# jacklishufan/InstructAny2Pix

Hardware: AMD Instinct MI355X
Metric: denoise-steps/sec (512x512, 50-step DDIM, batch 8) (higher is better)
Workload: dtype f16; 1 GPU; BASELINE configs[2]: 512x512, latent [8,4,64,64], 50-step DDIM, ctx 81 (77 text + 4 IP tokens), SDXL-base UNet + IP-Adapter; global_batch=8, parallelism=dp1, context_kv=projected in every step (reference schedule, as rounds 1-4), ranks=1, dist_backend=none (single process), weight_broadcast_route=none

## Files before the change

### include/ia2p.h

```cpp
#ifndef IA2P_H
#define IA2P_H

#include <stddef.h>
#include <stdint.h>

#ifdef __cplusplus
extern "C" {
#endif

typedef struct ia2p_ctx ia2p_ctx;

typedef enum {
  IA2P_OK = 0,
  IA2P_ERR_INVALID = 1,
  IA2P_ERR_SHAPE = 2,
  IA2P_ERR_KEY = 3,
  IA2P_ERR_STATE = 4,
  IA2P_ERR_NOMEM = 5,
  IA2P_ERR_HIP = 6,
  IA2P_ERR_ARCH = 7
} ia2p_status;

#define IA2P_MAX_BLOCKS 4

typedef struct {
  int in_channels, out_channels;
  int n_blocks;
  int block_out_channels[IA2P_MAX_BLOCKS];
  int transformer_layers_per_block[IA2P_MAX_BLOCKS];
  int num_heads[IA2P_MAX_BLOCKS];
  int layers_per_block;
  int cross_attention_dim;
  int norm_num_groups;
  float norm_eps;
  int addition_time_embed_dim;
  int projection_class_embeddings_input_dim;
  int time_embed_dim;
  int time_proj_dim;
  int mid_transformer_layers;
  int num_time_ids;
} ia2p_unet_config;

ia2p_status ia2p_create(const ia2p_unet_config* cfg, ia2p_ctx** out);
void ia2p_destroy(ia2p_ctx* ctx);
const char* ia2p_last_error(ia2p_ctx* ctx);
int ia2p_device_is_gfx950(void);

size_t ia2p_arena_bytes(ia2p_ctx* ctx);
ia2p_status ia2p_bind_arena(ia2p_ctx* ctx, void* dev_arena, size_t bytes);
ia2p_status ia2p_load_tensor(ia2p_ctx* ctx, const char* key, const void* dev_src, const int64_t* shape, int ndim, void* stream);
ia2p_status ia2p_finalize_weights(ia2p_ctx* ctx);
size_t ia2p_arena_raw_bytes(ia2p_ctx* ctx);
ia2p_status ia2p_adopt_arena(ia2p_ctx* ctx, int with_ip_adapter);
ia2p_status ia2p_adopt_arena_on(ia2p_ctx* ctx, int with_ip_adapter, void* stream);
ia2p_status ia2p_bcast_arena(ia2p_ctx* ctx, void* rccl_comm, int root, int with_ip_adapter, void* stream);
int ia2p_rccl_available(void);
ia2p_status ia2p_set_gn_fuse(ia2p_ctx* ctx, int mode);
ia2p_status ia2p_set_ip_adapter(ia2p_ctx* ctx, int enabled, int num_tokens, float scale);

size_t ia2p_workspace_bytes(ia2p_ctx* ctx, int B, int h, int w, int L);
ia2p_status ia2p_unet_forward(ia2p_ctx* ctx, void* stream, const void* sample, float timestep, const void* context, int L,
                              const void* text_embeds, const void* time_ids, void* out, int B, int h, int w,
                              void* workspace, size_t workspace_bytes);
ia2p_status ia2p_unet_forward_v(ia2p_ctx* ctx, void* stream, const void* sample, const float* timesteps, const float* ip_scales,
                                const void* context, const void* kv, int L, const void* text_embeds, const void* time_ids, void* out,
                                int B, int h, int w, void* workspace, size_t workspace_bytes);

size_t ia2p_context_kv_bytes(ia2p_ctx* ctx, int B, int L);
ia2p_status ia2p_project_context(ia2p_ctx* ctx, void* stream, const void* context, int L, int B, void* kv, size_t kv_bytes,
                                 void* workspace, size_t workspace_bytes);
ia2p_status ia2p_unet_forward_kv(ia2p_ctx* ctx, void* stream, const void* sample, float timestep, const void* kv, int L,
                                 const void* text_embeds, const void* time_ids, void* out, int B, int h, int w,
                                 void* workspace, size_t workspace_bytes);

ia2p_status ia2p_autotune(ia2p_ctx* ctx, void* stream, const void* sample, float timestep, const void* context, int L,
                          const void* text_embeds, const void* time_ids, void* out, int B, int h, int w,
                          void* workspace, size_t workspace_bytes, int reps, int* sites);
size_t ia2p_plan_export(char* buf, size_t len);
int ia2p_plan_import(const char* text);
void ia2p_plan_clear(void);
unsigned long long ia2p_plan_generation(void);

ia2p_status ia2p_ddim_step(void* stream, const void* x, const void* eps_u, const void* eps_c, float g, float c_x, float c_e,
                           void* out, void* out2, int64_t n);
ia2p_status ia2p_ddim_step_v(void* stream, const void* x, const void* eps_u, const void* eps_c, const float* coef, void* out, void* out2,
                             int B, int64_t per);
ia2p_status ia2p_mask_blend(void* stream, const void* x, const void* init, const void* noise, const void* mask, float c0, float c1,
                            void* out, void* out2, int B, int C, int64_t HW);

ia2p_status ia2p_groupnorm_silu(void* stream, const void* x, void* y, const void* gamma, const void* beta, int B, int HW, int C,
                                int groups, float eps, int silu, float* partial_ws );
ia2p_status ia2p_layernorm(void* stream, const void* x, void* y, const void* gamma, const void* beta, int M, int C, float eps);
ia2p_status ia2p_gemm(void* stream, const void* A, const void* W, const void* bias, const void* residual, void* C,
                      int M, int N, int K, int geglu);
typedef struct { const float* stats; int slots; const float* colsum; const float* fbias; float eps; } ia2p_ln_fold;
ia2p_status ia2p_ffn(void* stream, const void* X, const void* W1p, const void* b1p, const void* W2, const void* b2, const void* R, void* H, void* out,
                     int M, int C, int splitk, float* partial);
ia2p_status ia2p_fold_layernorm(void* stream, const void* W, const void* gamma, const void* beta, const void* bias, void* Wf,
                                float* colsum, float* fbias, int N, int K);
ia2p_status ia2p_gemm_ex(void* stream, const void* A, const void* W, const void* bias, const void* residual, void* C, int M, int N, int K,
                         int geglu, const ia2p_ln_fold* ln, float* stats_out, int* stats_slots, int splitk, float* partial);
ia2p_status ia2p_gemm_splitk(void* stream, const void* A, const void* W, const void* bias, const void* residual, void* C,
                             int M, int N, int K, int splitk, float* partial);
ia2p_status ia2p_conv3x3(void* stream, const void* x, const void* Wp, const void* bias, const void* rowvec, const void* residual,
                         void* y, int B, int Hs, int Ws, int Cin, int Co, int stride, int up);
ia2p_status ia2p_gn_colstats(void* stream, const void* x, int M, int C, int rows, double* out );
ia2p_status ia2p_gn_apply_stats(void* stream, const void* x0, int C0, const double* st0, int rows0, const void* x1 , int C1, const double* st1, int rows1,
                                const void* gamma, const void* beta, void* y , int B, int HW, int groups, float eps, int silu);
typedef struct {
  const void* x0; int C0; const double* st0; int rows0;
  const void* x1; int C1; const double* st1; int rows1;
  const void* gamma; const void* beta; int groups; float eps;
  const void* Wp; const void* bias; const void* rowvec; const void* residual; void* y;
  int B, H, W, Co;
  const void* xa; int Ca;
  int splitk; float* partial;
  double* gn_out;
} ia2p_conv_gn;
ia2p_status ia2p_conv3x3_gn(void* stream, const ia2p_conv_gn* d, int* gn_out_rows);
ia2p_status ia2p_gemm_gnstats(void* stream, const void* A, const void* W, const void* bias, const void* residual, void* C, int M, int N, int K, int splitk, float* partial,
                              int HW, double* gn_out, int* rows);
ia2p_status ia2p_conv3x3_splitk(void* stream, const void* x, const void* Wp, const void* bias, const void* rowvec, const void* residual,
                                void* y, int B, int Hs, int Ws, int Cin, int Co, int splitk, float* partial);
ia2p_status ia2p_conv3x3_cat(void* stream, const void* x, const void* x2, const void* Wcat, const void* bias, void* y,
                             int B, int Hs, int Ws, int Cin, int Cin2, int Co);
ia2p_status ia2p_pack_conv3x3(void* stream, const void* w_oihw, void* w_packed, int Co, int Cin);
ia2p_status ia2p_pack_conv_out(void* stream, const void* w_oihw, void* w_packed, int Co, int C);
ia2p_status ia2p_pack_geglu(void* stream, const void* src, void* dst, int rows, int rowlen);
ia2p_status ia2p_conv_in(void* stream, const void* x_nchw, const void* w_oihw, const void* bias, void* y_nhwc, void* w_scratch,
                         int B, int Cin, int H, int W, int Co);
ia2p_status ia2p_conv_out(void* stream, const void* x_nhwc, const void* w_packed, const void* bias, void* y_nchw, int B, int C, int H, int W, int Co);
ia2p_status ia2p_attention(void* stream, const void* Q, int ldq, void* O, int ldo, int B, int heads, int Nq, int nseg,
                           const void* K0, const void* V0, int ld0, int nkeys0, float w0,
                           const void* K1, const void* V1, int ld1, int nkeys1, float w1);
ia2p_status ia2p_qproj_attention(void* stream, const void* X, const void* Wq, const void* bias, const ia2p_ln_fold* ln, void* O, int ldo,
                                 int B, int heads, int Nq, int K, int nseg,
                                 const void* K0, const void* V0, int ld0, int nkeys0, float w0,
                                 const void* K1, const void* V1, int ld1, int nkeys1, float w1);
ia2p_status ia2p_qkv_self_attention(void* stream, const void* X, const void* Wqkv, const void* bias, const ia2p_ln_fold* ln, void* O, int ldo,
                                    int B, int heads, int K);
ia2p_status ia2p_ip_attn_map(void* stream, const void* Q, int ldq, const void* Kip, int ldk, void* out, int B, int heads, int Nq, int ntok);
ia2p_status ia2p_linear_small(void* stream, const void* X, const void* W, const void* bias, void* out, int M, int N, int K,
                              int silu_in, int silu_out);


typedef struct ia2p_vae ia2p_vae;
typedef struct {
  int in_channels, out_channels, latent_channels;
  int n_blocks;
  int block_out_channels[IA2P_MAX_BLOCKS];
  int layers_per_block;
  int norm_num_groups;
  float norm_eps;
  float stream_scale;
} ia2p_vae_config;
ia2p_status ia2p_vae_create(const ia2p_vae_config* cfg, ia2p_vae** out);
void ia2p_vae_destroy(ia2p_vae* vae);
const char* ia2p_vae_last_error(ia2p_vae* vae);
size_t ia2p_vae_arena_bytes(ia2p_vae* vae);
ia2p_status ia2p_vae_bind_arena(ia2p_vae* vae, void* dev_arena, size_t bytes);
ia2p_status ia2p_vae_load_tensor(ia2p_vae* vae, const char* key, const void* dev_src, const int64_t* shape, int ndim, void* stream);
ia2p_status ia2p_vae_finalize_weights(ia2p_vae* vae);
size_t ia2p_vae_workspace_bytes(ia2p_vae* vae, int B, int h, int w, int decode);
ia2p_status ia2p_vae_decode(ia2p_vae* vae, void* stream, const void* latents, void* image, int B, int h, int w, void* workspace, size_t workspace_bytes);
ia2p_status ia2p_vae_encode(ia2p_vae* vae, void* stream, const void* image, void* moments, int B, int h, int w, void* workspace, size_t workspace_bytes);

ia2p_status ia2p_image_from_u8(void* stream, const void* src, void* dst, int B, int H, int W, int C, int normalize);
ia2p_status ia2p_image_to_u8(void* stream, const void* src, void* dst, int B, int H, int W, int C);
ia2p_status ia2p_image_to_f32(void* stream, const void* src, float* dst, int B, int H, int W, int C, int nhwc);
ia2p_status ia2p_image_requantize(void* stream, const void* src, void* dst, int64_t n);

typedef struct ia2p_clip ia2p_clip;
typedef struct {
  int vocab_size, hidden_size, num_layers, num_heads, intermediate_size, max_positions;
  int projection_dim;
  int hidden_act;
  int eos_token_id;
  float layer_norm_eps;
} ia2p_clip_config;
ia2p_status ia2p_clip_create(const ia2p_clip_config* cfg, ia2p_clip** out);
void ia2p_clip_destroy(ia2p_clip* clip);
const char* ia2p_clip_last_error(ia2p_clip* clip);
size_t ia2p_clip_arena_bytes(ia2p_clip* clip);
ia2p_status ia2p_clip_bind_arena(ia2p_clip* clip, void* dev_arena, size_t bytes);
ia2p_status ia2p_clip_load_tensor(ia2p_clip* clip, const char* key, const void* dev_src, const int64_t* shape, int ndim, void* stream);
ia2p_status ia2p_clip_finalize_weights(ia2p_clip* clip);
size_t ia2p_clip_workspace_bytes(ia2p_clip* clip, int B, int T);
ia2p_status ia2p_clip_encode(ia2p_clip* clip, void* stream, const int32_t* input_ids, int B, int T, void* hidden_penultimate,
                             void* last_hidden, void* pooled, void* workspace, size_t workspace_bytes);
ia2p_status ia2p_clip_encode_embeds(ia2p_clip* clip, void* stream, const void* inputs_embeds, int B, int T, void* hidden_penultimate,
                                    void* last_hidden, void* workspace, size_t workspace_bytes);
ia2p_status ia2p_prior_step(void* stream, const float* sample, const void* out_cond, const void* out_uncond, const float* noise, float g,
                            float sqrt_a, float sqrt_b, float k0, float k1, float sigma, float* out, int64_t n);

typedef struct ia2p_llm ia2p_llm;
typedef struct {
  int vocab_size, hidden_size, num_layers, num_heads, num_kv_heads, intermediate_size;
  float rms_norm_eps;
  float rope_theta;
} ia2p_llm_config;
ia2p_status ia2p_llm_create(const ia2p_llm_config* cfg, ia2p_llm** out);
void ia2p_llm_destroy(ia2p_llm* llm);
const char* ia2p_llm_last_error(ia2p_llm* llm);
size_t ia2p_llm_arena_bytes(ia2p_llm* llm);
ia2p_status ia2p_llm_bind_arena(ia2p_llm* llm, void* dev_arena, size_t bytes);
ia2p_status ia2p_llm_load_tensor(ia2p_llm* llm, const char* key, const void* dev_src, const int64_t* shape, int ndim, void* stream);
ia2p_status ia2p_llm_finalize_weights(ia2p_llm* llm);
ia2p_status ia2p_llm_set_weight_format(ia2p_llm* llm, int bits, const float* codebook);
int ia2p_llm_weight_bits(ia2p_llm* llm);
size_t ia2p_llm_kv_bytes(ia2p_llm* llm, int max_positions);
ia2p_status ia2p_llm_bind_kv(ia2p_llm* llm, void* dev_cache, size_t bytes, int max_positions);
size_t ia2p_llm_workspace_bytes(ia2p_llm* llm, int max_T);
ia2p_status ia2p_llm_reset(ia2p_llm* llm);
int ia2p_llm_position(ia2p_llm* llm);
ia2p_status ia2p_llm_embed(ia2p_llm* llm, void* stream, const int32_t* input_ids, int T, void* out);
ia2p_status ia2p_llm_prefill(ia2p_llm* llm, void* stream, const void* inputs_embeds, int T, float* hidden_out, float* logits_out, void* workspace,
                             size_t workspace_bytes);
ia2p_status ia2p_llm_decode(ia2p_llm* llm, void* stream, int token_id, float* hidden_out, float* logits_out, void* workspace, size_t workspace_bytes);
ia2p_status ia2p_llm_gemv(void* stream, const void* W, const float* x, float* out, int N, int K);
size_t ia2p_llm_q4_packed_bytes(int64_t N, int64_t K);
ia2p_status ia2p_llm_quantize_q4(void* stream, const void* W, int64_t N, int64_t K, const float* codebook, void* packed, float* absmax);
ia2p_status ia2p_llm_dequantize_q4(void* stream, const void* packed, const float* absmax, int64_t N, int64_t K, const float* codebook, void* W);
ia2p_status ia2p_llm_gemv_q4(void* stream, const void* packed, const float* absmax, const float* codebook, const float* x, float* out, int N, int K);
ia2p_status ia2p_gelu(void* stream, void* x, int64_t n);

#ifdef __cplusplus
}
#endif
#endif
```

### instructany2pix_amd/_ffi.py

```python
from __future__ import annotations

import ctypes as C
import os

_HERE = os.path.dirname(os.path.abspath(__file__))
LIB_PATH = os.path.join(_HERE, "libia2p_hip.so")

IA2P_OK = 0
_STATUS_NAMES = {1: "INVALID", 2: "SHAPE", 3: "KEY", 4: "STATE", 5: "NOMEM", 6: "HIP", 7: "ARCH"}
MAX_BLOCKS = 4


class UNetConfigC(C.Structure):
    _fields_ = [
        ("in_channels", C.c_int), ("out_channels", C.c_int), ("n_blocks", C.c_int),
        ("block_out_channels", C.c_int * MAX_BLOCKS), ("transformer_layers_per_block", C.c_int * MAX_BLOCKS),
        ("num_heads", C.c_int * MAX_BLOCKS), ("layers_per_block", C.c_int), ("cross_attention_dim", C.c_int),
        ("norm_num_groups", C.c_int), ("norm_eps", C.c_float), ("addition_time_embed_dim", C.c_int),
        ("projection_class_embeddings_input_dim", C.c_int), ("time_embed_dim", C.c_int), ("time_proj_dim", C.c_int),
        ("mid_transformer_layers", C.c_int), ("num_time_ids", C.c_int),
    ]


class LnFoldC(C.Structure):
    _fields_ = [("stats", C.c_void_p), ("slots", C.c_int), ("colsum", C.c_void_p), ("fbias", C.c_void_p), ("eps", C.c_float)]


class CLIPConfigC(C.Structure):
    _fields_ = [("vocab_size", C.c_int), ("hidden_size", C.c_int), ("num_layers", C.c_int), ("num_heads", C.c_int), ("intermediate_size", C.c_int),
                ("max_positions", C.c_int), ("projection_dim", C.c_int), ("hidden_act", C.c_int), ("eos_token_id", C.c_int), ("layer_norm_eps", C.c_float)]


class LLMConfigC(C.Structure):
    _fields_ = [("vocab_size", C.c_int), ("hidden_size", C.c_int), ("num_layers", C.c_int), ("num_heads", C.c_int), ("num_kv_heads", C.c_int),
                ("intermediate_size", C.c_int), ("rms_norm_eps", C.c_float), ("rope_theta", C.c_float)]


class VAEConfigC(C.Structure):
    _fields_ = [("in_channels", C.c_int), ("out_channels", C.c_int), ("latent_channels", C.c_int), ("n_blocks", C.c_int),
                ("block_out_channels", C.c_int * MAX_BLOCKS), ("layers_per_block", C.c_int), ("norm_num_groups", C.c_int),
                ("norm_eps", C.c_float), ("stream_scale", C.c_float)]


class ConvGnC(C.Structure):
    _fields_ = [("x0", C.c_void_p), ("C0", C.c_int), ("st0", C.c_void_p), ("rows0", C.c_int),
                ("x1", C.c_void_p), ("C1", C.c_int), ("st1", C.c_void_p), ("rows1", C.c_int),
                ("gamma", C.c_void_p), ("beta", C.c_void_p), ("groups", C.c_int), ("eps", C.c_float),
                ("Wp", C.c_void_p), ("bias", C.c_void_p), ("rowvec", C.c_void_p), ("residual", C.c_void_p), ("y", C.c_void_p),
                ("B", C.c_int), ("H", C.c_int), ("W", C.c_int), ("Co", C.c_int),
                ("xa", C.c_void_p), ("Ca", C.c_int), ("splitk", C.c_int), ("partial", C.c_void_p), ("gn_out", C.c_void_p)]


_P, _I, _F, _SZ, _I64 = C.c_void_p, C.c_int, C.c_float, C.c_size_t, C.c_int64
SIGNATURES = {
    "ia2p_create": (_I, [C.POINTER(UNetConfigC), C.POINTER(_P)]),
    "ia2p_destroy": (None, [_P]),
    "ia2p_last_error": (C.c_char_p, [_P]),
    "ia2p_device_is_gfx950": (_I, []),
    "ia2p_arena_bytes": (_SZ, [_P]),
    "ia2p_bind_arena": (_I, [_P, _P, _SZ]),
    "ia2p_load_tensor": (_I, [_P, C.c_char_p, _P, C.POINTER(_I64), _I, _P]),
    "ia2p_finalize_weights": (_I, [_P]),
    "ia2p_adopt_arena": (_I, [_P, _I]),
    "ia2p_adopt_arena_on": (_I, [_P, _I, _P]),
    "ia2p_arena_raw_bytes": (_SZ, [_P]),
    "ia2p_bcast_arena": (_I, [_P, _P, _I, _I, _P]),
    "ia2p_rccl_available": (_I, []),
    "ia2p_set_ip_adapter": (_I, [_P, _I, _I, _F]),
    "ia2p_workspace_bytes": (_SZ, [_P, _I, _I, _I, _I]),
    "ia2p_unet_forward": (_I, [_P, _P, _P, _F, _P, _I, _P, _P, _P, _I, _I, _I, _P, _SZ]),
    "ia2p_unet_forward_v": (_I, [_P, _P, _P, _P, _P, _P, _P, _I, _P, _P, _P, _I, _I, _I, _P, _SZ]),
    "ia2p_context_kv_bytes": (_SZ, [_P, _I, _I]),
    "ia2p_project_context": (_I, [_P, _P, _P, _I, _I, _P, _SZ, _P, _SZ]),
    "ia2p_unet_forward_kv": (_I, [_P, _P, _P, _F, _P, _I, _P, _P, _P, _I, _I, _I, _P, _SZ]),
    "ia2p_autotune": (_I, [_P, _P, _P, _F, _P, _I, _P, _P, _P, _I, _I, _I, _P, _SZ, _I, _P]),
    "ia2p_plan_export": (_SZ, [_P, _SZ]),
    "ia2p_plan_import": (_I, [C.c_char_p]),
    "ia2p_plan_clear": (None, []),
    "ia2p_plan_generation": (C.c_ulonglong, []),
    "ia2p_ddim_step": (_I, [_P, _P, _P, _P, _F, _F, _F, _P, _P, _I64]),
    "ia2p_ddim_step_v": (_I, [_P, _P, _P, _P, _P, _P, _P, _I, _I64]),
    "ia2p_mask_blend": (_I, [_P, _P, _P, _P, _P, _F, _F, _P, _P, _I, _I, _I64]),
    "ia2p_groupnorm_silu": (_I, [_P, _P, _P, _P, _P, _I, _I, _I, _I, _F, _I, _P]),
    "ia2p_layernorm": (_I, [_P, _P, _P, _P, _P, _I, _I, _F]),
    "ia2p_gemm": (_I, [_P, _P, _P, _P, _P, _P, _I, _I, _I, _I]),
    "ia2p_gemm_splitk": (_I, [_P, _P, _P, _P, _P, _P, _I, _I, _I, _I, _P]),
    "ia2p_ffn": (_I, [_P, _P, _P, _P, _P, _P, _P, _P, _P, _I, _I, _I, _P]),
    "ia2p_fold_layernorm": (_I, [_P, _P, _P, _P, _P, _P, _P, _P, _I, _I]),
    "ia2p_gemm_ex": (_I, [_P, _P, _P, _P, _P, _P, _I, _I, _I, _I, _P, _P, _P, _I, _P]),
    "ia2p_debug_set_gemm_splitk": (None, [_I]),
    "ia2p_conv3x3": (_I, [_P, _P, _P, _P, _P, _P, _P, _I, _I, _I, _I, _I, _I, _I]),
    "ia2p_conv3x3_splitk": (_I, [_P, _P, _P, _P, _P, _P, _P, _I, _I, _I, _I, _I, _I, _P]),
    "ia2p_pack_conv3x3": (_I, [_P, _P, _P, _I, _I]),
    "ia2p_pack_conv_out": (_I, [_P, _P, _P, _I, _I]),
    "ia2p_conv3x3_cat": (_I, [_P, _P, _P, _P, _P, _P, _I, _I, _I, _I, _I, _I]),
    "ia2p_pack_geglu": (_I, [_P, _P, _P, _I, _I]),
    "ia2p_conv_in": (_I, [_P, _P, _P, _P, _P, _P, _I, _I, _I, _I, _I]),
    "ia2p_conv_out": (_I, [_P, _P, _P, _P, _P, _I, _I, _I, _I, _I]),
    "ia2p_attention": (_I, [_P, _P, _I, _P, _I, _I, _I, _I, _I, _P, _P, _I, _I, _F, _P, _P, _I, _I, _F]),
    "ia2p_qkv_self_attention": (_I, [_P, _P, _P, _P, _P, _P, _I, _I, _I, _I]),
    "ia2p_qproj_attention": (_I, [_P, _P, _P, _P, _P, _P, _I, _I, _I, _I, _I, _I, _P, _P, _I, _I, _F, _P, _P, _I, _I, _F]),
    "ia2p_linear_small": (_I, [_P, _P, _P, _P, _P, _I, _I, _I, _I, _I]),
    "ia2p_ip_attn_map": (_I, [_P, _P, _I, _P, _I, _P, _I, _I, _I, _I]),
    "ia2p_debug_set_gemm_tile": (None, [_I]),
    "ia2p_debug_gemm_tile_info": (_I, [_I, _P]),
    "ia2p_debug_set_xattn_min_tiles": (None, [_I]),
    "ia2p_debug_set_attn_fold": (None, [_I]),
    "ia2p_debug_set_splitk_inkernel": (None, [C.c_longlong]),
    "ia2p_debug_invalidate_splitk_counters": (None, []),
    "ia2p_debug_fill_splitk_counters": (_I, [_P, _I]),
    "ia2p_debug_gemm_plan": (None, [_I, _I, _I, _I, _I, _P, _P]),
    "ia2p_clip_create": (_I, [C.POINTER(CLIPConfigC), C.POINTER(_P)]),
    "ia2p_clip_destroy": (None, [_P]),
    "ia2p_clip_last_error": (C.c_char_p, [_P]),
    "ia2p_clip_arena_bytes": (_SZ, [_P]),
    "ia2p_clip_bind_arena": (_I, [_P, _P, _SZ]),
    "ia2p_clip_load_tensor": (_I, [_P, C.c_char_p, _P, C.POINTER(C.c_int64), _I, _P]),
    "ia2p_clip_finalize_weights": (_I, [_P]),
    "ia2p_clip_workspace_bytes": (_SZ, [_P, _I, _I]),
    "ia2p_clip_encode": (_I, [_P, _P, _P, _I, _I, _P, _P, _P, _P, _SZ]),
    "ia2p_clip_encode_embeds": (_I, [_P, _P, _P, _I, _I, _P, _P, _P, _SZ]),
    "ia2p_prior_step": (_I, [_P, _P, _P, _P, _P, _F, _F, _F, _F, _F, _F, _P, _I64]),
    "ia2p_llm_create": (_I, [C.POINTER(LLMConfigC), C.POINTER(_P)]),
    "ia2p_llm_destroy": (None, [_P]),
    "ia2p_llm_last_error": (C.c_char_p, [_P]),
    "ia2p_llm_arena_bytes": (_SZ, [_P]),
    "ia2p_llm_bind_arena": (_I, [_P, _P, _SZ]),
    "ia2p_llm_load_tensor": (_I, [_P, C.c_char_p, _P, C.POINTER(C.c_int64), _I, _P]),
    "ia2p_llm_finalize_weights": (_I, [_P]),
    "ia2p_llm_kv_bytes": (_SZ, [_P, _I]),
    "ia2p_llm_bind_kv": (_I, [_P, _P, _SZ, _I]),
    "ia2p_llm_workspace_bytes": (_SZ, [_P, _I]),
    "ia2p_llm_reset": (_I, [_P]),
    "ia2p_llm_position": (_I, [_P]),
    "ia2p_llm_embed": (_I, [_P, _P, _P, _I, _P]),
    "ia2p_llm_prefill": (_I, [_P, _P, _P, _I, _P, _P, _P, _SZ]),
    "ia2p_llm_decode": (_I, [_P, _P, _I, _P, _P, _P, _SZ]),
    "ia2p_llm_gemv": (_I, [_P, _P, _P, _P, _I, _I]),
    "ia2p_llm_set_weight_format": (_I, [_P, _I, C.POINTER(_F)]),
    "ia2p_llm_weight_bits": (_I, [_P]),
    "ia2p_llm_q4_packed_bytes": (_SZ, [_I64, _I64]),
    "ia2p_llm_quantize_q4": (_I, [_P, _P, _I64, _I64, C.POINTER(_F), _P, _P]),
    "ia2p_llm_dequantize_q4": (_I, [_P, _P, _P, _I64, _I64, C.POINTER(_F), _P]),
    "ia2p_llm_gemv_q4": (_I, [_P, _P, _P, C.POINTER(_F), _P, _P, _I, _I]),
    "ia2p_gelu": (_I, [_P, _P, _I64]),
    "ia2p_vae_create": (_I, [C.POINTER(VAEConfigC), C.POINTER(_P)]),
    "ia2p_vae_destroy": (None, [_P]),
    "ia2p_vae_last_error": (C.c_char_p, [_P]),
    "ia2p_vae_arena_bytes": (_SZ, [_P]),
    "ia2p_vae_bind_arena": (_I, [_P, _P, _SZ]),
    "ia2p_vae_load_tensor": (_I, [_P, C.c_char_p, _P, C.POINTER(_I64), _I, _P]),
    "ia2p_vae_finalize_weights": (_I, [_P]),
    "ia2p_vae_workspace_bytes": (_SZ, [_P, _I, _I, _I, _I]),
    "ia2p_vae_decode": (_I, [_P, _P, _P, _P, _I, _I, _I, _P, _SZ]),
    "ia2p_vae_encode": (_I, [_P, _P, _P, _P, _I, _I, _I, _P, _SZ]),
    "ia2p_image_from_u8": (_I, [_P, _P, _P, _I, _I, _I, _I, _I]),
    "ia2p_image_to_u8": (_I, [_P, _P, _P, _I, _I, _I, _I]),
    "ia2p_image_to_f32": (_I, [_P, _P, _P, _I, _I, _I, _I, _I]),
    "ia2p_image_requantize": (_I, [_P, _P, _P, _I64]),
    "ia2p_profile_enable": (_I, [_P, _I]),
    "ia2p_profile_classes": (_I, []),
    "ia2p_profile_read_region": (_I, [_P, _I, C.POINTER(_I64), C.POINTER(C.c_double), C.POINTER(C.c_double), C.POINTER(C.c_double)]),
    "ia2p_profile_read_prefetch": (_I, [_P, _I, _P]),
    "ia2p_set_gn_fuse": (_I, [_P, _I]),
    "ia2p_debug_set_gn_plan": (None, [_I]),
    "ia2p_gn_colstats": (_I, [_P, _P, _I, _I, _I, _P]),
    "ia2p_gn_apply_stats": (_I, [_P, _P, _I, _P, _I, _P, _I, _P, _I, _P, _P, _P, _I, _I, _I, _F, _I]),
    "ia2p_conv3x3_gn": (_I, [_P, C.POINTER(ConvGnC), _P]),
    "ia2p_gemm_gnstats": (_I, [_P, _P, _P, _P, _P, _P, _I, _I, _I, _I, _P, _I, _P, _P]),
    "ia2p_profile_roles": (_I, []),
    "ia2p_profile_read_role_class": (_I, [_P, _I, _I, C.POINTER(_I64), C.POINTER(C.c_double)]),
    "ia2p_profile_read_role": (_I, [_P, _I, C.c_char_p, _I, C.POINTER(_I64), C.POINTER(C.c_double), C.POINTER(C.c_double), C.POINTER(C.c_double)]),
    "ia2p_profile_read": (_I, [_P, _I, C.c_char_p, _I, C.POINTER(_I64), C.POINTER(C.c_double), C.POINTER(C.c_double), C.POINTER(C.c_double)]),
}

_lib = None


class IA2PError(RuntimeError):
    pass


def lib() -> C.CDLL:
    global _lib
    if _lib is None:
        if not os.path.exists(LIB_PATH):
            raise IA2PError(f"{LIB_PATH} is missing: build it with `python -m instructany2pix_amd.build` "
                            f"(the denoise path has no non-HIP fallback)")
        import torch
        l = C.CDLL(LIB_PATH)
        for name, (res, args) in SIGNATURES.items():
            fn = getattr(l, name)
            fn.restype, fn.argtypes = res, args
        _lib = l
    return _lib


def check(status: int, ctx=None, vae=False, clip=False, llm=False):
    if status == IA2P_OK:
        return
    msg = (lib().ia2p_llm_last_error(ctx) if llm else lib().ia2p_clip_last_error(ctx) if clip else lib().ia2p_vae_last_error(ctx) if vae
           else lib().ia2p_last_error(ctx))
    msg = msg.decode() if msg else ""
    text = f"ia2p {_STATUS_NAMES.get(status, status)}: {msg}"
    if status in (1, 2):
        raise ValueError(text)
    if status == 3:
        raise KeyError(text)
    if status == 5:
        raise MemoryError(text)
    raise IA2PError(text)


def ptr(t):
    if t is None:
        return None
    assert t.is_cuda and t.is_contiguous(), "ia2p needs contiguous device tensors"
    return C.c_void_p(t.data_ptr())


def current_stream():
    import torch
    return C.c_void_p(torch.cuda.current_stream().cuda_stream)


def make_config(cfg) -> UNetConfigC:
    c = UNetConfigC()
    c.in_channels, c.out_channels = cfg.in_channels, cfg.out_channels
    c.n_blocks = len(cfg.block_out_channels)
    if c.n_blocks > MAX_BLOCKS:
        raise ValueError(f"at most {MAX_BLOCKS} resolution levels are supported")
    for i in range(c.n_blocks):
        c.block_out_channels[i] = cfg.block_out_channels[i]
        c.transformer_layers_per_block[i] = cfg.transformer_layers_per_block[i]
        c.num_heads[i] = cfg.attention_head_dim[i]
    c.layers_per_block = cfg.layers_per_block
    c.cross_attention_dim = cfg.cross_attention_dim
    c.norm_num_groups, c.norm_eps = cfg.norm_num_groups, cfg.norm_eps
    c.addition_time_embed_dim = cfg.addition_time_embed_dim
    c.projection_class_embeddings_input_dim = cfg.projection_class_embeddings_input_dim
    c.time_embed_dim, c.time_proj_dim = cfg.time_embed_dim, cfg.time_proj_dim
    c.mid_transformer_layers, c.num_time_ids = cfg.mid_block_transformer_layers, cfg.num_time_ids
    return c


def make_clip_config(cfg) -> CLIPConfigC:
    c = CLIPConfigC()
    c.vocab_size, c.hidden_size, c.num_layers, c.num_heads = cfg.vocab_size, cfg.hidden_size, cfg.num_hidden_layers, cfg.num_attention_heads
    c.intermediate_size, c.max_positions, c.projection_dim = cfg.intermediate_size, cfg.max_position_embeddings, cfg.projection_dim
    c.hidden_act = {"gelu": 1, "quick_gelu": 2, "gelu_new": 3}[cfg.hidden_act]
    c.eos_token_id, c.layer_norm_eps = cfg.eos_token_id, cfg.layer_norm_eps
    return c

# ... 21 lines not shown
```

### instructany2pix_amd/csrc/common.h

```cpp
#pragma once
#include <hip/hip_runtime.h>
#include <cstdio>
#include <cstdlib>
#include <stdint.h>

typedef _Float16 half_t;
typedef _Float16 h8 __attribute__((ext_vector_type(8)));
typedef _Float16 h4 __attribute__((ext_vector_type(4)));
typedef _Float16 h2 __attribute__((ext_vector_type(2)));
typedef float f4 __attribute__((ext_vector_type(4)));
typedef float f16v __attribute__((ext_vector_type(16)));
typedef __fp16 fp16x4 __attribute__((__vector_size__(4 * sizeof(__fp16))));

#define IA2P_WAVE 64

__device__ __forceinline__ float wave_sum(float v) {
#pragma unroll
  for (int o = 32; o > 0; o >>= 1) v += __shfl_xor(v, o, 64);
  return v;
}
__device__ __forceinline__ float wave_max(float v) {
#pragma unroll
  for (int o = 32; o > 0; o >>= 1) v = fmaxf(v, __shfl_xor(v, o, 64));
  return v;
}
__device__ __forceinline__ float silu_f(float x) { return x * __builtin_amdgcn_rcpf(1.0f + __expf(-x)); }
__device__ __forceinline__ float erf_as_f(float x) {
  const float ax = fabsf(x);
  const float t = __builtin_amdgcn_rcpf(fmaf(0.3275911f, ax, 1.0f));
  const float poly = t * fmaf(t, fmaf(t, fmaf(t, fmaf(t, 1.061405429f, -1.453152027f), 1.421413741f), -0.284496736f), 0.254829592f);
  const float r = 1.0f - poly * __expf(-ax * ax);
  return copysignf(r, x);
}
__device__ __forceinline__ float gelu_erf_f(float x) { return 0.5f * x * (1.0f + erf_as_f(x * 0.70710678118654752440f)); }
constexpr int IA2P_PHI_LUT_N = 513;
__device__ __forceinline__ float gelu_lut_f(float g, const float2* lut) {
  const float f = fmaf(__builtin_amdgcn_fmed3f(g, -8.0f, 7.99f), 32.0f, 256.0f);
  const float fl = floorf(f);
#ifdef IA2P_TIMING_NOLUT
  const float2 e = lut[threadIdx.x & 63];
#else
  const float2 e = lut[(int)fl];
#endif
  return g * fmaf(f - fl, e.y, e.x);
}
__device__ __forceinline__ float quick_gelu_f(float x) { return x * __builtin_amdgcn_rcpf(1.0f + __expf(-1.702f * x)); }
__device__ __forceinline__ float gelu_tanh_f(float x) { return 0.5f * x * (1.0f + tanhf(0.79788456080286535588f * (x + 0.044715f * x * x * x))); }
#ifndef IA2P_WT_AUX
#define IA2P_WT_AUX 16
#endif
__device__ __forceinline__ __amdgpu_buffer_rsrc_t wt_rsrc(void* base, size_t bytes) {
  return __builtin_amdgcn_make_buffer_rsrc(base, 0, (int)(bytes < (size_t)0x7ffffff0 ? bytes : (size_t)0x7ffffff0), 0x00020000);
}
__device__ __forceinline__ void store16_wt(__amdgpu_buffer_rsrc_t r, size_t byte_off, h8 v) {
  typedef unsigned u4v __attribute__((__vector_size__(4 * sizeof(unsigned))));
  __builtin_amdgcn_raw_buffer_store_b128(__builtin_bit_cast(u4v, v), r, (int)byte_off, 0, IA2P_WT_AUX);
}
__device__ __forceinline__ void store8_wt(__amdgpu_buffer_rsrc_t r, size_t byte_off, h4 v) {
  typedef unsigned u2v __attribute__((__vector_size__(2 * sizeof(unsigned))));
  __builtin_amdgcn_raw_buffer_store_b64(__builtin_bit_cast(u2v, v), r, (int)byte_off, 0, IA2P_WT_AUX);
}
static inline const char* ia2p_exp_env(const char* name) {
#ifdef IA2P_EXPERIMENTS
  return getenv(name);
#else
  if (getenv(name)) {
    static thread_local int warned = 0;
    if (warned < 8) { ++warned; fprintf(stderr, "[ia2p] %s is set but this build ignores it (experiment knob: rebuild with IA2P_EXTRA_FLAGS=-DIA2P_EXPERIMENTS)\n", name); }
  }
  return nullptr;
#endif
}
static inline int ia2p_wt_mask() {
  static const int m = getenv("IA2P_WT") ? atoi(getenv("IA2P_WT")) : 31;
  return m;
}

__device__ __forceinline__ float ln_fold_f(float acc, float mean, float rstd, float colsum, float fbias) { return fmaf(rstd, fmaf(-mean, colsum, acc), fbias); }
__device__ __forceinline__ float2 ln_mean_rstd_f(float s1, float s2, int K, float eps) {
  const float inv = 1.f / (float)K;
  const float mean = __fmul_rn(s1, inv);
  const float var = fmaxf(fmaf(s2, inv, -__fmul_rn(mean, mean)), 0.f);
  return make_float2(mean, rsqrtf(__fadd_rn(var, eps)));
}
__device__ __forceinline__ float act_f(float x, int act) { return act == 1 ? gelu_erf_f(x) : act == 2 ? quick_gelu_f(x) : act == 3 ? gelu_tanh_f(x) : x; }


struct GemmArgs {
  const half_t* A;
  const half_t* W;
  half_t* C;
  const half_t* zero;
  int M, N, K;
  int lda, ldc, ldw;
  int rpb, bstride, roff;
  int Hs, Ws;
  int Ho, Wo;
  int stride, up;
  int pad;
  int Cin;
  const half_t* A2; int lda2, Cin2;
  const half_t* A3; int lda3, Cin3;
  const half_t* bias;
  const half_t* rowvec;
  int rowvec_ld, rows_per_batch;
  const half_t* residual;
  int ldr;
  int geglu;
  const float* phi_lut;
  int m_fastest;
  int vec8;
  int c_wt;
  int group_w;
  const void* pf;
  long pf_bytes;
  int pf_blocks;
  int splitk;
  float* partial;
#ifdef IA2P_CLOCK_STAMP
  unsigned long long* stamp;
#endif
  int* sk_counters;
  float acc_scale, bias_scale;
  int act;
  const float* ln_stats;
  int ln_slots;
  const float* ln_cs;
  const float* ln_bias;
  float ln_eps;
  float* stats_out;
  double* gn_out;
  const half_t* A1b; int lda1b;
  struct GnIn {
    const double* st0; int rows0;
    const double* st1; int rows1;
    int C0;
    const half_t* gamma; const half_t* beta;
    int gs;
    int groups;
    float eps; int silu;
  } gn;
};

static inline bool ia2p_fits_buffer(size_t rows, size_t ld) { return rows * ld * 2 < (size_t)0x7ffffe00; }
constexpr int IA2P_GN_MAX_SLOTS = 16;
static inline bool ia2p_conv_gn_ok(const GemmArgs& a) {
  if (!a.gn.st0) return true;
  const int HW = a.Ho * a.Wo, C1 = a.Cin - a.gn.C0;
  return a.up == 0 && a.gn.silu && a.gn.gamma && a.gn.beta && a.gn.groups > 0 && a.gn.groups <= 64 && a.gn.gs > 0 && a.gn.gs * a.gn.groups == a.Cin && a.gn.gs <= 96 && a.gn.C0 > 0 && a.gn.C0 % 64 == 0 && C1 >= 0 && C1 % 64 == 0 &&
         a.gn.rows0 > 0 && HW % a.gn.rows0 == 0 && HW / a.gn.rows0 <= IA2P_GN_MAX_SLOTS && ((C1 == 0 && !a.gn.st1 && !a.A1b) || (C1 > 0 && a.gn.st1 && a.A1b && a.lda1b >= C1 && a.gn.rows1 > 0 && HW % a.gn.rows1 == 0 &&
         HW / a.gn.rows1 <= IA2P_GN_MAX_SLOTS && ia2p_fits_buffer(a.M, a.lda1b))) && a.Cin <= 48 * 1024 / 16;
}
static inline bool ia2p_conv_halo_ok(const GemmArgs& a) {
  const int c2 = a.A2 ? a.Cin2 : 0, c3 = a.A3 ? a.Cin3 : 0;
  return a.stride == 1 && (a.up == 0 || (a.up == 1 && !a.A2)) && a.pad == 1 && (a.Hs << a.up) == a.Ho && (a.Ws << a.up) == a.Wo && a.Ho > 0 && a.Ho % 16 == 0 && a.Wo % 16 == 0 && a.Cin >= 64 && a.Cin % 64 == 0 && c2 % 64 == 0 &&
         c3 % 64 == 0 && a.Cin2 == c2 && (a.A3 == nullptr || a.A2 != nullptr) && a.K == 9 * a.Cin + c2 + c3 && a.M % (a.Ho * a.Wo) == 0 && !a.rpb && !a.geglu &&
         ia2p_fits_buffer(a.M, a.lda) && ia2p_fits_buffer(a.N, a.ldw) && (!a.A2 || ia2p_fits_buffer(a.M, a.lda2)) && (!a.A3 || ia2p_fits_buffer(a.M, a.lda3));
}

struct GemmPlan { int variant; int splitk; int gn = 0; };
static inline bool ia2p_tile_geglu_only(int pp) { return pp == 4; }
static inline bool ia2p_geglu320_shape_ok(int M, int N, int K, bool conv, bool geglu) { return geglu && !conv && M > 0 && M % 256 == 0 && N > 0 && N % 320 == 0 && K >= 64 && K % 64 == 0; }
struct GemmTile { int bm, bn, stages, pp, halo; };
constexpr int IA2P_GEMM_NVARIANT = 28;
constexpr GemmTile IA2P_GEMM_TILES[IA2P_GEMM_NVARIANT] = {{128, 128, 2, 0, 0}, {128, 128, 3, 0, 0}, {128, 64, 2, 0, 0}, {128, 64, 3, 0, 0}, {64, 64, 2, 0, 0}, {64, 64, 3, 0, 0},
                                                          {64, 160, 2, 0, 0}, {64, 160, 3, 0, 0}, {128, 160, 2, 0, 0}, {128, 160, 3, 0, 0}, {160, 128, 2, 0, 0}, {160, 160, 2, 0, 0},
                                                          {256, 128, 3, 1, 0},
                                                          {64, 64, 4, 0, 0}, {64, 64, 6, 0, 0}, {128, 64, 4, 0, 0},
                                                          {128, 80, 2, 0, 0}, {128, 80, 4, 0, 0},
                                                          {256, 160, 3, 1, 0},
                                                          {128, 160, 3, 1, 0},
                                                          {32, 64, 3, 0, 0}, {32, 128, 3, 0, 0},
                                                          {256, 256, 2, 2, 0}, {256, 128, 2, 2, 0},
                                                          {256, 160, 3, 1, 1}, {256, 128, 3, 1, 1},
                                                          {256, 80, 3, 1, 1},
                                                          {256, 320, 2, 4, 0}};
GemmPlan ia2p_gemm_plan(int M, int N, int K, bool conv, bool geglu);
bool ia2p_plan_lookup(int M, int N, int K, bool conv, bool geglu, GemmPlan* out);
void ia2p_plan_set(int M, int N, int K, bool conv, bool geglu, GemmPlan pl);

struct AttnSeg {
  const half_t* K;
  const half_t* V;
  int nkeys, ld, rows_per_batch;
  float weight;
};

struct AttnArgs {
  const half_t* Q;
  half_t* O;
  int ldq, ldo, B, heads, Nq, nseg;
  float scale_log2e;
  int xcd_map;
  AttnSeg seg[2];
  const float* w1_b;
};
```

### instructany2pix_amd/csrc/engine.hip

```cpp
#include "engine_rt.h"

#include <dlfcn.h>
#include <rccl/rccl.h>

thread_local std::string g_err;

const half_t* zero_page() {
  static thread_local void* z[16] = {nullptr};
  int dev = 0;
  if (hipGetDevice(&dev) != hipSuccess || dev < 0 || dev >= 16) return nullptr;
  if (!z[dev]) {
    if (hipMalloc(&z[dev], 256) != hipSuccess) return nullptr;
    (void)hipMemset(z[dev], 0, 256);
  }
  return (const half_t*)z[dev];
}

struct Resnet {
  int cin, cout, temb_off;
  bool shortcut;
  size_t n1g, n1b, w1, b1, n2g, n2b, w2, b2, wsc, bsc;
  size_t wcat, bcat;
};
struct TBlock {
// ... 244 lines not shown
  if (c->temb_total != tot) return fail(c, IA2P_ERR_STATE, "internal: time_emb_proj stacking mismatch %d != %d", c->temb_total, tot);
  if (P.kv_cursor != c->kv_rows) return fail(c, IA2P_ERR_STATE, "internal: context K/V stacking mismatch %d != %d", P.kv_cursor, c->kv_rows);
  c->ngo = P.vec("conv_norm_out.weight", ch[0]); c->nbo = P.vec("conv_norm_out.bias", ch[0]);
  c->conv_out_w = P.conv3("conv_out.weight", g.out_channels, ch[0], PK_CONV_TAP); c->conv_out_b = P.vec("conv_out.bias", g.out_channels);

  int idx = 0;
  auto add_ip = [&](std::vector<std::pair<std::string, size_t>>& v) {
    for (auto& s : v) {
      const std::string& q = s.first;
      const size_t cc = (size_t)std::llround(std::sqrt((double)c->params[q + ".attn2.to_q.weight"].elems));
      const std::string k = "ip_adapter." + std::to_string(2 * idx + 1);
      P.reg(k + ".to_k_ip.weight", s.second, cc * ctx, PK_COPY, 0, 0, true);
      P.reg(k + ".to_v_ip.weight", s.second + cc * ctx, cc * ctx, PK_COPY, 0, 0, true);
      ++idx;
    }
  };
  add_ip(ipslots_down); add_ip(ipslots_up); add_ip(ipslots_mid);
  c->n_attn2 = idx;
  *raw_elems = P.cur; *fold_elems = P.fold_cur;
  return IA2P_OK;
}
static ia2p_status build_plan(ia2p_ctx* c) {
  size_t raw = 0, fold = 0;
  ia2p_status st = plan_pass(c, 0, &raw, &fold);
  if (st != IA2P_OK) return st;
  st = plan_pass(c, raw, &raw, &fold);
  if (st != IA2P_OK) return st;
  c->arena_raw_elems = raw;
  c->arena_elems = raw + fold;
  return IA2P_OK;
}

T2 wsalloc(RunCtx* c, size_t elems) {
  const size_t off = c->ws.alloc(elems * sizeof(half_t));
  if (off == (size_t)-1) { if (!c->failed) fail(c, IA2P_ERR_NOMEM, "workspace too small"); return T2{off, nullptr}; }
  return T2{off, c->dry ? nullptr : (half_t*)(c->ws_base + off)};
}
void wsfree(RunCtx* c, T2 t) {
  if (t.off == (size_t)-1) return;
  c->ws.release(t.off);
}

hipEvent_t get_event(RunCtx* c) {
  if (!c->evpool.empty()) { hipEvent_t e = c->evpool.back(); c->evpool.pop_back(); return e; }
  hipEvent_t e; (void)hipEventCreate(&e); return e;
}
static void set_prefetch(RunCtx* c, GemmArgs& a, const half_t* W, size_t bytes) {
  if (c->dry) { if (c->record) c->wseq.push_back({W, bytes}); return; }
  if (!c->prefetch || c->widx + 1 > c->wseq.size()) { ++c->widx; return; }
  const bool last = c->widx + 1 == c->wseq.size();
  if (last && !c->tail_pf) { ++c->widx; return; }
  const std::pair<const half_t*, size_t> nx = last ? std::make_pair(c->tail_pf, c->tail_pf_bytes) : c->wseq[c->widx + 1];
  ++c->widx;
  if (nx.second > ((size_t)96 << 20)) return;
  a.pf = nx.first; a.pf_bytes = (long)nx.second;
  static const size_t pf_cap = ia2p_exp_env("IA2P_PF_BLOCKS") ? (size_t)atoi(ia2p_exp_env("IA2P_PF_BLOCKS")) : 128;
  static const size_t pf_per = ia2p_exp_env("IA2P_PF_BLOCK_BYTES") ? (size_t)atol(ia2p_exp_env("IA2P_PF_BLOCK_BYTES")) : 131072;
  a.pf_blocks = (int)std::max<size_t>(1, std::min<size_t>(pf_cap, (nx.second + pf_per - 1) / pf_per));
}

static void tune_site(RunCtx* c, const GemmArgs& a, bool conv) {
  const GemmArgs* fa = c->tune_fused;
  const float gn_ms = (float)c->tune_gn_ms;
  c->tune_fused = nullptr; c->tune_gn_ms = 0.0;
  if (ia2p_plan_lookup(a.M, a.N, a.K, conv, a.geglu != 0, nullptr)) return;
  std::vector<GemmPlan> cands;
  ia2p_gemm_candidates(a.M, a.N, a.K, conv, a.geglu != 0, c->tune_slab_bytes, ia2p_exp_env("IA2P_TUNE_SLACK") ? atof(ia2p_exp_env("IA2P_TUNE_SLACK")) : 2.5, &cands);
  static const bool tune_log = getenv("IA2P_TUNE_LOG") != nullptr;
  hipEvent_t e0 = get_event(c), e1 = get_event(c);
  std::vector<float> best_ms(cands.size(), 1e30f);
  std::vector<char> ok(cands.size(), 1);
  for (size_t i = 0; i < cands.size(); ++i)
    if (IA2P_GEMM_TILES[cands[i].variant].halo && !(conv && ia2p_conv_halo_ok(a) && cands[i].splitk <= a.Cin / 64)) ok[i] = 0;
  for (int r = -1; r < c->tune_reps; ++r)
    for (size_t i = 0; i < cands.size(); ++i) {
      if (!ok[i]) continue;
      GemmArgs b = a;
      b.splitk = cands[i].splitk > 1 ? cands[i].splitk : 0;
      b.partial = cands[i].splitk > 1 ? (float*)c->tune_scratch : nullptr;
      bool good = hipMemsetAsync(c->tune_scratch + c->tune_slab_bytes, r & 1, c->tune_flush_bytes, c->stream) == hipSuccess;
      const size_t a_bytes = conv ? (size_t)(a.M / std::max(1, a.Ho * a.Wo)) * a.Hs * a.Ws * a.Cin * sizeof(half_t)
                                  : (a.rpb ? 0 : (size_t)a.M * a.lda * sizeof(half_t));
      good = good && ia2p_launch_touch(a.A, std::min<size_t>(a_bytes, (size_t)64 << 20), (unsigned*)c->tune_scratch, c->stream) == hipSuccess;
      if (a.residual) good = good && ia2p_launch_touch(a.residual, std::min<size_t>((size_t)a.M * a.ldr * sizeof(half_t), (size_t)64 << 20), (unsigned*)c->tune_scratch, c->stream) == hipSuccess;
      good = good && hipEventRecord(e0, c->stream) == hipSuccess;
      good = good && ia2p_launch_gemm_variant(b, conv, cands[i].variant, c->stream) == hipSuccess;
      good = good && hipEventRecord(e1, c->stream) == hipSuccess && hipEventSynchronize(e1) == hipSuccess;
      float ms = 0.f;
      good = good && hipEventElapsedTime(&ms, e0, e1) == hipSuccess;
      if (!good) { (void)hipGetLastError(); ok[i] = 0; continue; }
      if (r >= 0 && ms < best_ms[i]) best_ms[i] = ms;
    }
  c->evpool.push_back(e0); c->evpool.push_back(e1);
  float fastest = 1e30f;
  for (size_t i = 0; i < cands.size(); ++i) {
    if (!ok[i]) continue;
    if (tune_log) fprintf(stderr, "[ia2p tune] %d %d %d conv=%d geglu=%d variant=%d splitk=%d us=%.2f\n", a.M, a.N, a.K, (int)conv, a.geglu, cands[i].variant, cands[i].splitk, 1e3 * best_ms[i]);
    fastest = std::min(fastest, best_ms[i]);
  }
  GemmPlan best{-1, 1};
  for (size_t i = 0; i < cands.size() && best.variant < 0; ++i)
    if (ok[i] && best_ms[i] <= 1.02f * fastest) best = cands[i];
  if (fa && conv && best.variant >= 0 && gn_ms > 0.f) {
    std::vector<GemmPlan> fc;
    ia2p_conv_gn_candidates(*fa, c->tune_slab_bytes, &fc);
    std::vector<float> fms(fc.size(), 1e30f);
    hipEvent_t f0 = get_event(c), f1 = get_event(c);
    for (int r = -1; r < c->tune_reps; ++r)
      for (size_t i = 0; i < fc.size(); ++i) {
        GemmArgs b = *fa;
        b.splitk = fc[i].splitk > 1 ? fc[i].splitk : 0;
        b.partial = fc[i].splitk > 1 ? (float*)c->tune_scratch : nullptr;
        bool good = hipMemsetAsync(c->tune_scratch + c->tune_slab_bytes, r & 1, c->tune_flush_bytes, c->stream) == hipSuccess;
        const size_t a_bytes = (size_t)(fa->M / std::max(1, fa->Ho * fa->Wo)) * fa->Hs * fa->Ws * fa->gn.C0 * sizeof(half_t);
        good = good && ia2p_launch_touch(fa->A, std::min<size_t>(a_bytes, (size_t)64 << 20), (unsigned*)c->tune_scratch, c->stream) == hipSuccess;
        if (fa->A1b) good = good && ia2p_launch_touch(fa->A1b, std::min<size_t>((size_t)fa->M * fa->lda1b * sizeof(half_t), (size_t)64 << 20), (unsigned*)c->tune_scratch, c->stream) == hipSuccess;
        if (fa->residual) good = good && ia2p_launch_touch(fa->residual, std::min<size_t>((size_t)fa->M * fa->ldr * sizeof(half_t), (size_t)64 << 20), (unsigned*)c->tune_scratch, c->stream) == hipSuccess;
        good = good && hipEventRecord(f0, c->stream) == hipSuccess;
        good = good && ia2p_launch_gemm_variant(b, true, fc[i].variant, c->stream) == hipSuccess;
        good = good && hipEventRecord(f1, c->stream) == hipSuccess && hipEventSynchronize(f1) == hipSuccess;
        float ms = 0.f;
        good = good && hipEventElapsedTime(&ms, f0, f1) == hipSuccess;
        if (!good) { (void)hipGetLastError(); fms[i] = -1.f; continue; }
        if (r >= 0 && fms[i] >= 0.f && ms < fms[i]) fms[i] = ms;
      }
    c->evpool.push_back(f0); c->evpool.push_back(f1);
    float unfused = 1e30f;
    for (size_t i = 0; i < cands.size(); ++i)
      if (ok[i]) unfused = std::min(unfused, best_ms[i]);
    unfused += gn_ms;
    int bi = -1;
    for (size_t i = 0; i < fc.size(); ++i) {
      if (tune_log && fms[i] >= 0.f) fprintf(stderr, "[ia2p tune] %d %d %d conv=1 FUSED groupnorm variant=%d splitk=%d us=%.2f (groupnorm launch %.2f us + best plain plan = %.2f us)\n", fa->M, fa->N, fa->K, fc[i].variant, fc[i].splitk,
                                             1e3 * fms[i], 1e3 * gn_ms, 1e3 * unfused);
      if (fms[i] >= 0.f && fms[i] < 1e29f && (bi < 0 || fms[i] < fms[bi])) bi = (int)i;
    }
    if (bi >= 0 && fms[bi] < 0.97f * unfused) best = fc[bi];
  }
  if (best.variant < 0) { fail(c, IA2P_ERR_HIP, "autotune: no candidate plan ran for %d x %d x %d", a.M, a.N, a.K); return; }
  ia2p_plan_set(a.M, a.N, a.K, conv, a.geglu != 0, best);
  ++c->tune_sites;
}

static int gn_fallback_rows(int HW) {
  for (int k = 1; k <= HW / 16; ++k)
    if (HW % k == 0 && (HW / k) % 16 == 0 && HW / k <= 1024) return HW / k;
  return 0;
}
static int gn_epilogue_rows(const GemmArgs& a, bool conv, int variant, int splitk, bool combined, int HW) {
  const int bm = IA2P_GEMM_TILES[ia2p_gemm_variant_ran(a, conv, variant)].bm;
  return (!a.geglu && !a.act && a.ldc % 8 == 0 && a.N % 8 == 0 && bm % 16 == 0 && HW % bm == 0 && a.M % HW == 0 && HW / bm <= IA2P_GN_MAX_SLOTS && (splitk <= 1 || combined)) ? bm : 0;
}
static void run_gemm(RunCtx* c, GemmArgs& a, bool conv, const char* what, double flops, double bytes, int* stat_slots = nullptr, GnWant* gw = nullptr) {
  if (c->tuning && !c->dry && !c->failed) tune_site(c, a, conv);
  c->tune_fused = nullptr; c->tune_gn_ms = 0.0;
  const GemmPlan pl = ia2p_gemm_plan(a.M, a.N, a.K, conv, a.geglu != 0);
  if (pl.variant < 0 || pl.variant >= IA2P_GEMM_NVARIANT) { fail(c, IA2P_ERR_INVALID, "%s: tile variant %d out of range", what, pl.variant); return; }
  if (c->tuning && !c->dry && pl.splitk > 1 && (size_t)pl.splitk * a.M * a.N * sizeof(float) > c->tune_slab_bytes) {
    fail(c, IA2P_ERR_NOMEM, "%s: plan (variant %d, K split %d) needs %zu bytes of slabs, the autotune scratch holds %zu", what, pl.variant, pl.splitk,
         (size_t)pl.splitk * a.M * a.N * sizeof(float), c->tune_slab_bytes);
    return;
  }
  T2 slab{(size_t)-1, nullptr};
  if (pl.splitk > 1) {
    a.splitk = pl.splitk;
    if (c->tuning && !c->dry) a.partial = (float*)c->tune_scratch;
    else { slab = wsalloc(c, (size_t)pl.splitk * a.M * a.N * 2); a.partial = (float*)slab.p; }
  }
  struct Rel { RunCtx* c; T2 t; ~Rel() { wsfree(c, t); } } rel{c, slab};
  int combined = pl.splitk > 1 && ia2p_splitk_inkernel(a.M, a.N, pl.splitk);
  int gn_rows_epi = 0;
  if (gw) {
    gw->out = GnStats{};
    gn_rows_epi = gn_epilogue_rows(a, conv, pl.variant, pl.splitk, combined != 0, gw->HW);
    if (gn_rows_epi) {
      gw->out.buf = wsalloc(c, (size_t)(a.M / gn_rows_epi) * a.N * 8);
      a.gn_out = (double*)gw->out.buf.p;
    }
  }
#ifdef IA2P_CLOCK_STAMP
  if (c->stamp_buf && c->role == c->stamp_role && (pl.splitk <= 1 || combined) && !c->dry && !c->tuning && c->stamp_n < c->stamp_cap) {
    const GemmTile& t = IA2P_GEMM_TILES[pl.variant];
    const int tiles = ((a.M + t.bm - 1) / t.bm) * ((a.N + t.bn - 1) / t.bn) * (pl.splitk > 1 ? pl.splitk : 1);
    if (tiles <= RunCtx::STAMP_WG && !t.halo) {
      unsigned long long* rec = c->stamp_buf + (size_t)c->stamp_n * RunCtx::STAMP_WG * 8;
      if (pl.splitk > 1) a.stamp = rec;
      else a.partial = (float*)rec;
      c->stamp_meta.push_back({a.M, a.N, a.K, pl.splitk > 1 ? -100 * pl.splitk - pl.variant : pl.variant, tiles});
      ++c->stamp_n;
    }
  }
#endif
  {
    ProfScope ps(c, (conv ? PK_CONV0 : PK_GEMM0) + pl.variant, flops, bytes);
    ps.pf = a.pf ? (double)a.pf_bytes : 0.0;
    int ran = pl.variant;
    CHECK_LAUNCH(c, ia2p_launch_gemm_variant(a, conv, pl.variant, c->stream, false, &combined, &ran), what);
    ps.set_class(conv && a.gn.st0 && ran >= 24 && ran <= 26 ? PK_HALO_GN0 + ran - 24 : (conv ? PK_CONV0 : PK_GEMM0) + ran);
  }
  if (pl.splitk > 1 && !combined) {
    ProfScope ps(c, PK_REDUCE, 0, (double)pl.splitk * a.M * a.N * 4 + 2.0 * a.M * a.N);
    CHECK_LAUNCH(c, ia2p_launch_splitk_reduce(a, c->stream), what);
  }
  if (gw && gw->out.buf.off != (size_t)-1) {
    if (gn_rows_epi && (pl.splitk <= 1 || combined)) gw->out.rows = gn_rows_epi;
    else { wsfree(c, gw->out.buf); gw->out = GnStats{}; }
  }
  if (stat_slots) *stat_slots = (pl.splitk > 1 && !combined) ? 1 : (a.N + IA2P_GEMM_TILES[pl.variant].bn - 1) / IA2P_GEMM_TILES[pl.variant].bn;
}

static GemmArgs gemm_args(RunCtx* c, const half_t* A, int lda, const half_t* W, const half_t* bias, const half_t* residual, int ldr,
                          half_t* C, int ldc, int M, int N, int K, int geglu, int rpb, int bstride, int roff, int ldw,
                          const LnIn* ln, float* stats_out, int act) {
  GemmArgs a;
  memset(&a, 0, sizeof a);
  a.pad = 1;
  if (ln) { a.ln_stats = ln->stats; a.ln_slots = ln->slots; a.ln_cs = ln->cs; a.ln_bias = ln->lb; a.ln_eps = ln->eps; }
  a.stats_out = stats_out;
  a.act = act;
  a.A = A; a.W = W; a.C = C; a.zero = zero_page(); a.M = M; a.N = N; a.K = K; a.ldw = ldw ? ldw : K; a.lda = lda; a.ldc = ldc;
  a.rpb = rpb; a.bstride = bstride; a.roff = roff; a.bias = bias; a.residual = residual; a.ldr = ldr; a.geglu = geglu;
  a.rows_per_batch = 1;
  a.m_fastest = (long)M * K <= (long)N * K ? 1 : 0;
  a.acc_scale = c->ep_acc_scale; a.bias_scale = c->ep_bias_scale; c->ep_acc_scale = c->ep_bias_scale = 1.f;
  return a;
}
static double gemm_bytes(int M, int N, int K, int geglu, bool residual) { return 2.0 * ((double)M * K + (double)N * K + (double)M * (geglu ? N / 2 : N) + (residual ? (double)M * N : 0)); }
void op_gemm(RunCtx* c, const half_t* A, int lda, const half_t* W, const half_t* bias, const half_t* residual, int ldr,
             half_t* C, int ldc, int M, int N, int K, int geglu, int rpb, int bstride, int roff, int ldw,
             const LnIn* ln, float* stats_out, int* stat_slots, int act, GnWant* gw) {
  GemmArgs a = gemm_args(c, A, lda, W, bias, residual, ldr, C, ldc, M, N, K, geglu, rpb, bstride, roff, ldw, ln, stats_out, act);
  set_prefetch(c, a, W, (size_t)N * K * sizeof(half_t));
  run_gemm(c, a, false, "gemm", 2.0 * M * N * K, gemm_bytes(M, N, K, geglu, residual != nullptr), stat_slots, gw);
}
static void run_ffn(RunCtx* c, GemmArgs& a, GemmArgs& b, int* stat_slots_b) {
  set_prefetch(c, a, a.W, (size_t)a.N * a.K * sizeof(half_t));
  set_prefetch(c, b, b.W, (size_t)b.N * b.K * sizeof(half_t));
  { RoleScope role(c, ROLE_FF_IN); run_gemm(c, a, false, "ff.net.0", 2.0 * a.M * (double)a.N * a.K, gemm_bytes(a.M, a.N, a.K, 1, false)); }
  RoleScope role(c, ROLE_FF_OUT);
  run_gemm(c, b, false, "ff.net.2", 2.0 * b.M * (double)b.N * b.K, gemm_bytes(b.M, b.N, b.K, 0, true), stat_slots_b);
}
void op_conv3(RunCtx* c, const half_t* X, int B, int Hs, int Ws, int Cin, const half_t* W, const half_t* bias, int Co,
              int stride, int up, const half_t* rowvec, int rowvec_ld, const half_t* residual, half_t* Y, int pad_lo, const half_t* X2, int Cin2,
              const half_t* X3, int Cin3, const ConvGn* gn, GnWant* gw) {
  GemmArgs a;
  memset(&a, 0, sizeof a);
  if ((Cin2 > 0 && (stride != 1 || up || pad_lo != 1 || Cin2 % 64)) || (Cin3 > 0 && (Cin2 <= 0 || Cin3 % 64)) || Cin2 < 0 || Cin3 < 0 ||
      (!c->dry && ((Cin2 > 0) != (X2 != nullptr) || (Cin3 > 0) != (X3 != nullptr)))) { fail(c, IA2P_ERR_SHAPE, "conv3x3 with appended 1x1 blocks: stride 1, no upsampling, Cin2 / Cin3 %% 64 == 0 (stride %d up %d pad %d Cin %d Cin2 %d Cin3 %d, X2 %s, X3 %s)", stride, up, pad_lo, Cin, Cin2, Cin3, X2 ? "set" : "null", X3 ? "set" : "null"); return; }
  a.pad = pad_lo;
  const int Hv = Hs << up, Wv = Ws << up;
  a.Ho = (Hv + pad_lo + 1 - 3) / stride + 1; a.Wo = (Wv + pad_lo + 1 - 3) / stride + 1;
  a.A = X; a.W = W; a.C = Y; a.zero = zero_page(); a.M = B * a.Ho * a.Wo; a.N = Co; a.K = 9 * Cin + Cin2 + Cin3; a.ldw = a.K; a.lda = Cin; a.ldc = Co;
  if (gn && gn->fused) {
    a.lda = gn->C0; a.A1b = gn->X1b; a.lda1b = Cin - gn->C0;
    a.gn.st0 = (const double*)gn->s0.buf.p; a.gn.rows0 = gn->s0.rows; a.gn.st1 = (const double*)gn->s1.buf.p; a.gn.rows1 = gn->s1.rows; a.gn.C0 = gn->C0;
    a.gn.gamma = gn->gamma; a.gn.beta = gn->beta; a.gn.groups = gn->groups; a.gn.gs = Cin / gn->groups; a.gn.eps = gn->eps; a.gn.silu = 1;
  }
  a.A2 = X2; a.lda2 = Cin2; a.Cin2 = Cin2;
  a.A3 = X3; a.lda3 = Cin3; a.Cin3 = Cin3;
  a.Hs = Hs; a.Ws = Ws; a.stride = stride; a.up = up; a.Cin = Cin;
  a.bias = bias; a.rowvec = rowvec; a.rowvec_ld = rowvec_ld; a.rows_per_batch = a.Ho * a.Wo; a.residual = residual; a.ldr = Co;
  a.m_fastest = 0;
  a.acc_scale = c->ep_acc_scale; a.bias_scale = c->ep_bias_scale; c->ep_acc_scale = c->ep_bias_scale = 1.f;
  set_prefetch(c, a, W, (size_t)Co * a.K * sizeof(half_t));
  GemmArgs fa;
  if (gn && gn->tune && !gn->fused && c->tuning && !c->dry && gn->s0.ok() && gn->Xraw) {
    fa = a;
    fa.A = gn->Xraw; fa.lda = gn->C0; fa.A1b = gn->X1b; fa.lda1b = Cin - gn->C0;
    fa.gn.st0 = (const double*)gn->s0.buf.p; fa.gn.rows0 = gn->s0.rows; fa.gn.st1 = gn->X1b ? (const double*)gn->s1.buf.p : nullptr; fa.gn.rows1 = gn->s1.rows; fa.gn.C0 = gn->C0;
    fa.gn.gamma = gn->gamma; fa.gn.beta = gn->beta; fa.gn.groups = gn->groups; fa.gn.gs = Cin / gn->groups; fa.gn.eps = gn->eps; fa.gn.silu = 1;
    if (ia2p_conv_gn_ok(fa)) c->tune_fused = &fa;
  }
  RoleScope role(c, ROLE_CONV3X3);
  run_gemm(c, a, true, "conv3x3", 2.0 * a.M * (double)Co * a.K, 2.0 * ((double)B * Hs * Ws * Cin + (double)Co * a.K + (double)a.M * Co + (residual ? (double)a.M * Co : 0) + (double)a.M * (Cin2 + Cin3)), nullptr, gw);
}
void op_gn(RunCtx* c, const half_t* x, half_t* y, size_t g, size_t b, int B, int HW, int C, float eps, int silu, float* partial, const half_t* x2, int Ca) {
  RoleScope role(c, ROLE_GROUPNORM);
  ProfScope ps(c, PK_GN, 8.0 * B * HW * C, 4.0 * B * HW * C);
  if (x2) CHECK_LAUNCH(c, ia2p_launch_groupnorm(x, Ca, y, C, W_(c, g), W_(c, b), partial, B, HW, C, c->groups, eps, silu, c->stream, x2, C - Ca, Ca), "groupnorm");
  else CHECK_LAUNCH(c, ia2p_launch_groupnorm(x, C, y, C, W_(c, g), W_(c, b), partial, B, HW, C, c->groups, eps, silu, c->stream), "groupnorm");
}
void op_ln(RunCtx* c, const half_t* x, half_t* y, size_t g, size_t b, int M, int C) {
  ProfScope ps(c, PK_LN, 8.0 * M * C, 4.0 * M * C);
  CHECK_LAUNCH(c, ia2p_launch_layernorm(x, C, y, C, W_(c, g), W_(c, b), M, C, 1e-5f, c->stream), "layernorm");
}

struct Fwd {
  ia2p_ctx* c;
  int B, h, w, L;
  const half_t* ctxp;
  T2 temb_all;
  float* gn_partial;
  T2 kv_text, kv_ip;
  const float* ip_scales = nullptr;
  std::unordered_map<size_t, GnStats> gst;
  bool gn_on = false;
  bool tune_like = false;
};
static void gst_put(Fwd& f, T2 t, const GnStats& s) { if (s.ok() && t.off != (size_t)-1) f.gst[t.off] = s; else if (s.buf.off != (size_t)-1) wsfree(f.c, s.buf); }
static GnStats gst_get(Fwd& f, T2 t) { auto it = f.gst.find(t.off); return it == f.gst.end() ? GnStats{} : it->second; }
static void act_free(Fwd& f, T2 t) {
  auto it = f.gst.find(t.off);
  if (it != f.gst.end()) { wsfree(f.c, it->second.buf); f.gst.erase(it); }
  wsfree(f.c, t);
}

struct TuneGnTimer {
  RunCtx* c; hipEvent_t e0{}, e1{}; bool on;
  explicit TuneGnTimer(RunCtx* c_) : c(c_), on(c_->tuning && !c_->dry && !c_->failed && c_->gn_fuse != 0) {
    if (on) { e0 = get_event(c); e1 = get_event(c); (void)hipEventRecord(e0, c->stream); }
  }
  void stop() {
    if (!on) return;
    float ms = 0.f;
    if (hipEventRecord(e1, c->stream) == hipSuccess && hipEventSynchronize(e1) == hipSuccess && hipEventElapsedTime(&ms, e0, e1) == hipSuccess) c->tune_gn_ms = ms;
    c->evpool.push_back(e0); c->evpool.push_back(e1);
    on = false;
  }
};
struct RegionScope { RunCtx* c; int prev; RegionScope(RunCtx* c_, int r) : c(c_), prev(c_->region) { c->region = r; } ~RegionScope() { c->region = prev; } };

static bool gn_conv_fusable(Fwd& f, int H, int Wd, int cin, int cout, int cin2, int cin3, const GnStats& s0, const GnStats* s1, int c0) {
  if (!f.gn_on || !s0.ok() || (s1 && !s1->ok())) return false;
  GemmArgs a;
  memset(&a, 0, sizeof a);
  a.pad = 1; a.Hs = a.Ho = H; a.Ws = a.Wo = Wd; a.stride = 1; a.Cin = cin; a.M = f.B * H * Wd; a.N = cout; a.K = 9 * cin + cin2 + cin3; a.lda = c0; a.ldw = a.K; a.ldc = cout;
  a.Cin2 = cin2; a.Cin3 = cin3; a.lda2 = cin2; a.lda3 = cin3;
  if (cin2) a.A2 = (const half_t*)16;
  if (cin3) a.A3 = (const half_t*)16;
  const GemmPlan pl = ia2p_gemm_plan(a.M, a.N, a.K, true, false);
  if (!pl.gn || !ia2p_conv_gn_fusable(a, pl.variant, pl.splitk)) return false;
  const int HW = H * Wd, groups = f.c->groups;
  if (cin % groups || cin / groups > 96 || c0 % 64 || (cin - c0) % 64 || cin > 3072) return false;
  return HW % s0.rows == 0 && HW / s0.rows <= IA2P_GN_MAX_SLOTS && (!s1 || (HW % s1->rows == 0 && HW / s1->rows <= IA2P_GN_MAX_SLOTS));
}

static GnStats gn_ensure_stats(Fwd& f, T2 t, int C, int HW) {
  GnStats s = gst_get(f, t);
  if (s.ok() && HW % s.rows == 0 && HW / s.rows <= IA2P_GN_MAX_SLOTS) return s;
  RunCtx* c = f.c;
  const int rows = gn_fallback_rows(HW);
  if (!rows || C % 8) return GnStats{};
  auto it = f.gst.find(t.off);
  if (it != f.gst.end()) { wsfree(c, it->second.buf); f.gst.erase(it); }
  s = GnStats{};
  s.buf = wsalloc(c, (size_t)(f.B * HW / rows) * C * 8);
  s.rows = rows;
  {
    RoleScope role(c, ROLE_GROUPNORM);
    ProfScope ps(c, PK_GN, 4.0 * f.B * HW * C, 2.0 * f.B * HW * C);
    CHECK_LAUNCH(c, ia2p_launch_gn_colstats(t.p, C, f.B * HW, C, rows, (double*)s.buf.p, c->stream), "groupnorm statistics");
  }
  f.gst[t.off] = s;
  return s;
}

static T2 run_resnet(Fwd& f, const Resnet& r, T2 x, int H, int Wd, const T2* x2t = nullptr, int cx = 0, bool out_stats = false) {
  const half_t* x2 = x2t ? x2t->p : nullptr;
  const bool two = x2t != nullptr;
  ia2p_ctx* c = f.c;
  RegionScope rs(c, PR_CONV_BLOCK);
  const int HW = H * Wd, M = f.B * HW;
  GnStats probe; probe.rows = gn_fallback_rows(HW);
  GnStats sx, sx2;
  bool fuse1 = probe.ok() && gn_conv_fusable(f, H, Wd, r.cin, r.cout, 0, 0, probe, two ? &probe : nullptr, two ? cx : r.cin);
  if (fuse1) {
    sx = gn_ensure_stats(f, x, two ? cx : r.cin, HW);
    if (two) sx2 = gn_ensure_stats(f, *x2t, r.cin - cx, HW);
    fuse1 = gn_conv_fusable(f, H, Wd, r.cin, r.cout, 0, 0, sx, two ? &sx2 : nullptr, two ? cx : r.cin);
  }
  GnWant w1{HW};
  const bool cat = r.shortcut && c->sc_fuse;
  const bool want1 = f.gn_on && probe.ok() && gn_conv_fusable(f, H, Wd, r.cout, r.cout, cat ? (two ? cx : r.cin) : 0, cat && two ? r.cin - cx : 0, probe, nullptr, r.cout);
  T2 hh = wsalloc(c, (size_t)M * r.cout);
  const bool twin = (c->gn_dry_mode >= 0 ? c->gn_dry_mode : c->gn_fuse) == 2;
  auto apply_stats = [&](const half_t* a0, int c0, const half_t* a1, const GnStats& s0, const GnStats& s1, size_t gam, size_t bet, int C, half_t* y) {
    GemmArgs::GnIn g;
    memset(&g, 0, sizeof g);
    g.st0 = (const double*)s0.buf.p; g.rows0 = s0.rows; g.st1 = a1 ? (const double*)s1.buf.p : nullptr; g.rows1 = s1.rows; g.C0 = c0; g.gamma = W_(c, gam); g.beta = W_(c, bet);
    g.groups = c->groups; g.gs = C / c->groups; g.eps = c->cfg.norm_eps; g.silu = 1;
    RoleScope role(c, ROLE_GROUPNORM);
    ProfScope ps(c, PK_GN, 8.0 * M * C, 4.0 * M * C);
    CHECK_LAUNCH(c, ia2p_launch_gn_apply_stats(a0, c0, a1, C - c0, y, C, f.B, HW, C, g, c->stream), "groupnorm (apply from producer statistics)");
  };
  if (fuse1 && twin) {
    T2 n1 = wsalloc(c, (size_t)M * r.cin);
    apply_stats(x.p, two ? cx : r.cin, x2, sx, sx2, r.n1g, r.n1b, r.cin, n1.p);
    op_conv3(c, n1.p, f.B, H, Wd, r.cin, W_(c, r.w1), W_(c, r.b1), r.cout, 1, 0, c->dry ? nullptr : f.temb_all.p + r.temb_off, c->temb_total, nullptr, hh.p, 1, nullptr, 0, nullptr, 0, nullptr, want1 ? &w1 : nullptr);
    wsfree(c, n1);
  } else if (fuse1) {
    ConvGn g;
    g.fused = true; g.X1b = x2; g.C0 = two ? cx : r.cin; g.s0 = sx; g.s1 = sx2; g.gamma = W_(c, r.n1g); g.beta = W_(c, r.n1b); g.eps = c->cfg.norm_eps; g.groups = c->groups;
    op_conv3(c, x.p, f.B, H, Wd, r.cin, W_(c, r.w1), W_(c, r.b1), r.cout, 1, 0, c->dry ? nullptr : f.temb_all.p + r.temb_off, c->temb_total, nullptr, hh.p, 1, nullptr, 0, nullptr, 0, &g, want1 ? &w1 : nullptr);
  } else {
    T2 n1 = wsalloc(c, (size_t)M * r.cin);
    const bool tune = f.tune_like && probe.ok() && H % 16 == 0 && Wd % 16 == 0;
    ConvGn tg1;
    if (tune) {
      tg1.tune = true; tg1.Xraw = x.p; tg1.X1b = x2; tg1.C0 = two ? cx : r.cin; tg1.gamma = W_(c, r.n1g); tg1.beta = W_(c, r.n1b); tg1.eps = c->cfg.norm_eps; tg1.groups = c->groups;
      tg1.s0 = gn_ensure_stats(f, x, tg1.C0, HW);
      if (two) tg1.s1 = gn_ensure_stats(f, *x2t, r.cin - cx, HW);
    }
    TuneGnTimer tg(c);
    op_gn(c, x.p, n1.p, r.n1g, r.n1b, f.B, HW, r.cin, c->cfg.norm_eps, 1, f.gn_partial, x2, cx);
    tg.stop();
    op_conv3(c, n1.p, f.B, H, Wd, r.cin, W_(c, r.w1), W_(c, r.b1), r.cout, 1, 0, c->dry ? nullptr : f.temb_all.p + r.temb_off, c->temb_total, nullptr, hh.p, 1, nullptr, 0, nullptr, 0, tune ? &tg1 : nullptr,
             want1 ? &w1 : nullptr);
    wsfree(c, n1);
  }
  const GnStats sh = w1.out;
  const bool fuse2 = want1 && gn_conv_fusable(f, H, Wd, r.cout, r.cout, cat ? (two ? cx : r.cin) : 0, cat && two ? r.cin - cx : 0, sh, nullptr, r.cout);
  ConvGn g2;
  g2.fused = fuse2 && !twin; g2.C0 = r.cout; g2.s0 = sh; g2.gamma = W_(c, r.n2g); g2.beta = W_(c, r.n2b); g2.eps = c->cfg.norm_eps; g2.groups = c->groups;
  T2 n2{(size_t)-1, nullptr};
  const bool tune2 = f.tune_like && probe.ok() && H % 16 == 0 && Wd % 16 == 0;
  if (tune2) {
    g2.tune = true; g2.Xraw = hh.p;
    g2.s0 = gn_ensure_stats(f, hh, r.cout, HW);
  }
  if (!fuse2 || twin) {
    n2 = wsalloc(c, (size_t)M * r.cout);
    if (fuse2) apply_stats(hh.p, r.cout, nullptr, sh, GnStats{}, r.n2g, r.n2b, r.cout, n2.p);
    else {
      TuneGnTimer tg(c);
      op_gn(c, hh.p, n2.p, r.n2g, r.n2b, f.B, HW, r.cout, c->cfg.norm_eps, 1, f.gn_partial);
      tg.stop();
    }
    if (!tune2) wsfree(c, hh);
  }
  const half_t* in2 = g2.fused ? hh.p : n2.p;
  GnWant w2{HW};
  GnWant* gw2 = f.gn_on && out_stats && ia2p_plan_any_gn(M) ? &w2 : nullptr;
  T2 xs{(size_t)-1, nullptr};
  const half_t* resid = x.p;
  if (r.shortcut && !cat) {
    xs = wsalloc(c, (size_t)M * r.cout);
    { RoleScope role(c, ROLE_CONV3X3); op_gemm(c, x.p, r.cin, W_(c, r.wsc), W_(c, r.bsc), nullptr, 0, xs.p, r.cout, M, r.cout, r.cin); }
    resid = xs.p;
  }
  T2 out = wsalloc(c, (size_t)M * r.cout);
  if (cat && two) op_conv3(c, in2, f.B, H, Wd, r.cout, W_(c, r.wcat), W_(c, r.bcat), r.cout, 1, 0, nullptr, 0, nullptr, out.p, 1, x.p, cx, x2, r.cin - cx, &g2, gw2);
  else if (cat) op_conv3(c, in2, f.B, H, Wd, r.cout, W_(c, r.wcat), W_(c, r.bcat), r.cout, 1, 0, nullptr, 0, nullptr, out.p, 1, x.p, r.cin, nullptr, 0, &g2, gw2);
  else op_conv3(c, in2, f.B, H, Wd, r.cout, W_(c, r.w2), W_(c, r.b2), r.cout, 1, 0, nullptr, 0, c->dry ? nullptr : resid, out.p, 1, nullptr, 0, nullptr, 0, &g2, gw2);
  if (g2.fused) wsfree(c, hh); else { wsfree(c, n2); if (tune2) act_free(f, hh); }
  if (sh.buf.off != (size_t)-1) wsfree(c, sh.buf);
  if (r.shortcut && !cat) wsfree(c, xs);
  if (gw2) gst_put(f, out, w2.out);
  return out;
}

static void op_qkv_sattn(RunCtx* c, const half_t* A, int lda, const half_t* W, const LnIn* ln, int M, int C, const AttnArgs& x) {
  GemmArgs a;
  memset(&a, 0, sizeof a);
  a.pad = 1;
  if (ln) { a.ln_stats = ln->stats; a.ln_slots = ln->slots; a.ln_cs = ln->cs; a.ln_bias = ln->lb; a.ln_eps = ln->eps; }
  a.A = A; a.W = W; a.zero = zero_page(); a.M = M; a.N = 3 * C; a.K = C; a.ldw = C; a.lda = lda; a.ldc = 3 * C;
  a.rows_per_batch = 1;
  set_prefetch(c, a, W, (size_t)3 * C * C * sizeof(half_t));
  RoleScope role(c, ROLE_QKV_SATTN);
#ifdef IA2P_CLOCK_STAMP
  if (c->stamp_buf && c->role == c->stamp_role && !c->dry && !c->tuning && c->stamp_n < c->stamp_cap && x.B * x.heads <= RunCtx::STAMP_WG) {
    a.partial = (float*)(c->stamp_buf + (size_t)c->stamp_n * RunCtx::STAMP_WG * 8);
    c->stamp_meta.push_back({a.M, a.N, a.K, -4, x.B * x.heads});
    ++c->stamp_n;
  }
#endif
  ProfScope ps(c, PK_QKVATTN, 2.0 * M * 3.0 * C * C + 4.0 * x.B * x.heads * (double)x.Nq * x.Nq * 64, 2.0 * ((double)M * C + 3.0 * C * C + (double)M * C));
  ps.pf = a.pf ? (double)a.pf_bytes : 0.0;
  CHECK_LAUNCH(c, ia2p_launch_qkv_sattn(a, x, c->stream), "qkv projection + self-attention");
}

static void op_attn(RunCtx* c, const AttnArgs& a) {
  double keys = 0;
  for (int s = 0; s < a.nseg; ++s) keys += a.seg[s].nkeys;
  ProfScope ps(c, PK_ATTN, 4.0 * a.B * a.heads * (double)a.Nq * keys * 64, 2.0 * ((double)a.B * a.Nq * a.heads * 64 * 2 + 2.0 * a.B * keys * a.heads * 64));
  CHECK_LAUNCH(c, ia2p_launch_attention(a, c->stream), "attention");
}

static void op_qxattn(RunCtx* c, const half_t* A, int lda, const half_t* W, const LnIn* ln, int M, int N, int K, const AttnArgs& x) {
  GemmArgs a;
  memset(&a, 0, sizeof a);
  a.pad = 1;
  if (ln) { a.ln_stats = ln->stats; a.ln_slots = ln->slots; a.ln_cs = ln->cs; a.ln_bias = ln->lb; a.ln_eps = ln->eps; }
  a.A = A; a.W = W; a.zero = zero_page(); a.M = M; a.N = N; a.K = K; a.ldw = K; a.lda = lda; a.ldc = N;
  a.rows_per_batch = 1;
  a.m_fastest = M <= N ? 1 : 0;
  a.acc_scale = a.bias_scale = 1.f;
  set_prefetch(c, a, W, (size_t)N * K * sizeof(half_t));
  double keys = 0;
  for (int s = 0; s < x.nseg; ++s) keys += x.seg[s].nkeys;
  RoleScope role(c, ROLE_Q_XATTN);
#ifdef IA2P_CLOCK_STAMP
  if (c->stamp_buf && c->role == c->stamp_role && !c->dry && !c->tuning && c->stamp_n < c->stamp_cap && (M / 128) * (N / 64) <= RunCtx::STAMP_WG) {
    a.partial = (float*)(c->stamp_buf + (size_t)c->stamp_n * RunCtx::STAMP_WG * 8);
    c->stamp_meta.push_back({a.M, a.N, a.K, -5, (M / 128) * (N / 64)});
    ++c->stamp_n;
  }
#endif
  ProfScope ps(c, PK_QXATTN, 2.0 * M * N * K + 4.0 * x.B * x.heads * (double)x.Nq * keys * 64,
               2.0 * ((double)M * K + (double)N * K + (double)M * N + 2.0 * x.B * keys * x.heads * 64));
  CHECK_LAUNCH(c, ia2p_launch_qproj_xattn(a, x, c->stream), "to_q + cross-attention");
}

static T2 run_transformer(Fwd& f, const Transformer& t, T2 x, int H, int Wd, bool out_stats = false) {
  ia2p_ctx* c = f.c;
  RegionScope rs(c, PR_TRANSFORMER);
  const int HW = H * Wd, M = f.B * HW, C = t.c;
  const int ctxd = c->cfg.cross_attention_dim;
  const int Lt = c->ip_enabled ? f.L - c->ip_tokens : f.L;
  const int Li = c->ip_enabled ? c->ip_tokens : 0;
  const float sl2e = 0.125f * 1.4426950408889634f;
  T2 n = wsalloc(c, (size_t)M * C);
  op_gn(c, x.p, n.p, t.ng, t.nb, f.B, HW, C, 1e-6f, 0, f.gn_partial);
  T2 tk = wsalloc(c, (size_t)M * C);
  T2 stt = wsalloc(c, (size_t)M * ((C + 63) / 64) * 2 * 2);
  float* st = (float*)stt.p;
  int slots = 0;
  const float eps = 1e-5f;
  auto F_ = [&](size_t off) { return (const float*)(c->arena + off); };
  const bool fold = c->ln_fold;
  if (!fold) st = nullptr;
  { RoleScope role(c, ROLE_PROJ_IO); op_gemm(c, n.p, C, W_(c, t.win), W_(c, t.bin), nullptr, 0, tk.p, C, M, C, C, 0, 0, 0, 0, 0, nullptr, st, &slots); }
  wsfree(c, n);
  T2 lnb = fold ? T2{(size_t)-1, nullptr} : wsalloc(c, (size_t)M * C);
  T2 qkv = wsalloc(c, (size_t)M * 3 * C), att = wsalloc(c, (size_t)M * C);
  T2 ff = wsalloc(c, (size_t)M * 4 * C);
  const int ldkv = c->kv_rows;
  for (const TBlock& b : t.blocks) {
    {
    RoleScope role_sa(c, ROLE_QKV_SATTN);
#ifdef IA2P_NO_SATTN_FUSE
    bool fuse_sa = false;
#else
    bool fuse_sa = fold && c->sattn_fuse && HW == 256 && C == t.heads * 64 && (long)f.B * t.heads >= c->xattn_min_tiles;
#endif
    AttnArgs sa;
    memset(&sa, 0, sizeof sa);
    sa.O = att.p; sa.ldo = C; sa.B = f.B; sa.heads = t.heads; sa.Nq = HW; sa.nseg = 1; sa.scale_log2e = sl2e;
    sa.seg[0].nkeys = HW; sa.seg[0].weight = 1.f;
    if (fuse_sa) {
      GemmArgs g;
      memset(&g, 0, sizeof g);
      g.A = tk.p; g.W = W_(c, b.fqkv); g.M = M; g.N = 3 * C; g.K = C; g.lda = C; g.ldw = C; g.ldc = 3 * C;
      g.ln_stats = st; g.ln_slots = slots; g.ln_cs = F_(b.cs1); g.ln_bias = F_(b.lb1);
      fuse_sa = ia2p_qkv_sattn_ok(g, sa);
    }
    if (fuse_sa) {
      const LnIn ln{st, slots, F_(b.cs1), F_(b.lb1), eps};
      op_qkv_sattn(c, tk.p, C, W_(c, b.fqkv), &ln, M, C, sa);
    } else if (fold) {
      const LnIn ln{st, slots, F_(b.cs1), F_(b.lb1), eps};
      op_gemm(c, tk.p, C, W_(c, b.fqkv), nullptr, nullptr, 0, qkv.p, 3 * C, M, 3 * C, C, 0, 0, 0, 0, 0, &ln);
    } else {
      op_ln(c, tk.p, lnb.p, b.ln1g, b.ln1b, M, C);
      op_gemm(c, lnb.p, C, W_(c, b.wqkv), nullptr, nullptr, 0, qkv.p, 3 * C, M, 3 * C, C);
    }
    if (!fuse_sa) {
      AttnArgs a;
      memset(&a, 0, sizeof a);
      a.Q = qkv.p; a.ldq = 3 * C; a.O = att.p; a.ldo = C; a.B = f.B; a.heads = t.heads; a.Nq = HW; a.nseg = 1; a.scale_log2e = sl2e;
      a.seg[0].K = c->dry ? nullptr : qkv.p + C; a.seg[0].V = c->dry ? nullptr : qkv.p + 2 * C;
      a.seg[0].nkeys = HW; a.seg[0].ld = 3 * C; a.seg[0].rows_per_batch = HW; a.seg[0].weight = 1.f;
      op_attn(c, a);
    }
    }
    { RoleScope role(c, ROLE_ATTN_OUT); op_gemm(c, att.p, C, W_(c, b.wo1), W_(c, b.bo1), tk.p, C, tk.p, C, M, C, C, 0, 0, 0, 0, 0, nullptr, st, &slots); }
    {
      RoleScope role(c, ROLE_Q_XATTN);
      AttnArgs a;
      memset(&a, 0, sizeof a);
      a.Q = qkv.p; a.ldq = C; a.O = att.p; a.ldo = C; a.B = f.B; a.heads = t.heads; a.Nq = HW; a.nseg = Li ? 2 : 1; a.scale_log2e = sl2e;
      const half_t* kt = c->dry ? nullptr : f.kv_text.p + b.kv_col;
      const half_t* ki = (c->dry || !Li) ? nullptr : f.kv_ip.p + b.kv_col;
      a.seg[0].K = kt; a.seg[0].V = c->dry ? nullptr : kt + C; a.seg[0].nkeys = Lt; a.seg[0].ld = ldkv; a.seg[0].rows_per_batch = Lt; a.seg[0].weight = 1.f;
      a.seg[1].K = ki; a.seg[1].V = ki ? ki + C : nullptr; a.seg[1].nkeys = Li; a.seg[1].ld = ldkv; a.seg[1].rows_per_batch = Li; a.seg[1].weight = c->ip_scale;
      a.w1_b = Li ? f.ip_scales : nullptr;
      const bool fuse = c->xattn_fuse && HW % 128 == 0 && C == t.heads * 64 && (Lt + 63) / 64 + (Li + 63) / 64 <= 3 && (long)(M / 128) * t.heads >= c->xattn_min_tiles;
      if (fold) {
        const LnIn ln{st, slots, F_(b.cs2), F_(b.lb2), eps};
        if (fuse) op_qxattn(c, tk.p, C, W_(c, b.fq2), &ln, M, C, C, a);
        else op_gemm(c, tk.p, C, W_(c, b.fq2), nullptr, nullptr, 0, qkv.p, C, M, C, C, 0, 0, 0, 0, 0, &ln);
      } else {
        op_ln(c, tk.p, lnb.p, b.ln2g, b.ln2b, M, C);
        if (fuse) op_qxattn(c, lnb.p, C, W_(c, b.wq2), nullptr, M, C, C, a);
        else op_gemm(c, lnb.p, C, W_(c, b.wq2), nullptr, nullptr, 0, qkv.p, C, M, C, C);
      }
      if (!fuse) op_attn(c, a);
    }
    { RoleScope role(c, ROLE_ATTN_OUT); op_gemm(c, att.p, C, W_(c, b.wo2), W_(c, b.bo2), tk.p, C, tk.p, C, M, C, C, 0, 0, 0, 0, 0, nullptr, st, &slots); }
    if (!fold) op_ln(c, tk.p, lnb.p, b.ln3g, b.ln3b, M, C);
    {
      const LnIn ln{st, slots, F_(b.cs3), F_(b.lb3), eps};
      GemmArgs g1 = fold ? gemm_args(c, tk.p, C, W_(c, b.fff1), W_(c, b.bff1), nullptr, 0, ff.p, 4 * C, M, 8 * C, C, 1, 0, 0, 0, 0, &ln, nullptr, 0)
                         : gemm_args(c, lnb.p, C, W_(c, b.wff1), W_(c, b.bff1), nullptr, 0, ff.p, 4 * C, M, 8 * C, C, 1, 0, 0, 0, 0, nullptr, nullptr, 0);
      GemmArgs g2 = gemm_args(c, ff.p, 4 * C, W_(c, b.wff2), W_(c, b.bff2), tk.p, C, tk.p, C, M, C, 4 * C, 0, 0, 0, 0, 0, nullptr, st, 0);
      run_ffn(c, g1, g2, &slots);
    }
  }
  wsfree(c, stt); wsfree(c, lnb); wsfree(c, qkv); wsfree(c, att); wsfree(c, ff);
  (void)ctxd;
  T2 out = wsalloc(c, (size_t)M * C);
  GnWant gw{HW};
  const bool want = f.gn_on && out_stats && ia2p_plan_any_gn(M);
  { RoleScope role(c, ROLE_PROJ_IO); op_gemm(c, tk.p, C, W_(c, t.wout), W_(c, t.bout), x.p, C, out.p, C, M, C, C, 0, 0, 0, 0, 0, nullptr, nullptr, nullptr, 0, want ? &gw : nullptr); }
  wsfree(c, tk);
  if (want) gst_put(f, out, gw.out);
  return out;
}

static void project_context(ia2p_ctx* c, const half_t* context, int L, int B, half_t* kv_text, half_t* kv_ip) {
  RegionScope rs(c, PR_TRANSFORMER);
  RoleScope role(c, ROLE_CTX_KV);
  const int ctxd = c->cfg.cross_attention_dim;
  const int Lt = c->ip_enabled ? L - c->ip_tokens : L, Li = c->ip_enabled ? c->ip_tokens : 0;
  op_gemm(c, context, ctxd, W_(c, c->kv_text_base), nullptr, nullptr, 0, kv_text, c->kv_rows, B * Lt, c->kv_rows, ctxd, 0, Lt, L, 0);
  if (Li) op_gemm(c, context, ctxd, W_(c, c->kv_ip_base), nullptr, nullptr, 0, kv_ip, c->kv_rows, B * Li, c->kv_rows, ctxd, 0, Li, L, Lt);
}

static ia2p_status run_forward(ia2p_ctx* c, const half_t* sample, float timestep, const half_t* context, int L,
                               const half_t* text_embeds, const half_t* time_ids, half_t* out, int B, int h, int w,
                               const half_t* kv_cached = nullptr, const float* timesteps = nullptr, const float* ip_scales = nullptr) {
  const ia2p_unet_config& g = c->cfg;
  const int n = g.n_blocks;
  const int T = g.time_embed_dim, Tp = g.time_proj_dim, Ain = g.projection_class_embeddings_input_dim, Ad = g.addition_time_embed_dim;
  const int pooled = Ain - g.num_time_ids * Ad;
  Fwd f{c, B, h, w, L, context, T2{(size_t)-1, nullptr}, nullptr, T2{(size_t)-1, nullptr}, T2{(size_t)-1, nullptr}};
  f.ip_scales = ip_scales;
  const int gn_mode = c->gn_dry_mode >= 0 ? c->gn_dry_mode : c->gn_fuse;
  f.tune_like = c->gn_fuse != 0 && (c->dry ? c->gn_dry_mode == 3 || (c->gn_dry_mode < 0 && c->tuning) : c->tuning);
  f.gn_on = gn_mode != 0 && gn_mode != 3 && !c->tuning;

  T2 gnp = wsalloc(c, (size_t)B * 64 * g.norm_num_groups * 2 * 2);
  f.gn_partial = (float*)gnp.p;
  T2 tsin = wsalloc(c, (size_t)B * Tp), addin = wsalloc(c, (size_t)B * Ain), e1 = wsalloc(c, (size_t)B * T), emb0 = wsalloc(c, (size_t)B * T);
  T2 a1 = wsalloc(c, (size_t)B * T), emb = wsalloc(c, (size_t)B * T);
  f.temb_all = wsalloc(c, (size_t)B * c->temb_total);
  {
    RoleScope role(c, ROLE_EMBED);
    ProfScope ps(c, PK_EMBED, 0, 0);
    CHECK_LAUNCH(c, ia2p_launch_embed(timestep, timesteps, text_embeds, time_ids, tsin.p, addin.p, B, Tp, pooled, Ad, g.num_time_ids, c->stream), "embed");
    auto lin = [&](const half_t* X, int ldx, size_t w, size_t b, const half_t* add, int ldadd, half_t* o, int ldo, int N, int K, int si, int so, const char* what) {
      for (int r0 = 0; r0 < B; r0 += 16) {
        const int rows = std::min(16, B - r0);
        CHECK_LAUNCH(c, ia2p_launch_linear_small(c->dry ? nullptr : X + (size_t)r0 * ldx, ldx, W_(c, w), W_(c, b), (c->dry || !add) ? nullptr : add + (size_t)r0 * ldadd, ldadd,
                                                 c->dry ? nullptr : o + (size_t)r0 * ldo, ldo, rows, N, K, si, so, c->stream), what);
      }
    };
    lin(tsin.p, Tp, c->te1w, c->te1b, nullptr, 0, e1.p, T, T, Tp, 0, 1, "time_embedding.linear_1");
    lin(e1.p, T, c->te2w, c->te2b, nullptr, 0, emb0.p, T, T, T, 0, 0, "time_embedding.linear_2");
    lin(addin.p, Ain, c->ae1w, c->ae1b, nullptr, 0, a1.p, T, T, Ain, 0, 1, "add_embedding.linear_1");
    lin(a1.p, T, c->ae2w, c->ae2b, emb0.p, T, emb.p, T, T, T, 0, 1, "add_embedding.linear_2 (+ SiLU)");
    lin(emb.p, T, c->tw_all, c->tb_all, nullptr, 0, f.temb_all.p, c->temb_total, c->temb_total, T, 0, 0, "time_emb_proj (stacked)");
  }
  wsfree(c, tsin); wsfree(c, addin); wsfree(c, e1); wsfree(c, emb0); wsfree(c, a1); wsfree(c, emb);

  if (c->kv_rows > 0) {
    const int Lt = c->ip_enabled ? L - c->ip_tokens : L, Li = c->ip_enabled ? c->ip_tokens : 0;
    if (kv_cached) {
      f.kv_text.p = const_cast<half_t*>(kv_cached);
      if (Li) f.kv_ip.p = const_cast<half_t*>(kv_cached) + (size_t)B * Lt * c->kv_rows;
    } else {
      f.kv_text = wsalloc(c, (size_t)B * Lt * c->kv_rows);
      if (Li) f.kv_ip = wsalloc(c, (size_t)B * Li * c->kv_rows);
      project_context(c, context, L, B, f.kv_text.p, f.kv_ip.p);
    }
  }

  RegionScope rs_conv(c, PR_CONV_BLOCK);
  int H = h, Wd = w;
  std::vector<T2> skips;
  std::vector<int> skip_c;
  T2 x = wsalloc(c, (size_t)B * H * Wd * g.block_out_channels[0]);
  {
    RoleScope role(c, ROLE_CONV_IO);
    ProfScope ps(c, PK_CONV_IN, 2.0 * B * H * Wd * 9.0 * g.in_channels * g.block_out_channels[0],
                 2.0 * ((double)B * H * Wd * (g.in_channels + g.block_out_channels[0]) + 64.0 * g.block_out_channels[0]));
    CHECK_LAUNCH(c, ia2p_launch_conv_in(sample, W_(c, c->conv_in_w), W_(c, c->conv_in_b), x.p, B, g.in_channels, H, Wd, g.block_out_channels[0], c->stream), "conv_in");
  }
  skips.push_back(x); skip_c.push_back(g.block_out_channels[0]);
  for (int i = 0; i < n; ++i) {
    const Stage& st = c->down[i];
    for (size_t j = 0; j < st.res.size(); ++j) {
      const bool att = !st.att.empty();
      T2 r = run_resnet(f, st.res[j], x, H, Wd, nullptr, 0, !att);
      if (att) { T2 t = run_transformer(f, st.att[j], r, H, Wd, true); act_free(f, r); r = t; }
      x = r;
      skips.push_back(x); skip_c.push_back(st.res[j].cout);
    }
    if (st.resample) {
      const int Ho = (H - 1) / 2 + 1, Wo = (Wd - 1) / 2 + 1;
      T2 d = wsalloc(c, (size_t)B * Ho * Wo * st.rc);
      GnWant gw{Ho * Wo};
      const bool want = f.gn_on && ia2p_plan_any_gn(B * Ho * Wo);
      op_conv3(c, x.p, B, H, Wd, st.rc, W_(c, st.rw), W_(c, st.rb), st.rc, 2, 0, nullptr, 0, nullptr, d.p, 1, nullptr, 0, nullptr, 0, nullptr, want ? &gw : nullptr);
      if (want) gst_put(f, d, gw.out);
      H = Ho; Wd = Wo; x = d;
      skips.push_back(x); skip_c.push_back(st.rc);
    }
  }
  {
    T2 r0 = run_resnet(f, c->mid_r0, x, H, Wd);
    T2 t = run_transformer(f, c->mid_t, r0, H, Wd, true); act_free(f, r0);
    T2 r1 = run_resnet(f, c->mid_r1, t, H, Wd, nullptr, 0, true); act_free(f, t);
    x = r1;
  }
  for (int i = 0; i < n; ++i) {
    const Stage& st = c->up[i];
    for (size_t j = 0; j < st.res.size(); ++j) {
      T2 sk = skips.back(); skips.pop_back();
      const int cs = skip_c.back(); skip_c.pop_back();
      const int cx = st.res[j].cin - cs;
      const long M = (long)B * H * Wd;
      T2 r;
      const bool att = !st.att.empty();
      const bool last = i == n - 1 && j + 1 == st.res.size();
      if (c->sc_fuse && c->cat_free && st.res[j].shortcut && cx % 64 == 0 && cs % 64 == 0) {
        r = run_resnet(f, st.res[j], x, H, Wd, &sk, cx, !att && !last);
        act_free(f, x); act_free(f, sk);
      } else {
        T2 cat = wsalloc(c, (size_t)M * st.res[j].cin);
        {
          ProfScope ps(c, PK_CONCAT, 0, 4.0 * M * st.res[j].cin);
          CHECK_LAUNCH(c, ia2p_launch_concat(x.p, cx, cx, sk.p, cs, cs, cat.p, M, c->stream), "concat");
        }
        act_free(f, x); act_free(f, sk);
        r = run_resnet(f, st.res[j], cat, H, Wd, nullptr, 0, !att && !last);
        act_free(f, cat);
      }
      if (att) { T2 t = run_transformer(f, st.att[j], r, H, Wd, true); act_free(f, r); r = t; }
      x = r;
    }
    if (st.resample) {
      T2 u = wsalloc(c, (size_t)B * (2 * H) * (2 * Wd) * st.rc);
      GnWant gw{4 * H * Wd};
      const bool want = f.gn_on && ia2p_plan_any_gn(4 * B * H * Wd);
      op_conv3(c, x.p, B, H, Wd, st.rc, W_(c, st.rw), W_(c, st.rb), st.rc, 1, 1, nullptr, 0, nullptr, u.p, 1, nullptr, 0, nullptr, 0, nullptr, want ? &gw : nullptr);
      if (want) gst_put(f, u, gw.out);
      act_free(f, x);
      H *= 2; Wd *= 2; x = u;
    }
  }
  if (H != h || Wd != w) return fail(c, IA2P_ERR_SHAPE, "latent %dx%d does not survive the down/up path (needs divisibility by 2^%d)", h, w, n - 1);
  const int c0 = g.block_out_channels[0];
  T2 no = wsalloc(c, (size_t)B * H * Wd * c0);
  op_gn(c, x.p, no.p, c->ngo, c->nbo, B, H * Wd, c0, g.norm_eps, 1, f.gn_partial);
  act_free(f, x);
  {
    RoleScope role(c, ROLE_CONV_IO);
    ProfScope ps(c, PK_CONV_OUT, 2.0 * B * H * Wd * 9.0 * c0 * g.out_channels, 2.0 * ((double)B * H * Wd * (c0 + g.out_channels) + 9.0 * c0 * g.out_channels));
    CHECK_LAUNCH(c, ia2p_launch_conv_out(no.p, c0, W_(c, c->conv_out_w), W_(c, c->conv_out_b), out, B, c0, H, Wd, g.out_channels, c->stream), "conv_out");
  }
  for (auto& kv : f.gst) wsfree(c, kv.second.buf);
  f.gst.clear();
  wsfree(c, no); wsfree(c, f.temb_all); wsfree(c, gnp); wsfree(c, f.kv_text); wsfree(c, f.kv_ip);
  return c->failed ? IA2P_ERR_HIP : IA2P_OK;
}

ia2p_status rc_bind_arena(RunCtx* c, void* dev, size_t bytes) {
  if (!c || !dev) return fail(c, IA2P_ERR_INVALID, "bind_arena: null argument");
  if (bytes < c->arena_elems * sizeof(half_t)) return fail(c, IA2P_ERR_NOMEM, "arena needs %zu bytes, got %zu", c->arena_elems * sizeof(half_t), bytes);
  if (((uintptr_t)dev) & 255) return fail(c, IA2P_ERR_INVALID, "arena must be 256-byte aligned");
  c->arena = (half_t*)dev;
  c->finalized = false;
  c->wseq_key = -1;
  return IA2P_OK;
}
ia2p_status rc_load_tensor(RunCtx* c, const char* key, const void* src, const int64_t* shape, int ndim, void* stream) {
  if (!c || !key || !src || !shape) return fail(c, IA2P_ERR_INVALID, "load_tensor: null argument");
  if (!c->arena) return fail(c, IA2P_ERR_STATE, "load_tensor before bind_arena");
  auto it = c->params.find(key);
  if (it == c->params.end()) return fail(c, IA2P_ERR_KEY, "unknown parameter key '%s'", key);
  Param& p = it->second;
  size_t n = 1;
  for (int i = 0; i < ndim; ++i) n *= (size_t)shape[i];
  if (n != p.elems) return fail(c, IA2P_ERR_SHAPE, "parameter '%s': expected %zu elements, got %zu", key, p.elems, n);
  hipStream_t s = (hipStream_t)stream;
  half_t* dst = c->arena + p.off;
  hipError_t e = hipSuccess;
  switch (p.kind) {
    case PK_COPY: e = hipMemcpyAsync(dst, src, n * sizeof(half_t), hipMemcpyDeviceToDevice, s); break;
    case PK_CONV: e = ia2p_launch_pack_conv((const half_t*)src, dst, p.d0, p.d1, s); break;
    case PK_CONV_TAP: e = ia2p_launch_pack_conv((const half_t*)src, dst, p.d0, p.d1, s); break;
    case PK_GEGLU_W: case PK_GEGLU_B: e = ia2p_launch_pack_geglu((const half_t*)src, dst, p.d0, p.d1, s); break;
    case PK_PAD_CONV_IN: e = ia2p_launch_pack_conv_in((const half_t*)src, dst, p.d0, p.d1, s); break;
  }
  if (e != hipSuccess) return fail_hip(c, e, (std::string("load '") + key + "'").c_str());
  p.loaded = true;
  c->fold_dirty = true;
  return IA2P_OK;
}
ia2p_status rc_finalize(RunCtx* c, const char* what) {
  if (!c) return IA2P_ERR_INVALID;
  if (!c->arena) return fail(c, IA2P_ERR_STATE, "finalize before bind_arena");
  int missing = 0;
  std::string first;
  for (auto& kv : c->params)
    if (!kv.second.loaded && !kv.second.optional) { if (!missing) first = kv.first; ++missing; }
  if (missing) return fail(c, IA2P_ERR_KEY, "%d %s parameters not loaded (e.g. '%s')", missing, what, first.c_str());
  c->finalized = true;
  return IA2P_OK;
}
ia2p_status rc_adopt(RunCtx* c, bool with_optional) {
  if (!c || !c->arena) return fail(c, IA2P_ERR_STATE, "adopt_arena before bind_arena");
  for (auto& kv : c->params)
    if (with_optional || !kv.second.optional) kv.second.loaded = true;
  c->finalized = true;
  return IA2P_OK;
}

extern "C" {

int ia2p_device_is_gfx950(void) {
  int dev = 0;
  hipDeviceProp_t p;
  if (hipGetDevice(&dev) != hipSuccess || hipGetDeviceProperties(&p, dev) != hipSuccess) return 0;
  return strncmp(p.gcnArchName, "gfx950", 6) == 0;
}
// ... 439 lines not shown
                                const void* gamma, const void* beta, void* y, int B, int HW, int groups, float eps, int silu) {
  if (!x0 || !y || (C1 > 0 && !x1)) return fail(nullptr, IA2P_ERR_INVALID, "gn_apply_stats: null argument");
  GemmArgs::GnIn g;
  const ia2p_status st = gn_in_from_abi("gn_apply_stats", &g, C0, st0, rows0, C1, st1, rows1, gamma, beta, groups, eps, silu, HW);
  if (st != IA2P_OK) return st;
  hipError_t e = ia2p_launch_gn_apply_stats((const half_t*)x0, C0, C1 > 0 ? (const half_t*)x1 : nullptr, C1, (half_t*)y, C0 + C1, B, HW, C0 + C1, g, (hipStream_t)stream);
  RET_HIP(e, "gn_apply_stats");
}
ia2p_status ia2p_conv3x3_gn(void* stream, const ia2p_conv_gn* d, int* gn_out_rows) {
  if (gn_out_rows) *gn_out_rows = 0;
  if (!d || !d->x0 || !d->Wp || !d->y || (d->splitk > 1 && !d->partial) || (d->Ca > 0 && !d->xa)) return fail(nullptr, IA2P_ERR_INVALID, "conv3x3_gn: null argument");
  const int Cin = d->C0 + (d->st0 ? d->C1 : 0), HW = d->H * d->W;
  if (Cin % 64 || d->C0 % 64 || d->Co % 8 || d->Ca % 64 || d->B < 1 || HW < 1 || d->splitk < 0 || d->splitk > (9 * Cin + d->Ca) / 64 || d->splitk > 255) return fail(nullptr, IA2P_ERR_SHAPE, "conv3x3_gn: C0=%d C1=%d Co=%d Ca=%d splitk=%d", d->C0, d->C1, d->Co, d->Ca, d->splitk);
  GemmArgs a;
  memset(&a, 0, sizeof a);
  a.pad = 1; a.Ho = a.Hs = d->H; a.Wo = a.Ws = d->W; a.stride = 1;
  a.A = (const half_t*)d->x0; a.W = (const half_t*)d->Wp; a.C = (half_t*)d->y; a.zero = zero_page(); a.M = d->B * HW; a.N = d->Co; a.K = 9 * Cin + d->Ca; a.ldw = a.K; a.lda = d->C0; a.ldc = d->Co;
  a.Cin = Cin; a.bias = (const half_t*)d->bias; a.rowvec = (const half_t*)d->rowvec; a.rowvec_ld = d->Co; a.rows_per_batch = HW; a.residual = (const half_t*)d->residual; a.ldr = d->Co;
  if (d->Ca > 0) { a.A2 = (const half_t*)d->xa; a.lda2 = d->Ca; a.Cin2 = d->Ca; }
  if (d->splitk > 1) { a.splitk = d->splitk; a.partial = d->partial; }
  const GemmPlan pl = ia2p_gemm_plan(a.M, a.N, a.K, true, false);
  if (d->st0) {
    const ia2p_status st = gn_in_from_abi("conv3x3_gn", &a.gn, d->C0, d->st0, d->rows0, d->C1, d->st1, d->rows1, d->gamma, d->beta, d->groups, d->eps, 1, HW);
    if (st != IA2P_OK) return st;
    a.A1b = d->C1 > 0 ? (const half_t*)d->x1 : nullptr; a.lda1b = d->C1;
    if (d->C1 > 0 && !d->x1) return fail(nullptr, IA2P_ERR_INVALID, "conv3x3_gn: null second source");
    if (!ia2p_conv_gn_fusable(a, pl.variant, a.splitk) || !ia2p_conv_gn_ok(a)) return fail(nullptr, IA2P_ERR_SHAPE, "conv3x3_gn: this site has no halo-staged plan (variant %d) or its statistics do not fit the fused kernel", pl.variant);
  }
  const bool combined = a.splitk > 1 && ia2p_splitk_inkernel(a.M, a.N, a.splitk);
  int rows = 0;
  if (d->gn_out) { rows = gn_epilogue_rows(a, true, pl.variant, a.splitk, combined, HW); if (rows) a.gn_out = d->gn_out; }
  int comb = 0;
  hipError_t e = ia2p_launch_gemm_variant(a, true, pl.variant, (hipStream_t)stream, true, &comb);
  if (e == hipSuccess && gn_out_rows) *gn_out_rows = (rows && (a.splitk <= 1 || comb)) ? rows : 0;
  RET_HIP(e, "conv3x3_gn");
}
ia2p_status ia2p_gemm_gnstats(void* stream, const void* A, const void* W, const void* bias, const void* residual, void* C, int M, int N, int K, int splitk, float* partial,
                              int HW, double* gn_out, int* rows) {
  if (rows) *rows = 0;
  if (!A || !W || !C || !gn_out || !rows || (splitk > 1 && !partial)) return fail(nullptr, IA2P_ERR_INVALID, "gemm_gnstats: null argument");
  if (K % 64 || N % 8 || HW < 16 || M % HW || splitk < 0 || splitk > K / 64 || splitk > 255) return fail(nullptr, IA2P_ERR_SHAPE, "gemm_gnstats: K=%d N=%d HW=%d splitk=%d", K, N, HW, splitk);
  GemmArgs a;
  memset(&a, 0, sizeof a);
  a.pad = 1;
  a.A = (const half_t*)A; a.W = (const half_t*)W; a.C = (half_t*)C; a.zero = zero_page(); a.M = M; a.N = N; a.K = K; a.ldw = a.K; a.lda = K; a.ldc = N;
  a.bias = (const half_t*)bias; a.residual = (const half_t*)residual; a.ldr = N; a.rows_per_batch = 1; a.m_fastest = M <= N;
  if (splitk > 1) { a.splitk = splitk; a.partial = partial; }
  const GemmPlan pl = ia2p_gemm_plan(M, N, K, false, false);
  const bool combined = splitk > 1 && ia2p_splitk_inkernel(M, N, splitk);
  const int r = gn_epilogue_rows(a, false, pl.variant, a.splitk, combined, HW);
  if (r) a.gn_out = gn_out;
  int comb = 0;
  hipError_t e = ia2p_launch_gemm_variant(a, false, pl.variant, (hipStream_t)stream, true, &comb);
  if (e == hipSuccess) *rows = (r && (a.splitk <= 1 || comb)) ? r : 0;
  RET_HIP(e, "gemm_gnstats");
}
ia2p_status ia2p_conv3x3_cat(void* stream, const void* x, const void* x2, const void* Wcat, const void* bias, void* y, int B, int Hs, int Ws, int Cin, int Cin2, int Co) {
  if (!x || !x2 || !Wcat || !y) return fail(nullptr, IA2P_ERR_INVALID, "conv3x3_cat: null argument");
  if (Cin % 64 || Cin2 % 64 || Cin2 < 64 || Co % 4) return fail(nullptr, IA2P_ERR_SHAPE, "conv3x3_cat: Cin=%d, Cin2=%d (multiples of 64) Co=%d (mult of 4)", Cin, Cin2, Co);
  GemmArgs a;
  memset(&a, 0, sizeof a);
  a.pad = 1;
  a.Ho = Hs; a.Wo = Ws;
  a.A = (const half_t*)x; a.W = (const half_t*)Wcat; a.C = (half_t*)y; a.zero = zero_page(); a.M = B * Hs * Ws; a.N = Co; a.K = 9 * Cin + Cin2; a.ldw = a.K; a.lda = Cin; a.ldc = Co;
  a.Hs = Hs; a.Ws = Ws; a.stride = 1; a.up = 0; a.Cin = Cin; a.bias = (const half_t*)bias; a.rows_per_batch = Hs * Ws;
  a.A2 = (const half_t*)x2; a.lda2 = Cin2; a.Cin2 = Cin2;
  hipError_t e = ia2p_launch_gemm(a, true, (hipStream_t)stream, nullptr);
  RET_HIP(e, "conv3x3_cat");
}
ia2p_status ia2p_pack_conv3x3(void* stream, const void* src, void* dst, int Co, int Cin) {
  if (!src || !dst) return fail(nullptr, IA2P_ERR_INVALID, "pack_conv3x3: null argument");
  if (Cin % 64) return fail(nullptr, IA2P_ERR_SHAPE, "pack_conv3x3: Cin=%d must be a multiple of 64 (the layout of ia2p_conv3x3; ia2p_pack_conv_out packs for ia2p_conv_out)", Cin);
  hipError_t e = ia2p_launch_pack_conv((const half_t*)src, (half_t*)dst, Co, Cin, (hipStream_t)stream);
  RET_HIP(e, "pack_conv3x3");
}
ia2p_status ia2p_pack_conv_out(void* stream, const void* src, void* dst, int Co, int C) {
  if (!src || !dst) return fail(nullptr, IA2P_ERR_INVALID, "pack_conv_out: null argument");
  hipError_t e = ia2p_launch_pack_conv((const half_t*)src, (half_t*)dst, Co, C, (hipStream_t)stream);
  RET_HIP(e, "pack_conv_out");
}
ia2p_status ia2p_conv_in(void* stream, const void* x_nchw, const void* w_oihw, const void* bias, void* y_nhwc, void* w_scratch, int B, int Cin, int H, int W, int Co) {
  if (!x_nchw || !w_oihw || !bias || !y_nhwc || !w_scratch) return fail(nullptr, IA2P_ERR_INVALID, "conv_in: null argument");
  if (B < 1 || H < 1 || W < 1 || Cin < 1 || Cin * 9 > 64 || Co < 8 || Co % 8) return fail(nullptr, IA2P_ERR_SHAPE, "conv_in: Cin*9=%d must be <= 64, Co=%d a multiple of 8", Cin * 9, Co);
  hipError_t e = ia2p_launch_pack_conv_in((const half_t*)w_oihw, (half_t*)w_scratch, Co, Cin * 9, (hipStream_t)stream);
  if (e == hipSuccess) e = ia2p_launch_conv_in((const half_t*)x_nchw, (const half_t*)w_scratch, (const half_t*)bias, (half_t*)y_nhwc, B, Cin, H, W, Co, (hipStream_t)stream);
  RET_HIP(e, "conv_in");
}
ia2p_status ia2p_conv_out(void* stream, const void* x_nhwc, const void* w_packed, const void* bias, void* y_nchw, int B, int C, int H, int W, int Co) {
  if (!x_nhwc || !w_packed || !bias || !y_nchw) return fail(nullptr, IA2P_ERR_INVALID, "conv_out: null argument");
  if (B < 1 || H < 1 || W < 1 || C < 32 || C % 32 || Co < 1 || Co > 8) return fail(nullptr, IA2P_ERR_SHAPE, "conv_out: C=%d must be a multiple of 32, Co=%d <= 8", C, Co);
  hipError_t e = ia2p_launch_conv_out((const half_t*)x_nhwc, C, (const half_t*)w_packed, (const half_t*)bias, (half_t*)y_nchw, B, C, H, W, Co, (hipStream_t)stream);
  RET_HIP(e, "conv_out");
}
ia2p_status ia2p_pack_geglu(void* stream, const void* src, void* dst, int rows, int rowlen) {
  if (!src || !dst || rows % 32) return fail(nullptr, IA2P_ERR_SHAPE, "pack_geglu: rows must be a multiple of 32");
  hipError_t e = ia2p_launch_pack_geglu((const half_t*)src, (half_t*)dst, rows, rowlen, (hipStream_t)stream);
  RET_HIP(e, "pack_geglu");
}
ia2p_status ia2p_attention(void* stream, const void* Q, int ldq, void* O, int ldo, int B, int heads, int Nq, int nseg,
                           const void* K0, const void* V0, int ld0, int nkeys0, float w0, const void* K1, const void* V1, int ld1, int nkeys1, float w1) {
  if (!Q || !O || !K0 || !V0 || nseg < 1 || nseg > 2 || (nseg == 2 && (!K1 || !V1))) return fail(nullptr, IA2P_ERR_INVALID, "attention: bad argument");
  if (nkeys0 < 1 || (nseg == 2 && nkeys1 < 1) || ldq % 8 || ldo % 8 || (((uintptr_t)O) & 15) || ld0 % 8 || (nseg == 2 && ld1 % 8)) return fail(nullptr, IA2P_ERR_SHAPE, "attention: key counts must be >= 1, strides multiples of 8, O 16-byte aligned");
  AttnArgs a;
  memset(&a, 0, sizeof a);
  a.Q = (const half_t*)Q; a.ldq = ldq; a.O = (half_t*)O; a.ldo = ldo; a.B = B; a.heads = heads; a.Nq = Nq; a.nseg = nseg;
  a.scale_log2e = 0.125f * 1.4426950408889634f;
  a.seg[0] = AttnSeg{(const half_t*)K0, (const half_t*)V0, nkeys0, ld0, nkeys0, w0};
  a.seg[1] = AttnSeg{(const half_t*)K1, (const half_t*)V1, nkeys1, ld1, nkeys1, w1};
  hipError_t e = ia2p_launch_attention(a, (hipStream_t)stream);
  RET_HIP(e, "attention");
}
ia2p_status ia2p_qproj_attention(void* stream, const void* X, const void* Wq, const void* bias, const ia2p_ln_fold* ln, void* O, int ldo, int B, int heads,
                                 int Nq, int K, int nseg, const void* K0, const void* V0, int ld0, int nkeys0, float w0,
                                 const void* K1, const void* V1, int ld1, int nkeys1, float w1) {
  if (!X || !Wq || !O || !K0 || !V0 || nseg < 1 || nseg > 2 || (nseg == 2 && (!K1 || !V1))) return fail(nullptr, IA2P_ERR_INVALID, "qproj_attention: bad argument");
  if (ln && (!ln->stats || !ln->colsum || !ln->fbias || ln->slots < 1)) return fail(nullptr, IA2P_ERR_INVALID, "qproj_attention: incomplete ia2p_ln_fold");
  if (B < 1 || heads < 1 || Nq < 128 || Nq % 128 || K < 64 || K % 64 || nkeys0 < 1 || (nseg == 2 && nkeys1 < 1) || ldo % 8 || (((uintptr_t)O) & 15) || ld0 % 8 || (nseg == 2 && ld1 % 8))
    return fail(nullptr, IA2P_ERR_SHAPE, "qproj_attention: Nq=%d must be a multiple of 128, K=%d of 64, key counts >= 1, strides multiples of 8, O 16-byte aligned", Nq, K);
  GemmArgs a;
  memset(&a, 0, sizeof a);
  a.pad = 1;
  a.A = (const half_t*)X; a.W = (const half_t*)Wq; a.zero = zero_page(); a.M = B * Nq; a.N = heads * 64; a.K = K; a.ldw = K; a.lda = K; a.ldc = a.N;
  a.bias = (const half_t*)bias; a.rows_per_batch = 1; a.m_fastest = a.M <= a.N;
  if (ln) { a.ln_stats = ln->stats; a.ln_slots = ln->slots; a.ln_cs = ln->colsum; a.ln_bias = ln->fbias; a.ln_eps = ln->eps; }
  AttnArgs x;
  memset(&x, 0, sizeof x);
  x.O = (half_t*)O; x.ldo = ldo; x.B = B; x.heads = heads; x.Nq = Nq; x.nseg = nseg;
  x.scale_log2e = 0.125f * 1.4426950408889634f;
  x.seg[0] = AttnSeg{(const half_t*)K0, (const half_t*)V0, nkeys0, ld0, nkeys0, w0};
  x.seg[1] = AttnSeg{(const half_t*)K1, (const half_t*)V1, nkeys1, ld1, nkeys1, w1};
  if (!ia2p_qproj_xattn_ok(a, x)) return fail(nullptr, IA2P_ERR_SHAPE, "qproj_attention: shape not supported by the fused tile (bias must be 16-byte aligned)");
  hipError_t e = ia2p_launch_qproj_xattn(a, x, (hipStream_t)stream);
  RET_HIP(e, "qproj_attention");
}
ia2p_status ia2p_qkv_self_attention(void* stream, const void* X, const void* Wqkv, const void* bias, const ia2p_ln_fold* ln, void* O, int ldo, int B, int heads, int K) {
  if (!X || !Wqkv || !O) return fail(nullptr, IA2P_ERR_INVALID, "qkv_self_attention: null argument");
  if (ln && (!ln->stats || !ln->colsum || !ln->fbias || ln->slots < 1)) return fail(nullptr, IA2P_ERR_INVALID, "qkv_self_attention: incomplete ia2p_ln_fold");
  if (B < 1 || heads < 1 || K < 64 || K % 64 || ldo % 8 || (((uintptr_t)O) & 15)) return fail(nullptr, IA2P_ERR_SHAPE, "qkv_self_attention: K=%d (multiple of 64), ldo=%d (multiple of 8), O 16-byte aligned", K, ldo);
  GemmArgs a;
  memset(&a, 0, sizeof a);
  a.pad = 1;
  a.A = (const half_t*)X; a.W = (const half_t*)Wqkv; a.zero = zero_page(); a.M = B * 256; a.N = 3 * heads * 64; a.K = K; a.ldw = K; a.lda = K; a.ldc = a.N;
  a.bias = (const half_t*)bias; a.rows_per_batch = 1;
  if (ln) { a.ln_stats = ln->stats; a.ln_slots = ln->slots; a.ln_cs = ln->colsum; a.ln_bias = ln->fbias; a.ln_eps = ln->eps; }
  AttnArgs x;
  memset(&x, 0, sizeof x);
  x.O = (half_t*)O; x.ldo = ldo; x.B = B; x.heads = heads; x.Nq = 256; x.nseg = 1;
  x.scale_log2e = 0.125f * 1.4426950408889634f;
  x.seg[0].nkeys = 256; x.seg[0].weight = 1.f;
  if (!ia2p_qkv_sattn_ok(a, x)) return fail(nullptr, IA2P_ERR_SHAPE, "qkv_self_attention: shape / alignment not supported by the fused tile");
  hipError_t e = ia2p_launch_qkv_sattn(a, x, (hipStream_t)stream);
  RET_HIP(e, "qkv_self_attention");
}
ia2p_status ia2p_ip_attn_map(void* stream, const void* Q, int ldq, const void* Kip, int ldk, void* out, int B, int heads, int Nq, int ntok) {
  if (!Q || !Kip || !out || B < 1 || heads < 1 || Nq < 1) return fail(nullptr, IA2P_ERR_INVALID, "ip_attn_map: bad argument");
  if (ntok < 1 || ntok > 16 || ldq % 8 || ldq < heads * 64 || ldk < heads * 64) return fail(nullptr, IA2P_ERR_SHAPE, "ip_attn_map: ntok=%d (1..16), ldq=%d (mult of 8), ldk=%d", ntok, ldq, ldk);
  hipError_t e = ia2p_launch_ip_attn_map((const half_t*)Q, ldq, (const half_t*)Kip, ldk, (half_t*)out, B, heads, Nq, ntok, (hipStream_t)stream);
  RET_HIP(e, "ip_attn_map");
}
ia2p_status ia2p_linear_small(void* stream, const void* X, const void* W, const void* bias, void* out, int M, int N, int K, int silu_in, int silu_out) {
  if (!X || !W || !out) return fail(nullptr, IA2P_ERR_INVALID, "linear_small: null argument");
  if (M > 16 || K % 8) return fail(nullptr, IA2P_ERR_SHAPE, "linear_small: M=%d (<=16) K=%d (mult of 8)", M, K);
  hipError_t e = ia2p_launch_linear_small((const half_t*)X, K, (const half_t*)W, (const half_t*)bias, nullptr, 0, (half_t*)out, N, M, N, K, silu_in, silu_out, (hipStream_t)stream);
  RET_HIP(e, "linear_small");
}

ia2p_status ia2p_profile_enable(ia2p_ctx* c, int on) {
  if (!c) return IA2P_ERR_INVALID;
  for (auto& r : c->recs) { c->evpool.push_back(r.e0); c->evpool.push_back(r.e1); }
  c->recs.clear();
  for (int k = 0; k < PK_NCLASS; ++k) { c->p_ms[k] = c->p_fl[k] = c->p_by[k] = c->p_pf[k] = 0; c->p_n[k] = 0; }
  for (int k = 0; k < PR_NREGION; ++k) { c->r_ms[k] = c->r_fl[k] = c->r_by[k] = 0; c->r_n[k] = 0; }
  for (int k = 0; k < ROLE_NROLE; ++k) { c->o_ms[k] = c->o_fl[k] = c->o_by[k] = 0; c->o_n[k] = 0; for (int q = 0; q < PK_NCLASS; ++q) { c->oc_ms[k][q] = 0; c->oc_n[k][q] = 0; } }
  c->prof = on != 0;
  return IA2P_OK;
}
int ia2p_profile_classes(void) { return PK_NCLASS; }
static void prof_fold(ia2p_ctx* c) {
  for (auto& r : c->recs) {
    float t = 0.f;
    (void)hipEventSynchronize(r.e1);
    (void)hipEventElapsedTime(&t, r.e0, r.e1);
    c->p_ms[r.k] += t; c->p_fl[r.k] += r.flops; c->p_by[r.k] += r.bytes; c->p_pf[r.k] += r.pf; c->p_n[r.k] += 1;
    const int g = r.region >= 0 && r.region < PR_NREGION ? r.region : PR_OTHER;
    c->r_ms[g] += t; c->r_fl[g] += r.flops; c->r_by[g] += r.bytes; c->r_n[g] += 1;
    const int o = r.role >= 0 && r.role < ROLE_NROLE ? r.role : ROLE_OTHER;
    c->o_ms[o] += t; c->o_fl[o] += r.flops; c->o_by[o] += r.bytes; c->o_n[o] += 1;
    c->oc_ms[o][r.k] += t; c->oc_n[o][r.k] += 1;
    c->evpool.push_back(r.e0); c->evpool.push_back(r.e1);
  }
  c->recs.clear();
}
ia2p_status ia2p_profile_read_region(ia2p_ctx* c, int region, int64_t* launches, double* ms, double* flops, double* bytes) {
  if (!c || region < 0 || region >= PR_NREGION) return IA2P_ERR_INVALID;
  prof_fold(c);
  if (launches) *launches = c->r_n[region];
  if (ms) *ms = c->r_ms[region];
  if (flops) *flops = c->r_fl[region];
  if (bytes) *bytes = c->r_by[region];
  return IA2P_OK;
}
int ia2p_profile_roles(void) { return ROLE_NROLE; }
ia2p_status ia2p_profile_read_role(ia2p_ctx* c, int role, char* name, int name_len, int64_t* launches, double* ms, double* flops, double* bytes) {
  if (!c || role < 0 || role >= ROLE_NROLE) return IA2P_ERR_INVALID;
  prof_fold(c);
  if (name && name_len > 0) { strncpy(name, role_name(role), name_len - 1); name[name_len - 1] = 0; }
  if (launches) *launches = c->o_n[role];
  if (ms) *ms = c->o_ms[role];
  if (flops) *flops = c->o_fl[role];
  if (bytes) *bytes = c->o_by[role];
  return IA2P_OK;
}
ia2p_status ia2p_profile_read_role_class(ia2p_ctx* c, int role, int k, int64_t* launches, double* ms) {
  if (!c || role < 0 || role >= ROLE_NROLE || k < 0 || k >= PK_NCLASS) return IA2P_ERR_INVALID;
  prof_fold(c);
  if (launches) *launches = c->oc_n[role][k];
  if (ms) *ms = c->oc_ms[role][k];
  return IA2P_OK;
}
ia2p_status ia2p_profile_read_prefetch(ia2p_ctx* c, int k, double* bytes) {
  if (!c || k < 0 || k >= PK_NCLASS || !bytes) return IA2P_ERR_INVALID;
  prof_fold(c);
  *bytes = c->p_pf[k];
  return IA2P_OK;
}
ia2p_status ia2p_profile_read(ia2p_ctx* c, int k, char* name, int name_len, int64_t* launches, double* ms, double* flops, double* bytes) {
  if (!c || k < 0 || k >= PK_NCLASS) return IA2P_ERR_INVALID;
  prof_fold(c);
  if (name && name_len > 0) { strncpy(name, prof_name(k), name_len - 1); name[name_len - 1] = 0; }
  if (launches) *launches = c->p_n[k];
  if (ms) *ms = c->p_ms[k];
  if (flops) *flops = c->p_fl[k];
  if (bytes) *bytes = c->p_by[k];
  return IA2P_OK;
}

}
```

### instructany2pix_amd/csrc/engine_rt.h

```cpp
#pragma once

#include <hip/hip_runtime.h>

#include <cmath>
#include <cstdarg>
#include <cstdio>
#include <algorithm>
#include <cstdlib>
#include <cstring>
#include <string>
#include <unordered_map>
#include <vector>

#include "../../include/ia2p_debug.h"
#include "common.h"

hipError_t ia2p_launch_gemm(const GemmArgs& a, bool conv, hipStream_t s, int* picked, int* combined = nullptr);
hipError_t ia2p_launch_gemm_variant(const GemmArgs& a, bool conv, int variant, hipStream_t s, bool with_reduce = true, int* combined = nullptr, int* ran = nullptr);
int ia2p_gemm_variant_ran(const GemmArgs& a, bool conv, int v);
bool ia2p_conv_gn_fusable(const GemmArgs& a, int v, int splitk);
bool ia2p_plan_any_gn(int M);
void ia2p_conv_gn_candidates(const GemmArgs& a, size_t max_slab_bytes, std::vector<GemmPlan>* out);
hipError_t ia2p_launch_gn_colstats(const half_t* x, int ldx, int M, int C, int rows, double* out, hipStream_t s);
hipError_t ia2p_launch_gn_apply_stats(const half_t* x0, int ld0, const half_t* x1, int ld1, half_t* y, int ldy, int B, int HW, int C, const GemmArgs::GnIn& g, hipStream_t s);
hipError_t ia2p_launch_splitk_reduce(const GemmArgs& a, hipStream_t s);
bool ia2p_splitk_inkernel(int M, int N, int splitk);
void ia2p_gemm_candidates(int M, int N, int K, bool conv, bool geglu, size_t max_slab_bytes, double slack, std::vector<GemmPlan>* out);
hipError_t ia2p_launch_attention(const AttnArgs& a, hipStream_t s);
bool ia2p_qproj_xattn_ok(const GemmArgs& a, const AttnArgs& x);
hipError_t ia2p_launch_qproj_xattn(const GemmArgs& a, const AttnArgs& x, hipStream_t s);
bool ia2p_qkv_sattn_ok(const GemmArgs& a, const AttnArgs& x);
hipError_t ia2p_launch_qkv_sattn(const GemmArgs& a, const AttnArgs& x, hipStream_t s);
int ia2p_gn_chunks(int B, int HW);
hipError_t ia2p_launch_groupnorm(const half_t* x, int ldx, half_t* y, int ldy, const half_t* gamma, const half_t* beta,
                                 float* partial, int B, int HW, int C, int G, float eps, int silu, hipStream_t s, const half_t* x2 = nullptr, int ldx2 = 0, int Ca = 0);
hipError_t ia2p_launch_layernorm(const half_t* x, int ldx, half_t* y, int ldy, const half_t* gamma, const half_t* beta,
                                 int M, int C, float eps, hipStream_t s);
hipError_t ia2p_launch_embed(float t, const float* ts, const half_t* text_embeds, const half_t* time_ids, half_t* tsin, half_t* addin,
                             int B, int Tp, int P, int Ad, int nids, hipStream_t s);
hipError_t ia2p_launch_linear_small(const half_t* X, int ldx, const half_t* W, const half_t* bias, const half_t* addend, int ldadd,
                                    half_t* out, int ldo, int M, int N, int K, int silu_in, int silu_out, hipStream_t s);
hipError_t ia2p_launch_conv_in(const half_t* x, const half_t* w, const half_t* bias, half_t* y, int B, int Cin, int H, int W, int Co, hipStream_t s, float out_scale = 1.0f);
hipError_t ia2p_launch_conv_out(const half_t* x, int ldx, const half_t* w, const half_t* bias, half_t* y, int B, int C, int H, int W, int Co, hipStream_t s);
hipError_t ia2p_launch_concat(const half_t* a, int lda, int Ca, const half_t* b, int ldb, int Cb, half_t* y, long M, hipStream_t s);
hipError_t ia2p_launch_ddim_step(const half_t* x, const half_t* eps_u, const half_t* eps_c, float g, float c_x, float c_e,
                                 half_t* out, half_t* out2, long n, hipStream_t s, const float* coef = nullptr, long per = 1);
hipError_t ia2p_launch_mask_blend(const half_t* x, const half_t* init, const half_t* noise, const half_t* mask, float c0, float c1,
                                  half_t* out, half_t* out2, int B, int C, long HW, hipStream_t s);
hipError_t ia2p_launch_cat_rows(const half_t* a, int Ka, const half_t* b, int Kb, const half_t* bias_a, const half_t* bias_b, half_t* dst, half_t* bias_dst, int rows, hipStream_t s);
hipError_t ia2p_launch_fold_ln(const half_t* W, const half_t* gamma, const half_t* beta, const half_t* bias, half_t* Wf, float* cs, float* lb,
                               int N, int K, hipStream_t s);
hipError_t ia2p_launch_clip_embed(const int* ids, const half_t* tok, const half_t* embeds, const half_t* pos, half_t* x, float* stats, int rows, int T, int H,
                                  int vocab, hipStream_t s);
hipError_t ia2p_launch_prior_step(const float* smp, const half_t* o_c, const half_t* o_u, const float* noise, float g, float sqrt_a, float sqrt_b, float k0, float k1,
                                  float sigma, float* out, long n, hipStream_t s);
hipError_t ia2p_launch_causal_attention_small(const half_t* qkv, half_t* out, int B, int T, int heads, hipStream_t s);
hipError_t ia2p_launch_clip_pool(const int* ids, const half_t* x, const half_t* gamma, const half_t* beta, half_t* out, int B, int T, int H, int eos_id,
                                 float eps, hipStream_t s);
hipError_t ia2p_launch_ip_attn_map(const half_t* Q, int ldq, const half_t* Kip, int ldk, half_t* out, int B, int heads, int Nq, int ntok, hipStream_t s);
hipError_t ia2p_launch_touch(const void* p, size_t bytes, unsigned* sink, hipStream_t s);
hipError_t ia2p_launch_pack_conv(const half_t* src, half_t* dst, int Co, int Ci, hipStream_t s);
hipError_t ia2p_launch_pack_conv_in(const half_t* src, half_t* dst, int Co, int KT, hipStream_t s);
hipError_t ia2p_launch_pack_geglu(const half_t* src, half_t* dst, int rows, int rowlen, hipStream_t s);
hipError_t ia2p_launch_softmax_rows(half_t* x, long ld, int rows, int n, float scale, hipStream_t s);
hipError_t ia2p_launch_conv1x1_nchw(const half_t* x, const half_t* w, const half_t* bias, half_t* y, int B, int Ci, int Co, long HW, hipStream_t s);

extern thread_local std::string g_err;
const half_t* zero_page();

enum PKind { PK_COPY = 0, PK_CONV = 1, PK_GEGLU_W = 2, PK_GEGLU_B = 3, PK_PAD_CONV_IN = 4, PK_CONV_TAP = 5, PK_Q4 = 6 };

struct Param {
  size_t off;
  size_t elems;
  int kind;
  int d0, d1;
  bool loaded;
  bool optional;
};

struct Block { size_t off, size; bool free_; };

struct Arena {
  std::vector<Block> blocks;
  size_t cap, high;
  void reset(size_t c) { cap = c; high = 0; blocks.clear(); blocks.push_back({0, c, true}); }
  size_t alloc(size_t bytes) {
    bytes = (bytes + 255) & ~(size_t)255;
    for (size_t i = 0; i < blocks.size(); ++i)
      if (blocks[i].free_ && blocks[i].size >= bytes) {
        const size_t off = blocks[i].off;
        if (blocks[i].size > bytes) {
          Block rest{off + bytes, blocks[i].size - bytes, true};
          blocks[i].size = bytes;
          blocks.insert(blocks.begin() + i + 1, rest);
        }
        blocks[i].free_ = false;
        if (off + bytes > high) high = off + bytes;
        return off;
      }
    return (size_t)-1;
  }
  void release(size_t off) {
    for (size_t i = 0; i < blocks.size(); ++i)
      if (blocks[i].off == off && !blocks[i].free_) {
        blocks[i].free_ = true;
        if (i + 1 < blocks.size() && blocks[i + 1].free_) { blocks[i].size += blocks[i + 1].size; blocks.erase(blocks.begin() + i + 1); }
        if (i > 0 && blocks[i - 1].free_) { blocks[i - 1].size += blocks[i].size; blocks.erase(blocks.begin() + i); }
        return;
      }
  }
};

struct ProfRec { hipEvent_t e0, e1; int k; double flops, bytes; int region; double pf; int role; };
enum { PR_OTHER = 0, PR_CONV_BLOCK = 1, PR_TRANSFORMER = 2, PR_NREGION };
enum { ROLE_OTHER = 0, ROLE_FF_IN, ROLE_FF_OUT, ROLE_QKV_SATTN, ROLE_ATTN_OUT, ROLE_Q_XATTN, ROLE_CONV3X3, ROLE_GROUPNORM, ROLE_PROJ_IO, ROLE_CTX_KV, ROLE_EMBED, ROLE_CONV_IO, ROLE_NROLE };
const char* role_name(int r);
enum { PK_GEMM0 = 0, PK_CONV0 = IA2P_GEMM_NVARIANT, PK_ATTN = 2 * IA2P_GEMM_NVARIANT, PK_GN, PK_LN, PK_EMBED, PK_CONV_IN, PK_CONV_OUT, PK_CONCAT, PK_REDUCE, PK_QXATTN, PK_QKVATTN, PK_HALO_GN0 , PK_NCLASS = PK_HALO_GN0 + 3 };
const char* prof_name(int k);

void ia2p_sk_counters_invalidate();
int ia2p_default_xattn_min_tiles();
struct RunCtx {
  std::string err;
  std::unordered_map<std::string, Param> params;
  size_t arena_elems = 0;
  half_t* arena = nullptr;
  bool finalized = false;
  int groups = 32;
  Arena ws;
  char* ws_base = nullptr;
  bool dry = false;
  hipStream_t stream = nullptr;
  bool failed = false;
  std::vector<std::pair<const half_t*, size_t>> wseq;
  size_t widx = 0;
  bool record = false;
  int wseq_key = -1;
  bool prefetch = true;
  const half_t* tail_pf = nullptr;
  size_t tail_pf_bytes = 0;
  int xattn_min_tiles = 128;
  bool cat_free = true;
  bool sc_fuse = true;
  bool xattn_fuse = true;
  int gn_dry_mode = -1;
  int gn_fuse = 1;
  bool sattn_fuse = true;
  bool ln_fold = true;
  bool prof = false;
#ifdef IA2P_CLOCK_STAMP
  static constexpr int STAMP_WG = 2048;
  unsigned long long* stamp_buf = nullptr;
  int stamp_role = -1, stamp_cap = 0, stamp_n = 0;
  struct StampMeta { int M, N, K, variant, tiles; };
  std::vector<StampMeta> stamp_meta;
#endif
  bool tuning = false;
  int tune_reps = 5, tune_sites = 0;
  double tune_gn_ms = 0.0;
  const GemmArgs* tune_fused = nullptr;
  char* tune_scratch = nullptr;
  size_t tune_slab_bytes = 0, tune_flush_bytes = 0;
  std::vector<ProfRec> recs;
  std::vector<hipEvent_t> evpool;
  double p_ms[PK_NCLASS], p_fl[PK_NCLASS], p_by[PK_NCLASS], p_pf[PK_NCLASS];
  int64_t p_n[PK_NCLASS];
  int region = PR_OTHER;
  int role = ROLE_OTHER;
  double o_ms[ROLE_NROLE], o_fl[ROLE_NROLE], o_by[ROLE_NROLE];
  int64_t o_n[ROLE_NROLE];
  double oc_ms[ROLE_NROLE][PK_NCLASS];
  int64_t oc_n[ROLE_NROLE][PK_NCLASS];
  double r_ms[PR_NREGION], r_fl[PR_NREGION], r_by[PR_NREGION];
  int64_t r_n[PR_NREGION];
  float ep_acc_scale = 1.f, ep_bias_scale = 1.f;
  bool fold_dirty = false;
  RunCtx() {
    if (const char* e = getenv("IA2P_PREFETCH")) prefetch = atoi(e) != 0;
    if (const char* e = getenv("IA2P_LN_FOLD")) ln_fold = atoi(e) != 0;
    if (const char* e = getenv("IA2P_XATTN_FUSE")) xattn_fuse = sattn_fuse = atoi(e) != 0;
    if (const char* e = getenv("IA2P_GN_FUSE")) gn_fuse = atoi(e);
    if (const char* e = ia2p_exp_env("IA2P_SATTN_FUSE")) sattn_fuse = atoi(e) != 0;
    if (const char* e = ia2p_exp_env("IA2P_SC_FUSE")) sc_fuse = atoi(e) != 0;
    if (const char* e = ia2p_exp_env("IA2P_CAT_FREE")) cat_free = atoi(e) != 0;
    if (ia2p_default_xattn_min_tiles() >= 0) xattn_min_tiles = ia2p_default_xattn_min_tiles();
    for (int k = 0; k < PK_NCLASS; ++k) { p_ms[k] = p_fl[k] = p_by[k] = p_pf[k] = 0; p_n[k] = 0; }
    for (int k = 0; k < PR_NREGION; ++k) { r_ms[k] = r_fl[k] = r_by[k] = 0; r_n[k] = 0; }
    for (int k = 0; k < ROLE_NROLE; ++k) { o_ms[k] = o_fl[k] = o_by[k] = 0; o_n[k] = 0; for (int q = 0; q < PK_NCLASS; ++q) { oc_ms[k][q] = 0; oc_n[k][q] = 0; } }
  }
  ~RunCtx() {
    for (auto& r : recs) { (void)hipEventDestroy(r.e0); (void)hipEventDestroy(r.e1); }
    for (auto e : evpool) (void)hipEventDestroy(e);
  }
};

ia2p_status fail(RunCtx* c, ia2p_status st, const char* fmt, ...);
ia2p_status fail_hip(RunCtx* c, hipError_t e, const char* what);

struct T2 { size_t off; half_t* p; };
T2 wsalloc(RunCtx* c, size_t elems);
void wsfree(RunCtx* c, T2 t);
hipEvent_t get_event(RunCtx* c);

struct ProfScope {
  RunCtx* c; int k; double fl, by; hipEvent_t e0, e1; bool on; double pf = 0;
  ProfScope(RunCtx* c_, int k_, double fl_, double by_) : c(c_), k(k_), fl(fl_), by(by_), on(c_ && c_->prof && !c_->dry) {
    if (on) { e0 = get_event(c); e1 = get_event(c); (void)hipEventRecord(e0, c->stream); }
  }
  ~ProfScope() { if (on) { (void)hipEventRecord(e1, c->stream); c->recs.push_back(ProfRec{e0, e1, k, fl, by, c->region, pf, c->role}); } }
  void set_class(int kk) { k = kk; }
};
struct RoleScope { RunCtx* c; int prev; RoleScope(RunCtx* c_, int r) : c(c_), prev(c_->role) { c->role = r; } ~RoleScope() { c->role = prev; } };
#define CHECK_LAUNCH(c, expr, what)                                                             \
  do { if (!(c)->dry && !(c)->failed) { hipError_t e_ = (expr); if (e_ != hipSuccess) { if (e_ != hipErrorInvalidValue) ia2p_sk_counters_invalidate(); fail((c), IA2P_ERR_HIP, "%s: %s", what, hipGetErrorString(e_)); } } } while (0)

inline const half_t* W_(RunCtx* c, size_t off) { return c->arena + off; }

#define RET_HIP(e, what) do { if ((e) == hipSuccess) return IA2P_OK; if ((e) != hipErrorInvalidValue) ia2p_sk_counters_invalidate(); return fail(nullptr, IA2P_ERR_HIP, "%s: %s", what, hipGetErrorString(e)); } while (0)

struct GnStats { T2 buf{(size_t)-1, nullptr}; int rows = 0; bool ok() const { return rows > 0; } };
struct GnWant { int HW; GnStats out; };
struct ConvGn { bool fused = false; const half_t* X1b = nullptr; int C0 = 0; GnStats s0, s1; const half_t* gamma = nullptr; const half_t* beta = nullptr; float eps = 1e-5f; int groups = 32;
                bool tune = false; const half_t* Xraw = nullptr; };
struct LnIn { const float* stats; int slots; const float* cs; const float* lb; float eps; };

void op_gemm(RunCtx* c, const half_t* A, int lda, const half_t* W, const half_t* bias, const half_t* residual, int ldr,
             half_t* C, int ldc, int M, int N, int K, int geglu = 0, int rpb = 0, int bstride = 0, int roff = 0, int ldw = 0,
             const LnIn* ln = nullptr, float* stats_out = nullptr, int* stat_slots = nullptr, int act = 0, GnWant* gw = nullptr);
void op_conv3(RunCtx* c, const half_t* X, int B, int Hs, int Ws, int Cin, const half_t* W, const half_t* bias, int Co,
              int stride, int up, const half_t* rowvec, int rowvec_ld, const half_t* residual, half_t* Y, int pad_lo = 1, const half_t* X2 = nullptr, int Cin2 = 0, const half_t* X3 = nullptr, int Cin3 = 0,
              const ConvGn* gn = nullptr, GnWant* gw = nullptr);
void op_gn(RunCtx* c, const half_t* x, half_t* y, size_t g, size_t b, int B, int HW, int C, float eps, int silu, float* partial, const half_t* x2 = nullptr, int Ca = 0);
void op_ln(RunCtx* c, const half_t* x, half_t* y, size_t g, size_t b, int M, int C);

ia2p_status rc_bind_arena(RunCtx* c, void* dev, size_t bytes);
ia2p_status rc_load_tensor(RunCtx* c, const char* key, const void* src, const int64_t* shape, int ndim, void* stream);
ia2p_status rc_finalize(RunCtx* c, const char* what);
ia2p_status rc_adopt(RunCtx* c, bool with_optional = true);
```

### instructany2pix_amd/csrc/gemm_kernel.h

```cpp
#pragma once
#include "gemm_epilogue.h"

template <int BM, int BN, int NSTAGE, bool CONV, int WGM = 2, int BK = 64, int PP = 0, int WGN = 2, int XA = 0>
__device__ __forceinline__ void gemm_tile_body(const half_t* hA, const half_t* hW, const half_t* hzero, int hM, int hN, int hK, int hlda, int hldw, int hrpb, int hbstride,
                                               int hroff, int hsplitk, int hgroup_w, int hflags, const GemmArgs& p, const AttnArgs* xa, const float* pre_ln_stats = nullptr, int pre_ln_slots = 0) {
  static_assert(PP != 1 || (WGM * WGN == 8 && (WGM == 4 || WGM == 8) && NSTAGE == 3), "ping-pong schedule: 8 waves (two groups of 4 by tile rows), 3-stage ring");
  static_assert(PP != 3 || (WGM == 4 && NSTAGE == 2 && !CONV), "two-slot ping-pong schedule: 8 waves, 2 k-tile slots");
  static_assert(PP != 2 || (WGM == 2 && WGN == 4 && NSTAGE == 2 && BK == 64 && BM == 256 && (BN == 256 || BN == 128) && XA == 0), "8-phase schedule: 256-row tiles, 2 x 4 waves, two k-tile buffers");
  constexpr int NWAVE = WGM * WGN;
  constexpr int WM = BM / WGM, WN = BN / WGN;
  constexpr int MR = WM / 16, NR = WN / 16;
  constexpr int ROWB = 2 * BK, CPR = ROWB / 16, RPP = 1024 / ROWB;
  using BS = BStage<BN, BK, NWAVE, PP>;
  constexpr int A_PW = BM / RPP / NWAVE, B_PW = BS::HI;
  constexpr bool B_UNEVEN = BS::UNEVEN;
  constexpr int BNL = BS::BNL;
  static_assert(BM % (RPP * NWAVE) == 0 && BN % 16 == 0 && WN % 16 == 0 && WM % 16 == 0, "tile / wave layout");
  constexpr int STAGE = (BM + BNL) * ROWB;
  constexpr int KSUB = BK / 32;
  extern __shared__ __attribute__((aligned(1024))) char smem[];

  const int tid = threadIdx.x;
  const int lane = tid & 63;
  const int wave = __builtin_amdgcn_readfirstlane(tid >> 6);
  constexpr bool LINBUF = !CONV && IA2P_LIN_BUF != 0;
  constexpr int OOB = 0x7fffff00;
  const __amdgpu_buffer_rsrc_t lin_rs_a = __builtin_amdgcn_make_buffer_rsrc((void*)hA, 0, 0x7ffffe00, 0x00020000);
  const __amdgpu_buffer_rsrc_t lin_rs_w = __builtin_amdgcn_make_buffer_rsrc((void*)hW, 0, 0x7ffffe00, 0x00020000);
  IA2P_STAMP(const unsigned long long stamp_entry = __builtin_amdgcn_s_memrealtime();)

  const int tiles_m = (hM + BM - 1) / BM, tiles_n = (hN + BN - 1) / BN;
  int bid = blockIdx.x;
  const int nsplit = hsplitk > 1 ? hsplitk : 1;
  const int split = bid < tiles_m * tiles_n ? 0 : udiv_small(bid, tiles_m * tiles_n);
  if (split < nsplit) bid -= split * tiles_m * tiles_n;
  if (__builtin_expect(split >= nsplit, 0)) {
    bid -= nsplit * tiles_m * tiles_n;
    const long per = ((p.pf_bytes + p.pf_blocks - 1) / p.pf_blocks + 4095) & ~4095L;
    const long lo = (long)bid * per, hi = min(lo + per, p.pf_bytes & ~15L);
    const char* src = (const char*)p.pf;
    unsigned acc = 0;
    constexpr long SW = NWAVE * 64 * 16;
#ifndef IA2P_PF_UNROLL
#define IA2P_PF_UNROLL 4
#endif
    constexpr int PU = IA2P_PF_UNROLL;
    for (long o = lo + tid * 16; o < hi; o += PU * SW) {
      unsigned v[PU];
#pragma unroll
      for (int u = 0; u < PU; ++u) v[u] = *(const unsigned*)(src + min(o + u * SW, hi - 16));
#pragma unroll
      for (int u = 0; u < PU; ++u) acc ^= v[u];
    }
    asm volatile("" ::"v"(acc));
    return;
  }
  int tm, tn;
  tile_order(bid, tiles_m, tiles_n, hgroup_w, hflags & 1, tm, tn);
  const int bm0 = tm * BM, bn0 = tn * BN;

  const int srow = lane / CPR, cpos = lane % CPR;
  constexpr int A_HP = PP == 2 ? A_PW / 2 : 1, B_HP = PP == 2 ? B_PW / 2 : 1;
  auto a_piece = [&](int i) { return PP == 2 ? (i / A_HP) * (BM / 2 / RPP) + wave * A_HP + i % A_HP : wave * A_PW + i; };
  const half_t* a_ptr[A_PW];
  int a_inc[A_PW];
  int a_voff[A_PW];
  const half_t* a_base[A_PW];
  int a_mask[A_PW];
#pragma unroll
  for (int i = 0; i < A_PW; ++i) {
    const int pi = a_piece(i);
    const int m = bm0 + pi * RPP + srow;
    const int gch = cpos ^ lds_swz<BK>(pi * RPP + srow);
    if (!CONV) {
      if (m < hM) {
        int src = m;
        if (__builtin_expect(hrpb != 0, 0)) { const int b = m / hrpb; src = b * hbstride + (m - b * hrpb) + hroff; }
        a_ptr[i] = hA + (size_t)src * hlda + gch * 8;
        a_inc[i] = BK;
        a_voff[i] = (src * hlda + gch * 8) * 2;
      } else { a_ptr[i] = hzero; a_inc[i] = 0; a_voff[i] = OOB; }
    } else {
      a_mask[i] = 0; a_base[i] = hzero;
      if (m < hM) {
        const int hw = p.Ho * p.Wo;
        const int b = m / hw, rem = m - b * hw;
        const int oy = rem / p.Wo, ox = rem - oy * p.Wo;
        const int y0 = oy * p.stride - p.pad, x0 = ox * p.stride - p.pad;
        const int Hv_ = p.Hs << p.up, Wv_ = p.Ws << p.up;
        int mk = 0;
#pragma unroll
        for (int t = 0; t < 9; ++t) mk |= ((unsigned)(y0 + t / 3) < (unsigned)Hv_ && (unsigned)(x0 + t % 3) < (unsigned)Wv_) ? 1 << t : 0;
        a_mask[i] = mk | ((y0 & 1) << 9) | ((x0 & 1) << 10);
        a_base[i] = hA + ((long)b * p.Hs * p.Ws + (long)(y0 >> p.up) * p.Ws + (x0 >> p.up)) * hlda + gch * 8;
      }
    }
  }
  const half_t* w_ptr[B_PW];
  int w_inc[B_PW];
  int w_voff[B_PW];
  const int b_npw = B_UNEVEN && wave >= NWAVE / 2 ? B_PW - 1 : B_PW;
  const int b_pi0 = B_UNEVEN ? (wave < NWAVE / 2 ? wave * B_PW : (NWAVE / 2) * B_PW + (wave - NWAVE / 2) * (B_PW - 1)) : wave * B_PW;
  auto b_piece = [&](int i) { return PP == 2 ? (i / B_HP) * (BN / 2 / RPP) + wave * B_HP + i % B_HP : b_pi0 + i; };
#pragma unroll
  for (int i = 0; i < B_PW; ++i) {
    const int pi = min(b_piece(i), BNL / RPP - 1);
    int n = bn0 + pi * RPP + srow;
    if constexpr (XA == 4) {
      const int jl = pi * RPP + srow;
      n = (jl >> 6) * (hN / 3) + tn * 64 + (jl & 63);
    }
    const int gch = cpos ^ lds_swz<BK>(pi * RPP + srow);
    if (n < hN && pi * RPP + srow < BN) { w_ptr[i] = hW + (size_t)n * hldw + gch * 8; w_inc[i] = BK; }
    else         { w_ptr[i] = hzero; w_inc[i] = 0; }
    if constexpr (LINBUF) w_voff[i] = w_inc[i] ? (n * hldw + gch * 8) * 2 : OOB;
  }

  const int nk_all = hK / BK;
  const int kt0 = nsplit == 1 ? 0 : udiv_small(split * nk_all, nsplit), kt1 = nsplit == 1 ? nk_all : udiv_small((split + 1) * nk_all, nsplit);
  int cin_main = 0, cin_extra = 0;
  if (CONV) { cin_main = p.Cin; cin_extra = p.Cin2; asm volatile("" : "+s"(cin_main), "+s"(cin_extra)); }
  const int nk_main = CONV ? 9 * (cin_main / BK) : 0;
  int tap = 0, ci0 = 0;
  if (CONV) {
    if (kt0 < nk_main) { tap = (kt0 * BK) / cin_main; ci0 = (kt0 * BK) % cin_main; }
    else {
      ci0 = kt0 * BK - 9 * cin_main; tap = 9;
      if (ci0 >= cin_extra) { ci0 -= cin_extra; tap = 10; }
    }
  }
  bool tap_fresh = true;
  auto k_next = [&](int& t, int& c) {
    if (t < 9) {
      c += BK;
      if (c >= cin_main) { c = 0; ++t; }
    } else {
      c += BK;
      if (t < 10 && c >= cin_extra) { c = 0; ++t; }
    }
  };
  int k_soff = kt0 * (2 * BK);
  if (kt0 && !LINBUF) {
    if (!CONV) {
#pragma unroll
      for (int i = 0; i < A_PW; ++i) a_ptr[i] += (size_t)kt0 * a_inc[i];
    }
#pragma unroll
    for (int i = 0; i < B_PW; ++i) w_ptr[i] += (size_t)kt0 * w_inc[i];
  }

  auto conv_tap_setup = [&]() {
    if (tap_fresh) {
      if (tap < 9) {
        const int ky = tap / 3, kx = tap - ky * 3;
        if (!p.up) {
          const long toff = ((long)ky * p.Ws + kx) * hlda + ci0;
#pragma unroll
          for (int i = 0; i < A_PW; ++i) {
            const bool ok = (a_mask[i] >> tap) & 1;
            a_ptr[i] = ok ? a_base[i] + toff : hzero;
            a_inc[i] = ok ? BK : 0;
          }
        } else {
#pragma unroll
          for (int i = 0; i < A_PW; ++i) {
            const bool ok = (a_mask[i] >> tap) & 1;
            const int dy = (ky + ((a_mask[i] >> 9) & 1)) >> 1, dx = (kx + ((a_mask[i] >> 10) & 1)) >> 1;
            a_ptr[i] = ok ? a_base[i] + ((long)dy * p.Ws + dx) * hlda + ci0 : hzero;
            a_inc[i] = ok ? BK : 0;
          }
        }
      } else {
        if (tap == 9) {
#pragma unroll
          for (int i = 0; i < A_PW; ++i) {
            const int m = bm0 + a_piece(i) * RPP + srow;
            const bool ok = m < hM;
            a_ptr[i] = ok ? p.A2 + (size_t)m * p.lda2 + ci0 + (cpos ^ lds_swz<BK>(a_piece(i) * RPP + srow)) * 8 : hzero;
            a_inc[i] = ok ? BK : 0;
          }
        } else {
#pragma unroll
          for (int i = 0; i < A_PW; ++i) {
            const int m = bm0 + a_piece(i) * RPP + srow;
            const bool ok = m < hM;
            a_ptr[i] = ok ? p.A3 + (size_t)m * p.lda3 + ci0 + (cpos ^ lds_swz<BK>(a_piece(i) * RPP + srow)) * 8 : hzero;
            a_inc[i] = ok ? BK : 0;
          }
        }
      }
// ... 430 lines not shown
```

### instructany2pix_amd/csrc/qxattn.hip

```cpp
#include "gemm_kernel.h"

#ifndef IA2P_QX_STAGES
#define IA2P_QX_STAGES 2
#endif
template <int MODE>
__global__ __launch_bounds__(256, 2) void qproj_xattn_kernel(const half_t* hA, const half_t* hW, const half_t* hzero, const float* h_ln_stats, int hM, int hN, int hK, int hlda, int hldw,
                                                             int h_slots_gw, const GemmArgs p, const AttnArgs xa) {
  gemm_tile_body<128, 64, IA2P_QX_STAGES, false, 2, 64, 0, 2, MODE + 1>(hA, hW, hzero, hM, hN, hK, hlda, hldw, 0, 0, 0, 0, IA2P_SKGW_GW(h_slots_gw), IA2P_SKGW_FLAGS(h_slots_gw), p, &xa, h_ln_stats,
                                                                        IA2P_SKGW_LO8(h_slots_gw));
}

bool ia2p_qproj_xattn_ok(const GemmArgs& a, const AttnArgs& x) {
  return x.Nq > 0 && x.Nq % 128 == 0 && a.M == x.B * x.Nq && a.N == x.heads * 64 && a.K >= 64 && a.K % 64 == 0 && a.splitk <= 1 && !a.rpb && !a.geglu && !a.residual && !a.rowvec &&
         !a.stats_out && !a.act && x.nseg >= 1 && x.nseg <= 2 && x.seg[0].nkeys > 0 && (x.nseg == 1 || x.seg[1].nkeys > 0) &&
         (!a.bias || ((((uintptr_t)a.bias) & 15) == 0 && a.N % 8 == 0)) && x.ldo % 8 == 0 && ((((uintptr_t)x.O) & 15) == 0) &&
         ia2p_fits_buffer(a.rpb ? ((size_t)a.M / a.rpb + 1) * (size_t)(a.bstride > 0 ? a.bstride : 0) + a.roff + a.rpb : (size_t)a.M, a.lda) && ia2p_fits_buffer(a.N, a.ldw) &&
         attn_kv_resident(x);
}

hipError_t ia2p_launch_qproj_xattn(const GemmArgs& a, const AttnArgs& x, hipStream_t s) {
  if (!ia2p_qproj_xattn_ok(a, x)) return hipErrorInvalidValue;
  constexpr int BM = 128, BN = 64, SMEM = EpiCfg<128, 64, IA2P_QX_STAGES, 2, 64, 2>::SMEM > 65536 ? EpiCfg<128, 64, IA2P_QX_STAGES, 2, 64, 2>::SMEM : 65536;
  static_assert(EpiCfg<BM, BN, IA2P_QX_STAGES, 2, 64, 2>::SMEM <= SMEM, "LDS budget");
  static bool attr_set[64] = {false};
  int dev = 0;
  (void)hipGetDevice(&dev);
  if (dev < 0 || dev >= 64 || !attr_set[dev]) {
    hipError_t e = hipFuncSetAttribute((const void*)qproj_xattn_kernel<0>, hipFuncAttributeMaxDynamicSharedMemorySize, SMEM);
    if (e == hipSuccess) e = hipFuncSetAttribute((const void*)qproj_xattn_kernel<1>, hipFuncAttributeMaxDynamicSharedMemorySize, SMEM);
    if (e == hipSuccess) e = hipFuncSetAttribute((const void*)qproj_xattn_kernel<2>, hipFuncAttributeMaxDynamicSharedMemorySize, SMEM);
    if (e != hipSuccess) return e;
    if (dev >= 0 && dev < 64) attr_set[dev] = true;
  }
  const int tiles_n = a.N / BN, tiles = (a.M / BM) * tiles_n;
  GemmArgs b = a;
  b.vec8 = 1; b.splitk = 0; b.sk_counters = nullptr;
#ifndef IA2P_CLOCK_STAMP
  b.partial = nullptr;
#endif
  b.group_w = ia2p_tile_group_w(tiles, tiles_n, SMEM, BM, BN);
  AttnArgs y = x;
  y.xcd_map = (((ia2p_wt_mask() & 8) && (size_t)x.B * x.Nq * x.ldo * 2 < (size_t)0x7ffffff0) ? 2 : 0) | (ia2p_attn_fold_enabled() ? 0 : 4);
  const int extra = (a.pf && a.pf_bytes >= 4096) ? a.pf_blocks : 0;
  int slots_gw;
  if (tiles + extra >= (1 << 21) || !ia2p_pack_skgw(b.ln_stats ? b.ln_slots : 0, b.group_w, b.m_fastest, b.ln_stats != nullptr, &slots_gw)) return hipErrorInvalidValue;
  const int mode = y.nseg == 1 ? 0 : (y.seg[1].nkeys <= 64 && y.seg[0].weight != 0.f) ? 1 : 2;
#define IA2P_QX_LAUNCH(MODE)                                                                                                                   \
  hipLaunchKernelGGL(qproj_xattn_kernel<MODE>, dim3(tiles + extra), dim3(256), SMEM, s, b.A, b.W, b.zero, b.ln_stats, b.M, b.N, b.K, b.lda, b.ldw, slots_gw, b, y)
  if (mode == 0) IA2P_QX_LAUNCH(0);
  else if (mode == 1) IA2P_QX_LAUNCH(1);
  else IA2P_QX_LAUNCH(2);
#undef IA2P_QX_LAUNCH
  return hipGetLastError();
}


__global__ __launch_bounds__(512, 2) void qkv_sattn_kernel(const half_t* hA, const half_t* hW, const half_t* hzero, const float* h_ln_stats, int hM, int hN, int hK, int hlda, int hldw,
                                                           int h_slots_gw, const GemmArgs p, const AttnArgs xa) {
#ifndef IA2P_SATTN_PP
#define IA2P_SATTN_PP 3
#endif
  gemm_tile_body<256, 192, 2, false, 4, 64, IA2P_SATTN_PP, 2, 4>(hA, hW, hzero, hM, hN, hK, hlda, hldw, 0, 0, 0, 0, IA2P_SKGW_GW(h_slots_gw), IA2P_SKGW_FLAGS(h_slots_gw), p, &xa, h_ln_stats, IA2P_SKGW_LO8(h_slots_gw));
}

bool ia2p_qkv_sattn_ok(const GemmArgs& a, const AttnArgs& x) {
  return x.Nq == 256 && x.B > 0 && a.M == x.B * 256 && a.N == 3 * x.heads * 64 && a.K >= 64 && a.K % 64 == 0 && a.splitk <= 1 && !a.geglu && !a.residual && !a.rowvec &&
         !a.stats_out && !a.act && !a.rpb && x.nseg == 1 && x.ldo % 8 == 0 && ((((uintptr_t)x.O) & 15) == 0) && (!a.bias || ((((uintptr_t)a.bias) & 7) == 0)) &&
         (!a.ln_stats || (((((uintptr_t)a.ln_cs) | ((uintptr_t)a.ln_bias)) & 15) == 0)) && ia2p_fits_buffer(a.M, a.lda) && ia2p_fits_buffer(a.N, a.ldw);
}

hipError_t ia2p_launch_qkv_sattn(const GemmArgs& a, const AttnArgs& x, hipStream_t s) {
  if (!ia2p_qkv_sattn_ok(a, x)) return hipErrorInvalidValue;
  constexpr int SMEM = EpiCfg<256, 192, 2, 4, 64, 2, 0>::SMEM;
  static_assert(SMEM >= 96 * 1024 + (2 * 256 + 2 * 192) * 4, "K / V / Q images + row and column constants");
  static bool attr_set[64] = {false};
  int dev = 0;
  (void)hipGetDevice(&dev);
  if (dev < 0 || dev >= 64 || !attr_set[dev]) {
    hipError_t e = hipFuncSetAttribute((const void*)qkv_sattn_kernel, hipFuncAttributeMaxDynamicSharedMemorySize, SMEM);
    if (e != hipSuccess) return e;
    if (dev >= 0 && dev < 64) attr_set[dev] = true;
  }
  const int tiles_n = x.heads, tiles = x.B * tiles_n;
  GemmArgs b = a;
  b.vec8 = 1; b.splitk = 0; b.sk_counters = nullptr;
#ifndef IA2P_CLOCK_STAMP
  b.partial = nullptr;
#endif
  b.m_fastest = 0;
  b.group_w = ia2p_tile_group_w(tiles, tiles_n, SMEM, 256, 192);
  AttnArgs y = x;
  y.seg[0].nkeys = 256; y.seg[0].weight = 1.f; y.nseg = 1;
  y.xcd_map = ((ia2p_wt_mask() & 8) && (size_t)x.B * x.Nq * x.ldo * 2 < (size_t)0x7ffffff0) ? 2 : 0;
  const int extra = (a.pf && a.pf_bytes >= 4096) ? a.pf_blocks : 0;
  int slots_gw;
  if (tiles + extra >= (1 << 21) || !ia2p_pack_skgw(b.ln_stats ? b.ln_slots : 0, b.group_w, b.m_fastest, b.ln_stats != nullptr, &slots_gw)) return hipErrorInvalidValue;
  hipLaunchKernelGGL(qkv_sattn_kernel, dim3(tiles + extra), dim3(512), SMEM, s, b.A, b.W, b.zero, b.ln_stats, b.M, b.N, b.K, b.lda, b.ldw, slots_gw, b, y);
  return hipGetLastError();
}
```

Measured before the change: 53.31 steps/s.

## Fold per-block context K/V projection tiles into fused qkv self-attention launch

Instead of projecting all cross-attention context K/V columns up front in one GEMM, per-block K/V projection tiles are appended as extra workgroups to the fused qkv+self-attention kernel. The intent is to fill idle CUs in that under-occupied launch and drop separate up-front GEMM work. The remaining columns are still projected up front in merged ranges. This adds kernarg-pointer tricks, a planning pass, and a CU-count gate that allows it only when total tiles fit on the device.

```diff
diff --git a/include/ia2p.h b/include/ia2p.h
--- a/include/ia2p.h
+++ b/include/ia2p.h
@@ -139,6 +139,9 @@
                                  const void* K1, const void* V1, int ld1, int nkeys1, float w1);
 ia2p_status ia2p_qkv_self_attention(void* stream, const void* X, const void* Wqkv, const void* bias, const ia2p_ln_fold* ln, void* O, int ldo,
                                     int B, int heads, int K);
+ia2p_status ia2p_qkv_self_attention_ctx(void* stream, const void* X, const void* Wqkv, const void* bias, const ia2p_ln_fold* ln, void* O, int ldo,
+                                        int B, int heads, int K, const void* context, int L, int Li, int ctx_dim, const void* Wkv_text, const void* Wkv_ip,
+                                        void* kv_text, void* kv_ip, int ldkv, int N, int* in_launch);
 ia2p_status ia2p_ip_attn_map(void* stream, const void* Q, int ldq, const void* Kip, int ldk, void* out, int B, int heads, int Nq, int ntok);
 ia2p_status ia2p_linear_small(void* stream, const void* X, const void* W, const void* bias, void* out, int M, int N, int K,
                               int silu_in, int silu_out);
diff --git a/instructany2pix_amd/_ffi.py b/instructany2pix_amd/_ffi.py
--- a/instructany2pix_amd/_ffi.py
+++ b/instructany2pix_amd/_ffi.py
@@ -99,6 +99,7 @@
     "ia2p_conv_out": (_I, [_P, _P, _P, _P, _P, _I, _I, _I, _I, _I]),
     "ia2p_attention": (_I, [_P, _P, _I, _P, _I, _I, _I, _I, _I, _P, _P, _I, _I, _F, _P, _P, _I, _I, _F]),
     "ia2p_qkv_self_attention": (_I, [_P, _P, _P, _P, _P, _P, _I, _I, _I, _I]),
+    "ia2p_qkv_self_attention_ctx": (_I, [_P, _P, _P, _P, _P, _P, _I, _I, _I, _I, _P, _I, _I, _I, _P, _P, _P, _P, _I, _I, _P]),
     "ia2p_qproj_attention": (_I, [_P, _P, _P, _P, _P, _P, _I, _I, _I, _I, _I, _I, _P, _P, _I, _I, _F, _P, _P, _I, _I, _F]),
     "ia2p_linear_small": (_I, [_P, _P, _P, _P, _P, _I, _I, _I, _I, _I]),
     "ia2p_ip_attn_map": (_I, [_P, _P, _I, _P, _I, _P, _I, _I, _I, _I]),
diff --git a/instructany2pix_amd/csrc/common.h b/instructany2pix_amd/csrc/common.h
--- a/instructany2pix_amd/csrc/common.h
+++ b/instructany2pix_amd/csrc/common.h
@@ -158,6 +158,12 @@
          ia2p_fits_buffer(a.M, a.lda) && ia2p_fits_buffer(a.N, a.ldw) && (!a.A2 || ia2p_fits_buffer(a.M, a.lda2)) && (!a.A3 || ia2p_fits_buffer(a.M, a.lda3));
 }
 
+struct CtxKvArgs {
+  GemmArgs g[2];
+  int nt[2];
+};
+struct CtxKvSlice { const half_t* ctx; int lda, L, Lt, Li, B; const half_t* Wt; const half_t* Wi; half_t* Ct; half_t* Ci; int ldc, N, K; };
+
 struct GemmPlan { int variant; int splitk; int gn = 0; };
 static inline bool ia2p_tile_geglu_only(int pp) { return pp == 4; }
 static inline bool ia2p_geglu320_shape_ok(int M, int N, int K, bool conv, bool geglu) { return geglu && !conv && M > 0 && M % 256 == 0 && N > 0 && N % 320 == 0 && K >= 64 && K % 64 == 0; }
diff --git a/instructany2pix_amd/csrc/engine.hip b/instructany2pix_amd/csrc/engine.hip
--- a/instructany2pix_amd/csrc/engine.hip
+++ b/instructany2pix_amd/csrc/engine.hip
@@ -420,9 +420,11 @@
   return (!a.geglu && !a.act && a.ldc % 8 == 0 && a.N % 8 == 0 && bm % 16 == 0 && HW % bm == 0 && a.M % HW == 0 && HW / bm <= IA2P_GN_MAX_SLOTS && (splitk <= 1 || combined)) ? bm : 0;
 }
 static void run_gemm(RunCtx* c, GemmArgs& a, bool conv, const char* what, double flops, double bytes, int* stat_slots = nullptr, GnWant* gw = nullptr) {
-  if (c->tuning && !c->dry && !c->failed) tune_site(c, a, conv);
+  const int plan_n = c->plan_n > 0 ? c->plan_n : a.N;
+  c->plan_n = 0;
+  if (c->tuning && !c->dry && !c->failed && plan_n == a.N) tune_site(c, a, conv);
   c->tune_fused = nullptr; c->tune_gn_ms = 0.0;
-  const GemmPlan pl = ia2p_gemm_plan(a.M, a.N, a.K, conv, a.geglu != 0);
+  const GemmPlan pl = ia2p_gemm_plan(a.M, plan_n, a.K, conv, a.geglu != 0);
   if (pl.variant < 0 || pl.variant >= IA2P_GEMM_NVARIANT) { fail(c, IA2P_ERR_INVALID, "%s: tile variant %d out of range", what, pl.variant); return; }
   if (c->tuning && !c->dry && pl.splitk > 1 && (size_t)pl.splitk * a.M * a.N * sizeof(float) > c->tune_slab_bytes) {
     fail(c, IA2P_ERR_NOMEM, "%s: plan (variant %d, K split %d) needs %zu bytes of slabs, the autotune scratch holds %zu", what, pl.variant, pl.splitk,
@@ -563,6 +565,7 @@
   const float* ip_scales = nullptr;
   std::unordered_map<size_t, GnStats> gst;
   bool gn_on = false;
+  std::unordered_map<int, int> kv_inlaunch;
   bool tune_like = false;
 };
 static void gst_put(Fwd& f, T2 t, const GnStats& s) { if (s.ok() && t.off != (size_t)-1) f.gst[t.off] = s; else if (s.buf.off != (size_t)-1) wsfree(f.c, s.buf); }
@@ -717,7 +720,7 @@
   return out;
 }
 
-static void op_qkv_sattn(RunCtx* c, const half_t* A, int lda, const half_t* W, const LnIn* ln, int M, int C, const AttnArgs& x) {
+static void op_qkv_sattn(RunCtx* c, const half_t* A, int lda, const half_t* W, const LnIn* ln, int M, int C, const AttnArgs& x, const CtxKvSlice* ck = nullptr) {
   GemmArgs a;
   memset(&a, 0, sizeof a);
   a.pad = 1;
@@ -733,9 +736,11 @@
     ++c->stamp_n;
   }
 #endif
-  ProfScope ps(c, PK_QKVATTN, 2.0 * M * 3.0 * C * C + 4.0 * x.B * x.heads * (double)x.Nq * x.Nq * 64, 2.0 * ((double)M * C + 3.0 * C * C + (double)M * C));
+  const double ck_rows = ck ? (double)ck->B * ck->L : 0.0;
+  ProfScope ps(c, PK_QKVATTN, 2.0 * M * 3.0 * C * C + 4.0 * x.B * x.heads * (double)x.Nq * x.Nq * 64 + (ck ? 2.0 * ck_rows * ck->N * ck->K : 0.0),
+               2.0 * ((double)M * C + 3.0 * C * C + (double)M * C) + (ck ? 2.0 * (ck_rows * ck->K + (ck->Li > 0 ? 2.0 : 1.0) * ck->N * ck->K + ck_rows * ck->N) : 0.0));
   ps.pf = a.pf ? (double)a.pf_bytes : 0.0;
-  CHECK_LAUNCH(c, ia2p_launch_qkv_sattn(a, x, c->stream), "qkv projection + self-attention");
+  CHECK_LAUNCH(c, ia2p_launch_qkv_sattn(a, x, c->stream, ck), "qkv projection + self-attention");
 }
 
 static void op_attn(RunCtx* c, const AttnArgs& a) {
@@ -768,6 +773,85 @@
   ProfScope ps(c, PK_QXATTN, 2.0 * M * N * K + 4.0 * x.B * x.heads * (double)x.Nq * keys * 64,
                2.0 * ((double)M * K + (double)N * K + (double)M * N + 2.0 * x.B * keys * x.heads * 64));
   CHECK_LAUNCH(c, ia2p_launch_qproj_xattn(a, x, c->stream), "to_q + cross-attention");
+}
+
+static void project_context(ia2p_ctx* c, const half_t* context, int L, int B, half_t* kv_text, half_t* kv_ip, int col0 = 0, int ncols = -1) {
+  RegionScope rs(c, PR_TRANSFORMER);
+  RoleScope role(c, ROLE_CTX_KV);
+  const int ctxd = c->cfg.cross_attention_dim;
+  const int Lt = c->ip_enabled ? L - c->ip_tokens : L, Li = c->ip_enabled ? c->ip_tokens : 0;
+  if (ncols < 0) ncols = c->kv_rows - col0;
+  const bool part = ncols != c->kv_rows;
+  if (part) c->plan_n = c->kv_rows;
+  op_gemm(c, context, ctxd, W_(c, c->kv_text_base + (size_t)col0 * ctxd), nullptr, nullptr, 0, kv_text ? kv_text + col0 : nullptr, c->kv_rows, B * Lt, ncols, ctxd, 0, Lt, L, 0);
+  if (part && Li) c->plan_n = c->kv_rows;
+  if (Li) op_gemm(c, context, ctxd, W_(c, c->kv_ip_base + (size_t)col0 * ctxd), nullptr, nullptr, 0, kv_ip ? kv_ip + col0 : nullptr, c->kv_rows, B * Li, ncols, ctxd, 0, Li, L, Lt);
+}
+
+static bool sattn_fusable(Fwd& f, const Transformer& t, const TBlock& b, int HW, const half_t* tk, const float* st, int slots, half_t* O) {
+#ifdef IA2P_NO_SATTN_FUSE
+  return false;
+#else
+  ia2p_ctx* c = f.c;
+  const int C = t.c, M = f.B * HW;
+  if (!(c->ln_fold && c->sattn_fuse && HW == 256 && C == t.heads * 64 && (long)f.B * t.heads >= c->xattn_min_tiles)) return false;
+  AttnArgs sa;
+  memset(&sa, 0, sizeof sa);
+  sa.O = O; sa.ldo = C; sa.B = f.B; sa.heads = t.heads; sa.Nq = HW; sa.nseg = 1;
+  GemmArgs g;
+  memset(&g, 0, sizeof g);
+  g.A = tk; g.W = W_(c, b.fqkv); g.M = M; g.N = 3 * C; g.K = C; g.lda = C; g.ldw = C; g.ldc = 3 * C;
+  g.ln_stats = st; g.ln_slots = slots; g.ln_cs = (const float*)(c->arena + b.cs1); g.ln_bias = (const float*)(c->arena + b.lb1);
+  return ia2p_qkv_sattn_ok(g, sa);
+#endif
+}
+static CtxKvSlice ctx_kv_slice(Fwd& f, const Transformer& t, const TBlock& b) {
+  ia2p_ctx* c = f.c;
+  const int ctxd = c->cfg.cross_attention_dim;
+  const int Li = c->ip_enabled ? c->ip_tokens : 0, Lt = f.L - Li;
+  CtxKvSlice k;
+  memset(&k, 0, sizeof k);
+  k.ctx = f.ctxp; k.lda = ctxd; k.L = f.L; k.Lt = Lt; k.Li = Li; k.B = f.B;
+  k.Wt = W_(c, b.wkv2); k.Wi = Li ? W_(c, b.wkvip) : nullptr;
+  k.Ct = f.kv_text.p ? f.kv_text.p + b.kv_col : nullptr; k.Ci = (Li && f.kv_ip.p) ? f.kv_ip.p + b.kv_col : nullptr;
+  k.ldc = c->kv_rows; k.N = 2 * t.c; k.K = ctxd;
+  return k;
+}
+static std::vector<std::pair<int, int>> plan_context_kv(Fwd& f, int h, int w) {
+  ia2p_ctx* c = f.c;
+  std::vector<std::pair<int, int>> up_front;
+  f.kv_inlaunch.clear();
+  const int ctxd = c->cfg.cross_attention_dim;
+  const int Li = c->ip_enabled ? c->ip_tokens : 0, Lt = f.L - Li;
+  bool on = c->ctx_kv_inlaunch && ia2p_gemm_plan(f.B * Lt, c->kv_rows, ctxd, false, false).splitk <= 1 && (!Li || ia2p_gemm_plan(f.B * Li, c->kv_rows, ctxd, false, false).splitk <= 1);
+  std::vector<std::pair<int, int>> cols;
+  auto visit = [&](const Transformer& t, int HW) {
+    for (const TBlock& b : t.blocks) {
+      cols.push_back({b.kv_col, 2 * t.c});
+      if (!on || !sattn_fusable(f, t, b, HW, nullptr, c->dry ? nullptr : (const float*)16, 1, nullptr)) continue;
+      AttnArgs sa;
+      memset(&sa, 0, sizeof sa);
+      sa.B = f.B; sa.heads = t.heads;
+      if (ia2p_qkv_sattn_ctx_ok(sa, ctx_kv_slice(f, t, b))) f.kv_inlaunch[b.kv_col] = 1;
+    }
+  };
+  int H = h, Wd = w;
+  for (const Stage& st : c->down) {
+    for (const Transformer& t : st.att) visit(t, H * Wd);
+    if (st.resample) { H = (H - 1) / 2 + 1; Wd = (Wd - 1) / 2 + 1; }
+  }
+  visit(c->mid_t, H * Wd);
+  for (const Stage& st : c->up) {
+    for (const Transformer& t : st.att) visit(t, H * Wd);
+    if (st.resample) { H *= 2; Wd *= 2; }
+  }
+  std::sort(cols.begin(), cols.end());
+  for (const auto& cw : cols) {
+    if (f.kv_inlaunch.count(cw.first)) continue;
+    if (!up_front.empty() && up_front.back().second == cw.first) up_front.back().second = cw.first + cw.second;
+    else up_front.push_back({cw.first, cw.first + cw.second});
+  }
+  return up_front;
 }
 
 static T2 run_transformer(Fwd& f, const Transformer& t, T2 x, int H, int Wd, bool out_stats = false) {
@@ -797,25 +881,20 @@
   for (const TBlock& b : t.blocks) {
     {
     RoleScope role_sa(c, ROLE_QKV_SATTN);
-#ifdef IA2P_NO_SATTN_FUSE
-    bool fuse_sa = false;
-#else
-    bool fuse_sa = fold && c->sattn_fuse && HW == 256 && C == t.heads * 64 && (long)f.B * t.heads >= c->xattn_min_tiles;
-#endif
+    const bool fuse_sa = sattn_fusable(f, t, b, HW, tk.p, st, slots, att.p);
     AttnArgs sa;
     memset(&sa, 0, sizeof sa);
     sa.O = att.p; sa.ldo = C; sa.B = f.B; sa.heads = t.heads; sa.Nq = HW; sa.nseg = 1; sa.scale_log2e = sl2e;
     sa.seg[0].nkeys = HW; sa.seg[0].weight = 1.f;
-    if (fuse_sa) {
-      GemmArgs g;
-      memset(&g, 0, sizeof g);
-      g.A = tk.p; g.W = W_(c, b.fqkv); g.M = M; g.N = 3 * C; g.K = C; g.lda = C; g.ldw = C; g.ldc = 3 * C;
-      g.ln_stats = st; g.ln_slots = slots; g.ln_cs = F_(b.cs1); g.ln_bias = F_(b.lb1);
-      fuse_sa = ia2p_qkv_sattn_ok(g, sa);
-    }
+    auto kvi = f.kv_inlaunch.find(b.kv_col);
+    const bool kv_mine = kvi != f.kv_inlaunch.end() && kvi->second == 1;
+    const CtxKvSlice ck = ctx_kv_slice(f, t, b);
+    const bool kv_here = kv_mine && fuse_sa && ia2p_qkv_sattn_ctx_ok(sa, ck);
+    if (kv_mine && !kv_here) project_context(c, f.ctxp, f.L, f.B, f.kv_text.p, f.kv_ip.p, b.kv_col, 2 * C);
+    if (kv_mine) kvi->second = 2;
     if (fuse_sa) {
       const LnIn ln{st, slots, F_(b.cs1), F_(b.lb1), eps};
-      op_qkv_sattn(c, tk.p, C, W_(c, b.fqkv), &ln, M, C, sa);
+      op_qkv_sattn(c, tk.p, C, W_(c, b.fqkv), &ln, M, C, sa, kv_here ? &ck : nullptr);
     } else if (fold) {
       const LnIn ln{st, slots, F_(b.cs1), F_(b.lb1), eps};
       op_gemm(c, tk.p, C, W_(c, b.fqkv), nullptr, nullptr, 0, qkv.p, 3 * C, M, 3 * C, C, 0, 0, 0, 0, 0, &ln);
@@ -876,15 +955,6 @@
   return out;
 }
 
-static void project_context(ia2p_ctx* c, const half_t* context, int L, int B, half_t* kv_text, half_t* kv_ip) {
-  RegionScope rs(c, PR_TRANSFORMER);
-  RoleScope role(c, ROLE_CTX_KV);
-  const int ctxd = c->cfg.cross_attention_dim;
-  const int Lt = c->ip_enabled ? L - c->ip_tokens : L, Li = c->ip_enabled ? c->ip_tokens : 0;
-  op_gemm(c, context, ctxd, W_(c, c->kv_text_base), nullptr, nullptr, 0, kv_text, c->kv_rows, B * Lt, c->kv_rows, ctxd, 0, Lt, L, 0);
-  if (Li) op_gemm(c, context, ctxd, W_(c, c->kv_ip_base), nullptr, nullptr, 0, kv_ip, c->kv_rows, B * Li, c->kv_rows, ctxd, 0, Li, L, Lt);
-}
-
 static ia2p_status run_forward(ia2p_ctx* c, const half_t* sample, float timestep, const half_t* context, int L,
                                const half_t* text_embeds, const half_t* time_ids, half_t* out, int B, int h, int w,
                                const half_t* kv_cached = nullptr, const float* timesteps = nullptr, const float* ip_scales = nullptr) {
@@ -930,7 +1000,9 @@
     } else {
       f.kv_text = wsalloc(c, (size_t)B * Lt * c->kv_rows);
       if (Li) f.kv_ip = wsalloc(c, (size_t)B * Li * c->kv_rows);
-      project_context(c, context, L, B, f.kv_text.p, f.kv_ip.p);
+      const std::vector<std::pair<int, int>> up_front = plan_context_kv(f, h, w);
+      if (c->tuning || f.tune_like) project_context(c, context, L, B, f.kv_text.p, f.kv_ip.p);
+      else for (const auto& r : up_front) project_context(c, context, L, B, f.kv_text.p, f.kv_ip.p, r.first, r.second - r.first);
     }
   }
 
@@ -1676,6 +1748,48 @@
   hipError_t e = ia2p_launch_qkv_sattn(a, x, (hipStream_t)stream);
   RET_HIP(e, "qkv_self_attention");
 }
+ia2p_status ia2p_qkv_self_attention_ctx(void* stream, const void* X, const void* Wqkv, const void* bias, const ia2p_ln_fold* ln, void* O, int ldo, int B, int heads, int K,
+                                        const void* context, int L, int Li, int ctx_dim, const void* Wkv_text, const void* Wkv_ip, void* kv_text, void* kv_ip, int ldkv, int N,
+                                        int* in_launch) {
+  if (!X || !Wqkv || !O || !context || !Wkv_text || !kv_text || (Li > 0 && (!Wkv_ip || !kv_ip))) return fail(nullptr, IA2P_ERR_INVALID, "qkv_self_attention_ctx: null argument");
+  if (ln && (!ln->stats || !ln->colsum || !ln->fbias || ln->slots < 1)) return fail(nullptr, IA2P_ERR_INVALID, "qkv_self_attention_ctx: incomplete ia2p_ln_fold");
+  if (B < 1 || heads < 1 || K < 64 || K % 64 || ldo % 8 || (((uintptr_t)O) & 15)) return fail(nullptr, IA2P_ERR_SHAPE, "qkv_self_attention_ctx: K=%d (multiple of 64), ldo=%d (multiple of 8), O 16-byte aligned", K, ldo);
+  if (Li < 0 || L <= Li || L > 0xffff || ctx_dim < 64 || ctx_dim % 64 || N < 8 || N % 8 || ldkv < N || ldkv % 8 || (((uintptr_t)kv_text) & 15) || (Li > 0 && (((uintptr_t)kv_ip) & 15)))
+    return fail(nullptr, IA2P_ERR_SHAPE, "qkv_self_attention_ctx: L=%d > Li=%d >= 0, ctx_dim=%d (multiple of 64), N=%d and ldkv=%d (multiples of 8, ldkv >= N), outputs 16-byte aligned", L, Li, ctx_dim, N, ldkv);
+  if (!zero_page()) return fail(nullptr, IA2P_ERR_HIP, "cannot allocate zero page");
+  GemmArgs a;
+  memset(&a, 0, sizeof a);
+  a.pad = 1;
+  a.A = (const half_t*)X; a.W = (const half_t*)Wqkv; a.zero = zero_page(); a.M = B * 256; a.N = 3 * heads * 64; a.K = K; a.ldw = K; a.lda = K; a.ldc = a.N;
+  a.bias = (const half_t*)bias; a.rows_per_batch = 1;
+  if (ln) { a.ln_stats = ln->stats; a.ln_slots = ln->slots; a.ln_cs = ln->colsum; a.ln_bias = ln->fbias; a.ln_eps = ln->eps; }
+  AttnArgs x;
+  memset(&x, 0, sizeof x);
+  x.O = (half_t*)O; x.ldo = ldo; x.B = B; x.heads = heads; x.Nq = 256; x.nseg = 1;
+  x.scale_log2e = 0.125f * 1.4426950408889634f;
+  x.seg[0].nkeys = 256; x.seg[0].weight = 1.f;
+  if (!ia2p_qkv_sattn_ok(a, x)) return fail(nullptr, IA2P_ERR_SHAPE, "qkv_self_attention_ctx: shape / alignment not supported by the fused tile");
+  const int Lt = L - Li;
+  CtxKvSlice k;
+  memset(&k, 0, sizeof k);
+  k.ctx = (const half_t*)context; k.lda = ctx_dim; k.L = L; k.Lt = Lt; k.Li = Li; k.B = B; k.Wt = (const half_t*)Wkv_text; k.Wi = (const half_t*)Wkv_ip;
+  k.Ct = (half_t*)kv_text; k.Ci = (half_t*)kv_ip; k.ldc = ldkv; k.N = N; k.K = ctx_dim;
+  const bool inl = ia2p_qkv_sattn_ctx_ok(x, k);
+  if (in_launch) *in_launch = inl ? 1 : 0;
+  hipError_t e = hipSuccess;
+  if (!inl) {
+    for (int seg = 0; seg < (Li > 0 ? 2 : 1) && e == hipSuccess; ++seg) {
+      GemmArgs g;
+      memset(&g, 0, sizeof g);
+      g.pad = 1;
+      g.A = k.ctx; g.W = seg ? k.Wi : k.Wt; g.C = seg ? k.Ci : k.Ct; g.zero = zero_page(); g.M = B * (seg ? Li : Lt); g.N = N; g.K = ctx_dim; g.ldw = ctx_dim; g.lda = ctx_dim; g.ldc = ldkv;
+      g.rpb = seg ? Li : Lt; g.bstride = L; g.roff = seg ? Lt : 0; g.rows_per_batch = 1; g.m_fastest = g.M <= g.N ? 1 : 0; g.acc_scale = g.bias_scale = 1.f;
+      e = ia2p_launch_gemm_variant(g, false, ia2p_gemm_plan(g.M, g.N, g.K, false, false).variant, (hipStream_t)stream);
+    }
+  }
+  if (e == hipSuccess) e = ia2p_launch_qkv_sattn(a, x, (hipStream_t)stream, inl ? &k : nullptr);
+  RET_HIP(e, "qkv_self_attention_ctx");
+}
 ia2p_status ia2p_ip_attn_map(void* stream, const void* Q, int ldq, const void* Kip, int ldk, void* out, int B, int heads, int Nq, int ntok) {
   if (!Q || !Kip || !out || B < 1 || heads < 1 || Nq < 1) return fail(nullptr, IA2P_ERR_INVALID, "ip_attn_map: bad argument");
   if (ntok < 1 || ntok > 16 || ldq % 8 || ldq < heads * 64 || ldk < heads * 64) return fail(nullptr, IA2P_ERR_SHAPE, "ip_attn_map: ntok=%d (1..16), ldq=%d (mult of 8), ldk=%d", ntok, ldq, ldk);
diff --git a/instructany2pix_amd/csrc/engine_rt.h b/instructany2pix_amd/csrc/engine_rt.h
--- a/instructany2pix_amd/csrc/engine_rt.h
+++ b/instructany2pix_amd/csrc/engine_rt.h
@@ -30,7 +30,10 @@
 bool ia2p_qproj_xattn_ok(const GemmArgs& a, const AttnArgs& x);
 hipError_t ia2p_launch_qproj_xattn(const GemmArgs& a, const AttnArgs& x, hipStream_t s);
 bool ia2p_qkv_sattn_ok(const GemmArgs& a, const AttnArgs& x);
-hipError_t ia2p_launch_qkv_sattn(const GemmArgs& a, const AttnArgs& x, hipStream_t s);
+int ia2p_cu_count();
+int ia2p_qkv_sattn_ctx_tiles(const CtxKvSlice& k);
+bool ia2p_qkv_sattn_ctx_ok(const AttnArgs& x, const CtxKvSlice& k);
+hipError_t ia2p_launch_qkv_sattn(const GemmArgs& a, const AttnArgs& x, hipStream_t s, const CtxKvSlice* ctx = nullptr);
 int ia2p_gn_chunks(int B, int HW);
 hipError_t ia2p_launch_groupnorm(const half_t* x, int ldx, half_t* y, int ldy, const half_t* gamma, const half_t* beta,
                                  float* partial, int B, int HW, int C, int G, float eps, int silu, hipStream_t s, const half_t* x2 = nullptr, int ldx2 = 0, int Ca = 0);
@@ -147,6 +150,8 @@
   int gn_dry_mode = -1;
   int gn_fuse = 1;
   bool sattn_fuse = true;
+  bool ctx_kv_inlaunch = true;
+  int plan_n = 0;
   bool ln_fold = true;
   bool prof = false;
 #ifdef IA2P_CLOCK_STAMP
@@ -180,6 +185,7 @@
     if (const char* e = getenv("IA2P_PREFETCH")) prefetch = atoi(e) != 0;
     if (const char* e = getenv("IA2P_LN_FOLD")) ln_fold = atoi(e) != 0;
     if (const char* e = getenv("IA2P_XATTN_FUSE")) xattn_fuse = sattn_fuse = atoi(e) != 0;
+    if (const char* e = getenv("IA2P_CTX_KV_INLAUNCH")) ctx_kv_inlaunch = atoi(e) != 0;
     if (const char* e = getenv("IA2P_GN_FUSE")) gn_fuse = atoi(e);
     if (const char* e = ia2p_exp_env("IA2P_SATTN_FUSE")) sattn_fuse = atoi(e) != 0;
     if (const char* e = ia2p_exp_env("IA2P_SC_FUSE")) sc_fuse = atoi(e) != 0;
diff --git a/instructany2pix_amd/csrc/gemm_kernel.h b/instructany2pix_amd/csrc/gemm_kernel.h
--- a/instructany2pix_amd/csrc/gemm_kernel.h
+++ b/instructany2pix_amd/csrc/gemm_kernel.h
@@ -1,9 +1,9 @@
 #pragma once
 #include "gemm_epilogue.h"
 
-template <int BM, int BN, int NSTAGE, bool CONV, int WGM = 2, int BK = 64, int PP = 0, int WGN = 2, int XA = 0>
+template <int BM, int BN, int NSTAGE, bool CONV, int WGM = 2, int BK = 64, int PP = 0, int WGN = 2, int XA = 0, bool SUB = false>
 __device__ __forceinline__ void gemm_tile_body(const half_t* hA, const half_t* hW, const half_t* hzero, int hM, int hN, int hK, int hlda, int hldw, int hrpb, int hbstride,
-                                               int hroff, int hsplitk, int hgroup_w, int hflags, const GemmArgs& p, const AttnArgs* xa, const float* pre_ln_stats = nullptr, int pre_ln_slots = 0) {
+                                               int hroff, int hsplitk, int hgroup_w, int hflags, const GemmArgs& p, const AttnArgs* xa, const float* pre_ln_stats = nullptr, int pre_ln_slots = 0, int bid0 = 0) {
   static_assert(PP != 1 || (WGM * WGN == 8 && (WGM == 4 || WGM == 8) && NSTAGE == 3), "ping-pong schedule: 8 waves (two groups of 4 by tile rows), 3-stage ring");
   static_assert(PP != 3 || (WGM == 4 && NSTAGE == 2 && !CONV), "two-slot ping-pong schedule: 8 waves, 2 k-tile slots");
   static_assert(PP != 2 || (WGM == 2 && WGN == 4 && NSTAGE == 2 && BK == 64 && BM == 256 && (BN == 256 || BN == 128) && XA == 0), "8-phase schedule: 256-row tiles, 2 x 4 waves, two k-tile buffers");
@@ -20,7 +20,9 @@
   constexpr int KSUB = BK / 32;
   extern __shared__ __attribute__((aligned(1024))) char smem[];
 
-  const int tid = threadIdx.x;
+  int tid_ = threadIdx.x;
+  if constexpr (SUB) asm volatile("" : "+v"(tid_));
+  const int tid = tid_;
   const int lane = tid & 63;
   const int wave = __builtin_amdgcn_readfirstlane(tid >> 6);
   constexpr bool LINBUF = !CONV && IA2P_LIN_BUF != 0;
@@ -30,12 +32,26 @@
   IA2P_STAMP(const unsigned long long stamp_entry = __builtin_amdgcn_s_memrealtime();)
 
   const int tiles_m = (hM + BM - 1) / BM, tiles_n = (hN + BN - 1) / BN;
-  int bid = blockIdx.x;
+  int bid = blockIdx.x - bid0;
   const int nsplit = hsplitk > 1 ? hsplitk : 1;
   const int split = bid < tiles_m * tiles_n ? 0 : udiv_small(bid, tiles_m * tiles_n);
   if (split < nsplit) bid -= split * tiles_m * tiles_n;
   if (__builtin_expect(split >= nsplit, 0)) {
     bid -= nsplit * tiles_m * tiles_n;
+    if constexpr (XA == 4) {
+      int off = 56 + (int)sizeof(GemmArgs) + (int)sizeof(AttnArgs);
+      asm volatile("" : "+s"(off));
+      const CtxKvArgs* ck = (const CtxKvArgs*)((const __attribute__((address_space(4))) char*)__builtin_amdgcn_kernarg_segment_ptr() + off);
+      const int nt0 = ck->nt[0], nct = nt0 + ck->nt[1];
+      if (bid < nct) {
+        const int which = bid >= nt0 ? 1 : 0;
+        const GemmArgs* g = ck->g + which;
+        gemm_tile_body<128, 160, 3, false, 4, 64, 1, 2, 0, true>(g->A, g->W, g->zero, g->M, g->N, g->K, g->lda, g->ldw, g->rpb, g->bstride, g->roff, 0, g->group_w, g->m_fastest ? 1 : 0, *g, nullptr,
+                                                            nullptr, 0, (int)blockIdx.x - (which ? bid - nt0 : bid));
+        return;
+      }
+      bid -= nct;
+    }
     const long per = ((p.pf_bytes + p.pf_blocks - 1) / p.pf_blocks + 4095) & ~4095L;
     const long lo = (long)bid * per, hi = min(lo + per, p.pf_bytes & ~15L);
     const char* src = (const char*)p.pf;
diff --git a/instructany2pix_amd/csrc/qxattn.hip b/instructany2pix_amd/csrc/qxattn.hip
--- a/instructany2pix_amd/csrc/qxattn.hip
+++ b/instructany2pix_amd/csrc/qxattn.hip
@@ -1,4 +1,6 @@
 #include "gemm_kernel.h"
+
+#include <cstring>
 
 #ifndef IA2P_QX_STAGES
 #define IA2P_QX_STAGES 2
@@ -56,7 +58,7 @@
 
 
 __global__ __launch_bounds__(512, 2) void qkv_sattn_kernel(const half_t* hA, const half_t* hW, const half_t* hzero, const float* h_ln_stats, int hM, int hN, int hK, int hlda, int hldw,
-                                                           int h_slots_gw, const GemmArgs p, const AttnArgs xa) {
+                                                           int h_slots_gw, const GemmArgs p, const AttnArgs xa, const CtxKvArgs ck) {
 #ifndef IA2P_SATTN_PP
 #define IA2P_SATTN_PP 3
 #endif
@@ -69,10 +71,55 @@
          (!a.ln_stats || (((((uintptr_t)a.ln_cs) | ((uintptr_t)a.ln_bias)) & 15) == 0)) && ia2p_fits_buffer(a.M, a.lda) && ia2p_fits_buffer(a.N, a.ldw);
 }
 
-hipError_t ia2p_launch_qkv_sattn(const GemmArgs& a, const AttnArgs& x, hipStream_t s) {
+constexpr int CK_BM = 128, CK_BN = 160;
+int ia2p_cu_count() {
+  static int cus[64] = {0};
+  int dev = 0;
+  if (hipGetDevice(&dev) != hipSuccess || dev < 0 || dev >= 64) { (void)hipGetLastError(); return 0; }
+  if (!cus[dev]) {
+    int n = 0;
+    if (hipDeviceGetAttribute(&n, hipDeviceAttributeMultiprocessorCount, dev) != hipSuccess) { (void)hipGetLastError(); n = 0; }
+    cus[dev] = n > 0 ? n : -1;
+  }
+  return cus[dev] > 0 ? cus[dev] : 0;
+}
+int ia2p_qkv_sattn_ctx_tiles(const CtxKvSlice& k) {
+  const int tn = (k.N + CK_BN - 1) / CK_BN;
+  return ((k.B * k.Lt + CK_BM - 1) / CK_BM) * tn + (k.Li > 0 ? ((k.B * k.Li + CK_BM - 1) / CK_BM) * tn : 0);
+}
+bool ia2p_qkv_sattn_ctx_ok(const AttnArgs& x, const CtxKvSlice& k) {
+  if (k.B < 1 || k.B != x.B || k.Lt < 1 || k.Li < 0 || k.L != k.Lt + k.Li || k.N < 8 || k.N % 8 || k.K < 64 || k.K % 64 || k.lda < k.K || k.ldc < k.N) return false;
+  if (k.Lt > 0xffff || k.Li > 0xffff || (long)k.B * k.L >= (1L << 21)) return false;
+  if (!ia2p_fits_buffer((size_t)k.B * k.L + k.L, k.lda) || !ia2p_fits_buffer(k.N, k.K)) return false;
+  return (long)x.B * x.heads + ia2p_qkv_sattn_ctx_tiles(k) <= ia2p_cu_count();
+}
+
+hipError_t ia2p_launch_qkv_sattn(const GemmArgs& a, const AttnArgs& x, hipStream_t s, const CtxKvSlice* ctx) {
   if (!ia2p_qkv_sattn_ok(a, x)) return hipErrorInvalidValue;
   constexpr int SMEM = EpiCfg<256, 192, 2, 4, 64, 2, 0>::SMEM;
   static_assert(SMEM >= 96 * 1024 + (2 * 256 + 2 * 192) * 4, "K / V / Q images + row and column constants");
+  constexpr int CK_SMEM = EpiCfg<CK_BM, CK_BN, 3, 4, 64, 2, 1>::SMEM;
+  static_assert(CK_SMEM <= SMEM, "a context K/V tile runs in the fused tile's LDS request");
+  CtxKvArgs ck;
+  memset(&ck, 0, sizeof ck);
+  if (ctx) {
+    if (!ia2p_qkv_sattn_ctx_ok(x, *ctx) || !ctx->ctx || !ctx->Wt || !ctx->Ct || (ctx->Li > 0 && (!ctx->Wi || !ctx->Ci))) return hipErrorInvalidValue;
+    const int tn = (ctx->N + CK_BN - 1) / CK_BN;
+    auto fill = [&](GemmArgs& g, const half_t* W, half_t* C, int rows, int roff) {
+      g.pad = 1;
+      g.A = ctx->ctx; g.W = W; g.C = C; g.zero = a.zero; g.M = ctx->B * rows; g.N = ctx->N; g.K = ctx->K; g.ldw = ctx->K; g.lda = ctx->lda; g.ldc = ctx->ldc;
+      g.rpb = rows; g.bstride = ctx->L; g.roff = roff; g.rows_per_batch = 1;
+      g.m_fastest = g.M <= g.N ? 1 : 0;
+      g.acc_scale = g.bias_scale = 1.f;
+      ia2p_gemm_prepare(g, CK_SMEM, CK_BM, CK_BN);
+    };
+    fill(ck.g[0], ctx->Wt, ctx->Ct, ctx->Lt, 0);
+    ck.nt[0] = ((ck.g[0].M + CK_BM - 1) / CK_BM) * tn;
+    if (ctx->Li > 0) {
+      fill(ck.g[1], ctx->Wi, ctx->Ci, ctx->Li, ctx->Lt);
+      ck.nt[1] = ((ck.g[1].M + CK_BM - 1) / CK_BM) * tn;
+    }
+  }
   static bool attr_set[64] = {false};
   int dev = 0;
   (void)hipGetDevice(&dev);
@@ -93,8 +140,9 @@
   y.seg[0].nkeys = 256; y.seg[0].weight = 1.f; y.nseg = 1;
   y.xcd_map = ((ia2p_wt_mask() & 8) && (size_t)x.B * x.Nq * x.ldo * 2 < (size_t)0x7ffffff0) ? 2 : 0;
   const int extra = (a.pf && a.pf_bytes >= 4096) ? a.pf_blocks : 0;
+  const int nct = ck.nt[0] + ck.nt[1];
   int slots_gw;
-  if (tiles + extra >= (1 << 21) || !ia2p_pack_skgw(b.ln_stats ? b.ln_slots : 0, b.group_w, b.m_fastest, b.ln_stats != nullptr, &slots_gw)) return hipErrorInvalidValue;
-  hipLaunchKernelGGL(qkv_sattn_kernel, dim3(tiles + extra), dim3(512), SMEM, s, b.A, b.W, b.zero, b.ln_stats, b.M, b.N, b.K, b.lda, b.ldw, slots_gw, b, y);
+  if (tiles + nct + extra >= (1 << 21) || !ia2p_pack_skgw(b.ln_stats ? b.ln_slots : 0, b.group_w, b.m_fastest, b.ln_stats != nullptr, &slots_gw)) return hipErrorInvalidValue;
+  hipLaunchKernelGGL(qkv_sattn_kernel, dim3(tiles + nct + extra), dim3(512), SMEM, s, b.A, b.W, b.zero, b.ln_stats, b.M, b.N, b.K, b.lda, b.ldw, slots_gw, b, y, ck);
   return hipGetLastError();
 }
```

Result: faster. 54.29 steps/s (median of 6 runs) (+1.8%).
